# mrjoshuak/go-blosc

Measured on AMD Instinct MI355X. Metric: GB/s compress+decompress, 1 GiB float32 Shuffle+LZ4, higher is better.
Workload: dtype u8; 1 GPU; 1024 MiB f32 frame per GPU, shuffle=1 typesize=4 + LZ4, compress then decompress, device-resident; index_trailer=True, chunk_bytes=4096, decode_entry=hb_decompress_frame_dev_hdr (header known to the host)

## Files before the change

go-blosc_amd/csrc/hb_dec_unit.h:

```cpp
#pragma once
#include "hb_lz4.h"
#include "hb_dec_common.h"

__device__ __forceinline__ uint32_t ld32(const uint8_t *p) { return ld4u(p); }

__device__ __forceinline__ void dec_plan_check(const uint8_t *__restrict__ index, uint64_t index_bytes, uint64_t n_src, uint64_t cap,
                                               DecPlan *plan, hb_result *result) {
    plan->mode = DEC_SERIAL; plan->fail = 0; plan->nunits = 0; plan->nbytes = 0; plan->post = 0; plan->stride = 1;
    result->status = HB_OK; result->flags = 0; result->bytes = 0; result->total_bytes = 0; result->reserved = 0;
    if (!index || index_bytes < HB_IDX_HDR_BYTES + 2 * HB_IDX_ENTRY) return;
    uint32_t h[8];
    for (int i = 0; i < 8; i++) h[i] = ld32(index + 4 * i);
    if (h[0] != HB_IDX_MAGIC || h[1] != (HB_IDX_VERSION | (HB_IDX_ENTRY << 16))) return;
    if (h[7] != (h[0] ^ h[1] ^ h[2] ^ h[3] ^ h[4] ^ h[5])) return;
    const uint64_t nunits = h[2];
    if (nunits == 0 || HB_IDX_HDR_BYTES + (nunits + 1) * HB_IDX_ENTRY > index_bytes) return;
    if (h[4] != n_src || h[5] > cap) return;
    if (h[3] != HB_CHUNK || nunits != ((uint64_t)h[5] + HB_CHUNK - 1) / HB_CHUNK) return;
    plan->nunits = (uint32_t)nunits;
    plan->nbytes = h[5];
    const uint32_t m = ((uint32_t)nunits + 7u) / 8u;
    uint32_t P = m / 4u + 1u;
    for (;;) {
        uint32_t x = P, y = m;
        while (y) { const uint32_t t = x % y; x = y; y = t; }
        if (x == 1u) break;
        P++;
    }
    plan->stride = P;
    plan->mode = DEC_INDEXED;
}

#ifndef DEC_IN_WIN
#define DEC_IN_WIN  1536u
#endif
#define DEC_IN_MARGIN 320u
#define DEC_OUT_MAX HB_CHUNK
#ifndef DEC_LEAN
#define DEC_LEAN 1
#endif
#ifndef DEC_WAVES
#define DEC_WAVES 6
#endif

struct DecCtx {
    const uint8_t *src; uint64_t n_src;
    uint8_t *dst;
    const uint8_t *ent;
    DecPlan *plan;
    uint32_t nbytes, nunits;
    int bun4, ush;
};
#ifndef DEC_PREFETCH
#define DEC_PREFETCH 0
#endif
#ifndef DEC_STAGE_DEPTH
#define DEC_STAGE_DEPTH 4
#endif
#define DEC_NO_UNIT 0xFFFFFFFFu
struct DecPre {
    uint32_t u;
    uint32_t e[8];
    uint32_t win;
};
typedef const __attribute__((address_space(4))) uint32_t *dec_cu32p;
__device__ __forceinline__ void dec_ld_uniform16(const uint8_t *p, uint32_t *o) {
    const uintptr_t a = (uintptr_t)p;
    const dec_cu32p q = (dec_cu32p)(a & ~(uintptr_t)3);
    const uint32_t sh = ((uint32_t)a & 3u) * 8u;
    const uint32_t w0 = q[0], w1 = q[1], w2 = q[2], w3 = q[3];
    uint32_t w4 = w3;
    if (sh != 0u) w4 = q[4];
    const uint32_t r0 = sh ? (uint32_t)((((uint64_t)w1 << 32) | w0) >> sh) : w0, r1 = sh ? (uint32_t)((((uint64_t)w2 << 32) | w1) >> sh) : w1;
    const uint32_t r2 = sh ? (uint32_t)((((uint64_t)w3 << 32) | w2) >> sh) : w2, r3 = sh ? (uint32_t)((((uint64_t)w4 << 32) | w3) >> sh) : w3;
    o[0] = (uint32_t)__builtin_amdgcn_readfirstlane((int)r0); o[1] = (uint32_t)__builtin_amdgcn_readfirstlane((int)r1);
    o[2] = (uint32_t)__builtin_amdgcn_readfirstlane((int)r2); o[3] = (uint32_t)__builtin_amdgcn_readfirstlane((int)r3);
}
__device__ __forceinline__ uint32_t dec_ld_uniform1(const uint8_t *p) {
    const uintptr_t a = (uintptr_t)p;
    return (uint32_t)__builtin_amdgcn_readfirstlane((int)((*(dec_cu32p)(a & ~(uintptr_t)3) >> (((uint32_t)a & 3u) * 8u)) & 255u));
}

template <int USH, class F>
__device__ __forceinline__ void dec_flush_ush(uint8_t *udst, const uint8_t *s_out, const uint32_t outlen, const int lane, const uint32_t ush_rt, F &&after) {
#if defined(LAB_DEC_FLUSH) && LAB_DEC_FLUSH == 1
    after();
#elif defined(LAB_DEC_FLUSH) && LAB_DEC_FLUSH == 2
    for (uint32_t i = lane * 16u; i < outlen; i += 1024u) st16u(udst + i, *(const u32x4 *)(s_out + i));
    after();
#else
    const uint32_t ush = USH > 0 ? (uint32_t)USH : ush_rt;
    constexpr uint32_t G = USH == 4 ? 8u : 16u;
    const uint32_t step = 64u * ush;
    uint8_t *p = udst + (uint32_t)lane * ush;
    const uint8_t *q = s_out + lane;
#if DEC_PREFETCH
    if (USH > 0 && outlen == DEC_OUT_MAX) {
#pragma unroll
        for (uint32_t g = 0; g < DEC_OUT_MAX / (64u * G); g++) {
#pragma unroll
            for (uint32_t k = 0; k < G; k++) p[k * step] = q[64u * k];
            p += G * step; q += 64u * G;
        }
        after();
        return;
    }
#endif
    uint32_t i = 0;
    for (; i + 64u * G <= outlen; i += 64u * G) {
#pragma unroll
        for (uint32_t k = 0; k < G; k++) p[k * step] = q[64u * k];
        p += G * step; q += 64u * G;
    }
    for (i += (uint32_t)lane; i < outlen; i += 64u) { *p = *q; p += step; q += 64; }
    after();
#endif
}
template <int USH, int BUN4>
__device__ __forceinline__ void dec_unit(const DecCtx &c, const uint32_t u, uint8_t *s_in, uint8_t *s_out, uint2 *s_tq, const int lane,
                                         const uint32_t u_next, DecPre &pre) {
    const uint8_t *const src = c.src; const uint64_t n_src = c.n_src; uint8_t *const dst = c.dst; const uint8_t *const ent = c.ent;
    DecPlan *const plan = c.plan; const uint32_t nbytes = c.nbytes, nunits = c.nunits;
    const int bun4 = BUN4 < 0 ? c.bun4 : BUN4, ush = USH < 0 ? c.ush : USH;
#define RFL(x) ((uint32_t)__builtin_amdgcn_readfirstlane((int)(x)))
#if DEC_PREFETCH
#define DEC_LD_BYTE(p) dec_ld_uniform1(p)
    uint32_t e[8];
    const bool have = pre.u == u;
    const bool staged0 = have && pre.win != 0u;
    if (have) { for (int k = 0; k < 8; k++) e[k] = pre.e[k]; }
    else { dec_ld_uniform16(ent + 16 * (size_t)u, e); dec_ld_uniform16(ent + 16 * (size_t)(u + 1), e + 4); }
    pre.u = DEC_NO_UNIT; pre.win = 0u;
    const uint32_t s0 = e[0], d0 = e[1], s1 = e[4], d1 = e[5], rem1 = e[6], tok1 = e[7];
    uint32_t rem = e[2], tokpos = e[3];
    uint32_t en[8];
    if (u_next != DEC_NO_UNIT) { dec_ld_uniform16(ent + 16 * (size_t)u_next, en); dec_ld_uniform16(ent + 16 * (size_t)(u_next + 1u), en + 4); }
#else
#define DEC_LD_BYTE(p) RFL((uint32_t)*(p))
    const bool staged0 = false;
    const u32x4 e0 = ld16u(ent + 16 * (size_t)u), e1 = ld16u(ent + 16 * (size_t)(u + 1));
    const uint32_t s0 = RFL(e0.x), d0 = RFL(e0.y), s1 = RFL(e1.x), d1 = RFL(e1.y), rem1 = RFL(e1.z), tok1 = RFL(e1.w);
    uint32_t rem = RFL(e0.z), tokpos = RFL(e0.w);
#endif
    const bool last = (u + 1 == nunits);
    bool ok = s0 <= s1 && s1 <= n_src && d0 <= d1 && d1 <= nbytes && (d1 - d0) <= DEC_OUT_MAX;
    if (u == 0) ok = ok && s0 == 0 && d0 == 0 && rem == HB_IDX_AT_TOKEN;
    if (last) ok = ok && s1 == n_src && d1 == nbytes;
    if (rem != HB_IDX_AT_TOKEN && tokpos >= n_src) ok = false;
    if (bun4 && ((d0 | d1) & 31u)) ok = false;
    const uint32_t ne = ush ? nbytes / (uint32_t)ush : 1u;
    const uint32_t pj = ush ? d0 / ne : 0u;
    if (ush && (pj >= (uint32_t)ush || d1 > (pj + 1u) * ne)) ok = false;
    uint8_t *const udst = ush ? dst + (size_t)(d0 - pj * ne) * (uint32_t)ush + pj : dst + d0;
    if (!ok) { if (lane == 0) atomicExch(&plan->fail, 1u); return; }
    const uint32_t slen = s1 - s0, outlen = d1 - d0;
    const uint8_t *g = src + s0;
    u32x4 pv0 = {0u, 0u, 0u, 0u}, pv1 = {0u, 0u, 0u, 0u};
    uint32_t pnv = 0;
    auto pf_issue = [&]() __attribute__((always_inline)) {
#if DEC_PREFETCH
        if (u_next == DEC_NO_UNIT) return;
        pre.u = u_next;
        for (int k = 0; k < 8; k++) pre.e[k] = en[k];
        const uint32_t ns0 = en[0], nd0 = en[1], nrem = en[2], ns1 = en[4], nd1 = en[5];
        if (!(ns0 <= ns1 && ns1 <= n_src && nd0 <= nd1 && nd1 <= nbytes && (nd1 - nd0) <= DEC_OUT_MAX)) return;
        if (nrem != HB_IDX_AT_TOKEN && nrem >= nd1 - nd0) return;
        const uint8_t *ng = src + ns0;
        const uint32_t nsh = (uint32_t)((uintptr_t)ng & 15u);
        const uint32_t avail = nsh + (ns1 - ns0);
        pnv = ((avail < DEC_IN_WIN ? avail : DEC_IN_WIN) + 15u) >> 4;
        const u32x4 *ga = (const u32x4 *)(ng - nsh);
        if ((uint32_t)lane < pnv) pv0 = ga[lane];
        if ((uint32_t)lane + 64u < pnv) pv1 = ga[lane + 64];
#endif
    };
    auto pf_commit = [&]() __attribute__((always_inline)) {
#if DEC_PREFETCH
        if (pnv == 0u) return;
        wave_sync();
        if ((uint32_t)lane < pnv) ((u32x4 *)s_in)[lane] = pv0;
        if ((uint32_t)lane + 64u < pnv) ((u32x4 *)s_in)[lane + 64] = pv1;
        pre.win = 1u;
        wave_sync();
#endif
    };

    if (rem != HB_IDX_AT_TOKEN && rem >= outlen) {
        const uint32_t left = rem - outlen;
        bool fine = slen == outlen;
        if (last) fine = fine && left == 0 && (DEC_LD_BYTE(src + tokpos) & 15u) == 0u; else fine = fine && rem1 == left && tok1 == tokpos;
        if (!fine) { if (lane == 0) atomicExch(&plan->fail, 1u); return; }
        if (ush) {
#if DEC_STAGE_DEPTH > 1
            constexpr int LD = (USH < 0 && DEC_STAGE_DEPTH > 2) ? 2 : DEC_STAGE_DEPTH;
            for (uint32_t i0 = lane * 16u; i0 < outlen; i0 += 1024u * LD) {
                u32x4 lv[LD];
#pragma unroll
                for (int k = 0; k < LD; k++) {
                    const uint32_t i = i0 + 1024u * k;
                    lv[k] = u32x4{0u, 0u, 0u, 0u};
                    if (i + 16u <= outlen) lv[k] = ld16u(g + i);
                }
#pragma unroll
                for (int k = 0; k < LD; k++) {
                    const uint32_t i = i0 + 1024u * k;
                    if (i + 16u <= outlen) *(u32x4 *)(s_out + i) = lv[k];
                    else for (uint32_t r = i; r < outlen; r++) s_out[r] = g[r];
                }
            }
#else
            for (uint32_t i = lane * 16u; i < outlen; i += 1024u) {
                if (i + 16u <= outlen) *(u32x4 *)(s_out + i) = ld16u(g + i);
                else for (uint32_t r = i; r < outlen; r++) s_out[r] = g[r];
            }
#endif
            wave_sync();
            pf_issue();
            dec_flush_ush<USH>(udst, s_out, outlen, lane, (uint32_t)ush, pf_commit);
            wave_sync();
            return;
        }
        pf_issue();
        if (!bun4) wave_copy_g2g(dst + d0, g, outlen, lane);
        else {
            for (uint32_t w = lane; w < outlen / 32u; w += 64) {
                u32x4 oa, ob;
                bitshuffle4_window<true>(ld16u(g + 32u * w), ld16u(g + 32u * w + 16u), oa, ob);
                st16u(dst + d0 + 32u * w, oa);
                st16u(dst + d0 + 32u * w + 16u, ob);
            }
        }
        pf_commit();
        return;
    }

    const uint32_t sh = (uint32_t)((uintptr_t)g & 15u);
    uint32_t wlo = 0, staged = 0;
    int shw = 0;
    auto stage = [&](const uint32_t at, const bool there = false) __attribute__((always_inline)) {
        wave_sync();
        const uint32_t a16 = (sh + at) & ~15u;
        const uint32_t avail = sh + slen - a16;
        const uint32_t cnt = avail < DEC_IN_WIN ? avail : DEC_IN_WIN;
        const u32x4 *ga = (const u32x4 *)(g - sh + a16);
        const uint32_t nv = (cnt + 15u) >> 4;
#if DEC_STAGE_DEPTH > 1
        if (!there) {
            constexpr int SV = (int)(((DEC_IN_WIN + 15u) / 16u + 63u) / 64u);
            static_assert(SV <= 4, "stage(): four vectors per lane");
            const u32x4 *gl = ga + lane; u32x4 *sl = (u32x4 *)s_in + lane;
            const uint32_t ul = (uint32_t)lane;
            u32x4 a0, a1, a2, a3;
            if (SV > 0 && ul < nv) a0 = gl[0];
            if (SV > 1 && ul + 64u < nv) a1 = gl[64];
            if (SV > 2 && ul + 128u < nv) a2 = gl[128];
            if (SV > 3 && ul + 192u < nv) a3 = gl[192];
            if (SV > 0 && ul < nv) sl[0] = a0;
            if (SV > 1 && ul + 64u < nv) sl[64] = a1;
            if (SV > 2 && ul + 128u < nv) sl[128] = a2;
            if (SV > 3 && ul + 192u < nv) sl[192] = a3;
        }
#else
        if (!there) for (uint32_t i = lane; i < nv; i += 64) ((u32x4 *)s_in)[i] = ga[i];
#endif
        wlo = a16 > sh ? a16 - sh : 0u;
        staged = a16 + cnt - sh;
        shw = (int)sh - (int)a16;
        wave_sync();
    };
#if DEC_STAGE_DEPTH > 1 && !DEC_PREFETCH
    uint32_t tokv = 0;
    if (rem != HB_IDX_AT_TOKEN) tokv = (uint32_t)src[tokpos];
    stage(0u, staged0);
    uint32_t tok = RFL(tokv);
#else
    stage(0u, staged0);
    uint32_t tok = 0;
    if (rem != HB_IDX_AT_TOKEN) tok = DEC_LD_BYTE(src + tokpos);
#endif
#define INB(i) s_in[(uint32_t)((int)(i) + shw)]
    uint32_t si = 0, di = 0;
    bool at_token = false;
    bool done = false;

    int slow = 1;
    uint32_t nq = 0;
    uint32_t last_ntok = DEC_BPERM_MIN; (void)last_ntok;
    if (rem == HB_IDX_AT_TOKEN) { rem = 0; slow = 0; }
    while (ok && !done) {
        if (slow) {
            if (slow == 2) {
                if (si >= slen) { ok = false; break; }
                tokpos = s0 + si;
                tok = RFL((uint32_t)((si >= wlo && si < staged) ? INB(si) : g[si]));
                si++;
                rem = tok >> 4;
                if (rem == 15u && !dec_read_ext(s_in, shw, wlo, staged, g, slen, si, rem, lane)) { ok = false; break; }
            }
            slow = 0;
            {
                const uint32_t take = min(rem, outlen - di);
                if (take > slen - si) { ok = false; break; }
                if (si >= wlo && si + take <= staged) { for (uint32_t i = lane; i < take; i += 64) s_out[di + i] = INB(si + i); }
                else { for (uint32_t i = lane; i < take; i += 64) s_out[di + i] = g[si + i]; }
                si += take; di += take; rem -= take;
            }
            if (rem > 0 || di == outlen) { at_token = false; done = true; break; }
            if (slen - si < 2) { ok = false; break; }
            const uint32_t b0 = RFL((uint32_t)((si >= wlo && si < staged) ? INB(si) : g[si]));
            const uint32_t b1 = RFL((uint32_t)((si + 1 >= wlo && si + 1 < staged) ? INB(si + 1) : g[si + 1]));
            const uint32_t offset = b0 | (b1 << 8);
            si += 2;
            uint32_t mlen = (tok & 15u) + 4u;
            if ((tok & 15u) == 15u && !dec_read_ext(s_in, shw, wlo, staged, g, slen, si, mlen, lane)) { ok = false; break; }
            if (offset == 0 || offset > di || mlen > outlen - di) { ok = false; break; }
            dec_match_copy(s_out, di, offset, mlen, lane);
            di += mlen;
            if (si >= wlo && si + 4u <= staged && di < outlen) {
                const uint32_t t2 = RFL((uint32_t)INB(si)), l2 = t2 >> 4;
                if (l2 < 15u && (t2 & 15u) == 15u) {
                    const uint32_t op = si + 1u + l2;
                    if (op + 3u <= staged && RFL((uint32_t)INB(op + 2u)) == 255u) slow = 2;
                }
            }
            continue;
        }
        if (nq == 0u && staged < slen && si + DEC_IN_MARGIN > staged) {
            stage(si);
        }
#if DEC_LEAN
        const bool stop = dec_fill_lean(s_in, (uint32_t)shw, staged, slen, si, nq, s_tq, lane, last_ntok);
        bool rewound = false;
        ok = dec_drain<true>(s_in, shw, s_out, outlen, 0u, di, si, nq, s_tq, stop, rewound, lane);
#else
        const bool stop = dec_fill(s_in, (uint32_t)shw, staged, slen, si, nq, s_tq, lane);
        bool rewound = false;
        ok = dec_drain(s_in, shw, s_out, outlen, 0u, di, si, nq, s_tq, stop, rewound, lane);
#endif
        if (!ok) break;
        if (rewound) { slow = 2; continue; }
        if (stop) {
            if (si == slen || di == outlen) { at_token = true; done = true; }
            else if (staged < slen && si + DEC_IN_MARGIN > staged) continue;
            else slow = 2;
        }
    }
    if (ok) {
        ok = (si == slen) && (di == outlen);
        if (last) ok = ok && (at_token || (rem == 0 && (tok & 15u) == 0u));
        else if (at_token) ok = ok && rem1 == HB_IDX_AT_TOKEN;
        else ok = ok && rem1 == rem && tok1 == tokpos;
    }
    if (!ok) { if (lane == 0) atomicExch(&plan->fail, 1u); wave_sync(); return; }
    wave_sync();
    pf_issue();
    if (bun4) {
        for (uint32_t w = lane; w < outlen / 32u; w += 64) {
            u32x4 oa, ob;
            bitshuffle4_window<true>(((const u32x4 *)s_out)[2 * w], ((const u32x4 *)s_out)[2 * w + 1], oa, ob);
            ((u32x4 *)s_out)[2 * w] = oa;
            ((u32x4 *)s_out)[2 * w + 1] = ob;
        }
        wave_sync();
    }
    if (ush) {
        dec_flush_ush<USH>(udst, s_out, outlen, lane, (uint32_t)ush, pf_commit);
    } else {
        uint8_t *o = dst + d0;
        uint32_t head = (uint32_t)((16u - ((uintptr_t)o & 15u)) & 15u);
        if (head > outlen) head = outlen;
        if ((uint32_t)lane < head) o[lane] = s_out[lane];
        const uint32_t body = (outlen - head) >> 4;
        if (head == 0) { for (uint32_t i = lane; i < body; i += 64) *(u32x4 *)(o + i * 16u) = *(const u32x4 *)(s_out + i * 16u); }
        else {
            for (uint32_t i = lane; i < body; i += 64) {
                const uint8_t *q = s_out + head + i * 16u;
                u32x4 v;
                v.x = (uint32_t)q[0] | ((uint32_t)q[1] << 8) | ((uint32_t)q[2] << 16) | ((uint32_t)q[3] << 24);
                v.y = (uint32_t)q[4] | ((uint32_t)q[5] << 8) | ((uint32_t)q[6] << 16) | ((uint32_t)q[7] << 24);
                v.z = (uint32_t)q[8] | ((uint32_t)q[9] << 8) | ((uint32_t)q[10] << 16) | ((uint32_t)q[11] << 24);
                v.w = (uint32_t)q[12] | ((uint32_t)q[13] << 8) | ((uint32_t)q[14] << 16) | ((uint32_t)q[15] << 24);
                *(u32x4 *)(o + head + i * 16u) = v;
            }
        }
        const uint32_t done_b = head + body * 16u;
        if (done_b + lane < outlen) o[done_b + lane] = s_out[done_b + lane];
        pf_commit();
    }
    wave_sync();
}
#undef DEC_LD_BYTE
```

go-blosc_amd/csrc/hb_getitem.hip:

```cpp
#include "hb_frame_plan.h"
#include "hb_dec_common.h"
#include "hb_dec_unit.h"
#include <vector>
#include <cstring>

namespace {

enum { GI_NONE = 0, GI_BYTE = 1, GI_BIT = 2 };

struct GiGeom {
    uint32_t mode, ts, ne, nbytes;
    uint32_t start, nitems;
    uint32_t nplanes, upp;
    uint32_t flo, fhi;
};

__host__ __device__ __forceinline__ void gi_range(const GiGeom &g, uint32_t j, uint32_t &lo, uint32_t &hi) {
    if (g.mode == GI_BYTE) { lo = j * g.ne + g.start; hi = lo + g.nitems; }
    else { lo = g.flo; hi = g.fhi; }
}
__device__ __forceinline__ const uint8_t *gi_src(const uint8_t *base, const GiGeom &g, uint32_t j, int staged) {
    uint32_t lo, hi;
    gi_range(g, j, lo, hi);
    return staged ? base + (size_t)j * g.upp * HB_CHUNK + (lo & (HB_CHUNK - 1u)) : base + lo;
}
__device__ __forceinline__ bool gi_indexed_ok(const DecPlan *plan) { return plan->mode == DEC_INDEXED && plan->fail == 0u; }

__global__ void k_gi_plan(const uint8_t *__restrict__ index, uint64_t index_bytes, uint64_t n_src, uint32_t nbytes, DecPlan *plan, hb_result *result) {
    dec_plan_check(index, index_bytes, n_src, (uint64_t)nbytes, plan, result);
    if (plan->mode == DEC_INDEXED && plan->nbytes != nbytes) plan->mode = DEC_SERIAL;
}

__device__ __forceinline__ void gi_unit_item(const uint8_t *__restrict__ src, uint64_t n_src, const uint8_t *ent, DecPlan *plan, uint32_t nunits, uint8_t *stage,
                                             const GiGeom &g, uint32_t it, uint8_t *s_in, uint8_t *s_out, uint2 *s_tq, int lane) {
    const uint32_t j = it / g.upp, k = it % g.upp;
    uint32_t lo, hi;
    gi_range(g, j, lo, hi);
    const uint32_t u0 = lo / HB_CHUNK, u = u0 + k;
    if (u > (hi - 1u) / HB_CHUNK) return;
    bool ok = u < nunits;
    if (ok) {
        const uint32_t d0 = RFL(ld4u(ent + 16 * (size_t)u + 4)), d1 = RFL(ld4u(ent + 16 * (size_t)(u + 1) + 4));
        const uint64_t end = (uint64_t)HB_CHUNK * (u + 1u);
        ok = d0 == HB_CHUNK * u && d1 == (uint32_t)(end < g.nbytes ? end : g.nbytes);
    }
    if (!ok) { if (lane == 0) atomicExch(&plan->fail, 1u); return; }
    DecCtx c; c.src = src; c.n_src = n_src; c.ent = ent; c.plan = plan; c.nbytes = g.nbytes; c.nunits = nunits; c.bun4 = 0; c.ush = 0;
    c.dst = (uint8_t *)((uintptr_t)stage + ((size_t)j * g.upp + k) * HB_CHUNK - (size_t)HB_CHUNK * u);
    DecPre pre; pre.u = DEC_NO_UNIT; pre.win = 0u;
    dec_unit<0, 0>(c, u, s_in, s_out, s_tq, lane, DEC_NO_UNIT, pre);
}

__global__ __launch_bounds__(64) __attribute__((amdgpu_waves_per_eu(DEC_WAVES))) void k_gi_units(const uint8_t *__restrict__ src, uint64_t n_src,
                                                    const uint8_t *__restrict__ index, DecPlan *plan, uint8_t *stage, const GiGeom g) {
    __shared__ __attribute__((aligned(16))) uint8_t s_in[DEC_IN_WIN + 128];
    __shared__ __attribute__((aligned(16))) uint8_t s_out[DEC_OUT_MAX + 64];
    __shared__ __attribute__((aligned(16))) uint2 s_tq[DEC_LEAN ? DTQ / 4 : DTQ];
    if (plan->mode != DEC_INDEXED) return;
    const int lane = threadIdx.x;
    const uint32_t nunits = plan->nunits;
    const uint8_t *ent = index + HB_IDX_HDR_BYTES;
    const uint32_t total = g.nplanes * g.upp;
    for (uint32_t it = blockIdx.x; it < total; it += gridDim.x) gi_unit_item(src, n_src, ent, plan, nunits, stage, g, it, s_in, s_out, s_tq, lane);
}

__device__ __forceinline__ bool gi_gate(const DecPlan *plan, const hb_result *r3) {
    if (r3) return !(plan && gi_indexed_ok(plan)) && r3->status == HB_OK;
    return !plan || gi_indexed_ok(plan);
}

template <int TS>
__device__ __forceinline__ void gi_gather_vec(uint8_t *__restrict__ dst, const uint8_t *__restrict__ base, const GiGeom &g, int staged, uint32_t head, uint32_t bx) {
    const uint32_t ngrp = (g.nitems - head) / 16u;
    const uint32_t t = bx * 256u + threadIdx.x;
    if (t < ngrp) {
        const uint32_t i0 = head + 16u * t;
        u32x4 p[TS], o[TS];
#pragma unroll
        for (int j = 0; j < TS; j++) p[j] = ld16u(gi_src(base, g, (uint32_t)j, staged) + i0);
        if constexpr (TS == 2) {
#pragma unroll
            for (int w = 0; w < 8; w++) o[w / 4][w % 4] = __builtin_amdgcn_perm(p[1][w / 2], p[0][w / 2], (w & 1) ? 0x07030602u : 0x05010400u);
        } else {
            constexpr int G = TS / 4;
            uint32_t T[G][16];
#pragma unroll
            for (int q = 0; q < G; q++)
#pragma unroll
                for (int k = 0; k < 4; k++)
                    transpose4x4(p[4 * q][k], p[4 * q + 1][k], p[4 * q + 2][k], p[4 * q + 3][k], T[q][4 * k], T[q][4 * k + 1], T[q][4 * k + 2], T[q][4 * k + 3]);
#pragma unroll
            for (int w = 0; w < 4 * TS; w++) o[w / 4][w % 4] = T[w % G][w / G];
        }
        uint8_t *d = dst + (size_t)i0 * TS;
#pragma unroll
        for (int q = 0; q < TS; q++) st16u(d + 16 * q, o[q]);
    }
    if (bx == 0) {
        const uint32_t body_end = head + 16u * ngrp, nedge = head + (g.nitems - body_end);
        for (uint32_t b = threadIdx.x; b < nedge * TS; b += 256u) {
            const uint32_t ie = b / TS, j = b % TS, i = ie < head ? ie : body_end + (ie - head);
            dst[(size_t)i * TS + j] = gi_src(base, g, j, staged)[i];
        }
    }
}
template <int TS>
__global__ __launch_bounds__(256) void k_gi_gather_vec(uint8_t *__restrict__ dst, const uint8_t *__restrict__ base, const DecPlan *plan, const GiGeom g,
                                                        int staged, uint32_t head) {
    if (!gi_gate(plan, nullptr)) return;
    gi_gather_vec<TS>(dst, base, g, staged, head, blockIdx.x);
}
__device__ __forceinline__ void gi_gather_bytes(uint8_t *__restrict__ dst, const uint8_t *__restrict__ base, const GiGeom &g, int staged, uint32_t bx, uint32_t gx) {
    const uint64_t total = (uint64_t)g.nitems * g.ts, stride = (uint64_t)gx * 256u;
    for (uint64_t b = (uint64_t)bx * 256u + threadIdx.x; b < total; b += stride) {
        const uint32_t i = (uint32_t)(b / g.ts), j = (uint32_t)(b % g.ts);
        dst[b] = gi_src(base, g, j, staged)[i];
    }
}
__global__ __launch_bounds__(256) void k_gi_gather_bytes(uint8_t *__restrict__ dst, const uint8_t *__restrict__ base, const DecPlan *plan, const GiGeom g, int staged) {
    if (!gi_gate(plan, nullptr)) return;
    gi_gather_bytes(dst, base, g, staged, blockIdx.x, gridDim.x);
}

__device__ __forceinline__ void gi_copy(uint8_t *__restrict__ dst, const uint8_t *__restrict__ src, uint64_t len, uint32_t bx, uint32_t gx) {
    const int lane = threadIdx.x & 63;
    const uint64_t nseg = (len + HB_CHUNK - 1) / HB_CHUNK, nw = (uint64_t)gx * 4u;
    for (uint64_t sgm = (uint64_t)bx * 4u + (threadIdx.x >> 6); sgm < nseg; sgm += nw) {
        const uint64_t at = sgm * HB_CHUNK;
        wave_copy_g2g(dst + at, src + at, (uint32_t)(len - at < HB_CHUNK ? len - at : HB_CHUNK), lane);
    }
}
__global__ __launch_bounds__(256) void k_gi_copy(uint8_t *__restrict__ dst, const uint8_t *__restrict__ src, uint64_t len, const DecPlan *plan, const hb_result *r3) {
    if (!gi_gate(plan, r3)) return;
    gi_copy(dst, src, len, blockIdx.x, gridDim.x);
}

__device__ __forceinline__ void gi_bit_verbatim(uint8_t *__restrict__ dst, const uint8_t *__restrict__ f, const GiGeom &g, uint64_t idx, uint64_t stride) {
    const uint32_t full = g.ne / 8u * 8u, e = g.start + g.nitems, v0 = g.start > full ? g.start : full;
    if (e <= v0) return;
    const uint64_t vb = (uint64_t)(e - v0) * g.ts;
    for (; idx < vb; idx += stride) dst[(size_t)(v0 - g.start) * g.ts + idx] = f[(size_t)v0 * g.ts + idx];
}
__device__ __forceinline__ void gi_bit_windows(const GiGeom &g, uint32_t &w0, uint32_t &w1) {
    const uint32_t full = g.ne / 8u * 8u, e = g.start + g.nitems, we = e < full ? e : full;
    w0 = g.start / 8u; w1 = (we + 7u) / 8u;
    if (g.start >= full || g.nitems == 0u) w1 = w0;
}
__device__ __forceinline__ void gi_bitun(uint8_t *__restrict__ dst, const uint8_t *__restrict__ f, const GiGeom &g, uint32_t bx, uint32_t gx) {
    uint32_t w0, w1;
    gi_bit_windows(g, w0, w1);
    const uint32_t e = g.start + g.nitems;
    const uint64_t total = (uint64_t)(w1 - w0) * g.ts, stride = (uint64_t)gx * 256u, tid = (uint64_t)bx * 256u + threadIdx.x;
    for (uint64_t idx = tid; idx < total; idx += stride) {
        const uint32_t w = w0 + (uint32_t)(idx / g.ts), bp = (uint32_t)(idx % g.ts);
        const uint8_t *s = f + (size_t)w * 8u * g.ts + 8u * bp;
        uint64_t x = 0;
#pragma unroll
        for (int i = 0; i < 8; i++) x |= (uint64_t)s[i] << (8 * i);
        const uint64_t y = bit_transpose8x8_msb(x);
#pragma unroll
        for (int el = 0; el < 8; el++) {
            const uint32_t i = 8u * w + (uint32_t)el;
            if (i >= g.start && i < e) dst[(size_t)(i - g.start) * g.ts + bp] = (uint8_t)(y >> (8 * el));
        }
    }
    gi_bit_verbatim(dst, f, g, tid, stride);
}
__global__ __launch_bounds__(256) void k_gi_bitun(uint8_t *__restrict__ dst, const uint8_t *__restrict__ f, const DecPlan *plan, const GiGeom g) {
    if (!gi_gate(plan, nullptr)) return;
    gi_bitun(dst, f, g, blockIdx.x, gridDim.x);
}
__device__ __forceinline__ void gi_bitun4(uint8_t *__restrict__ dst, const uint8_t *__restrict__ f, const GiGeom &g, uint32_t bx, uint32_t gx) {
    uint32_t w0, w1;
    gi_bit_windows(g, w0, w1);
    const uint32_t e = g.start + g.nitems;
    const uint64_t stride = (uint64_t)gx * 256u, tid = (uint64_t)bx * 256u + threadIdx.x;
    for (uint64_t idx = tid; idx < w1 - w0; idx += stride) {
        const uint32_t w = w0 + (uint32_t)idx;
        u32x4 oa, ob;
        bitshuffle4_window<true>(ld16u(f + (size_t)w * 32u), ld16u(f + (size_t)w * 32u + 16u), oa, ob);
        if (8u * w >= g.start && 8u * w + 8u <= e) {
            st16u(dst + (size_t)(8u * w - g.start) * 4u, oa);
            st16u(dst + (size_t)(8u * w - g.start) * 4u + 16u, ob);
        } else {
            const uint32_t el[8] = {oa.x, oa.y, oa.z, oa.w, ob.x, ob.y, ob.z, ob.w};
#pragma unroll
            for (int k = 0; k < 8; k++) {
                const uint32_t i = 8u * w + (uint32_t)k;
                if (i >= g.start && i < e) st4u(dst + (size_t)(i - g.start) * 4u, el[k]);
            }
        }
    }
    gi_bit_verbatim(dst, f, g, tid, stride);
}
__global__ __launch_bounds__(256) void k_gi_bitun4(uint8_t *__restrict__ dst, const uint8_t *__restrict__ f, const DecPlan *plan, const GiGeom g) {
    if (!gi_gate(plan, nullptr)) return;
    gi_bitun4(dst, f, g, blockIdx.x, gridDim.x);
}

__device__ __forceinline__ void gi_finish(const DecPlan *plan, const hb_result *r3, hb_result *result, uint64_t bytes, int preset) {
    int status = HB_OK; uint32_t flags = 0;
    if (preset >= 0) flags = (uint32_t)preset;
    else if (plan && gi_indexed_ok(plan)) flags = 3u;
    else if (r3) { status = r3->status; flags = r3->flags & 1u; }
    else status = HB_ERR_SHORT_BUFFER;
    result->status = status; result->flags = status ? 0u : flags; result->bytes = status ? 0 : bytes; result->total_bytes = result->bytes; result->reserved = 0;
}
__global__ void k_gi_finish(const DecPlan *plan, const hb_result *r3, hb_result *result, uint64_t bytes, int preset) { gi_finish(plan, r3, result, bytes, preset); }

enum { GIK_VEC2 = 0, GIK_VEC4, GIK_VEC8, GIK_VEC16, GIK_BYTES, GIK_BITUN4, GIK_BITUN, GIK_COPY, GIK_COUNT };
struct GiJob {
    GiGeom g;
    const uint8_t *frame;
    uint8_t *dst;
    uint64_t n, stage_off;
    uint32_t cbytes;
    int32_t path, status;
    uint32_t head, nblk;
    uint32_t pad;
};
static_assert(sizeof(GiJob) == 96, "GiJob is uploaded as it is");

__global__ __launch_bounds__(64) void k_gib_plan(const GiJob *__restrict__ jobs, DecPlan *plans, hb_result *results, uint32_t njobs) {
    const uint32_t j = blockIdx.x * 64u + threadIdx.x;
    if (j >= njobs) return;
    const GiJob &J = jobs[j];
    DecPlan *plan = plans + j;
    const uint64_t ioff = ((uint64_t)J.cbytes + 7u) & ~(uint64_t)7;
    dec_plan_check(J.path == 1 ? J.frame + ioff : nullptr, J.n - ioff, (uint64_t)J.cbytes - HB_HEADER_SIZE, (uint64_t)J.g.nbytes, plan, results + j);
    if (plan->mode == DEC_INDEXED && plan->nbytes != J.g.nbytes) plan->mode = DEC_SERIAL;
}

__global__ __launch_bounds__(64) __attribute__((amdgpu_waves_per_eu(DEC_WAVES))) void k_gib_units(const GiJob *__restrict__ jobs, DecPlan *plans,
                                                    const uint32_t *__restrict__ item0, uint32_t njobs, uint32_t total, uint8_t *stage) {
    __shared__ __attribute__((aligned(16))) uint8_t s_in[DEC_IN_WIN + 128];
    __shared__ __attribute__((aligned(16))) uint8_t s_out[DEC_OUT_MAX + 64];
    __shared__ __attribute__((aligned(16))) uint2 s_tq[DEC_LEAN ? DTQ / 4 : DTQ];
    const int lane = threadIdx.x;
    for (uint32_t it = blockIdx.x; it < total; it += gridDim.x) {
        const uint32_t j = hb_owner(item0, njobs, it);
        DecPlan *plan = plans + j;
        if (plan->mode != DEC_INDEXED) continue;
        const GiJob &J = jobs[j];
        const GiGeom g = J.g;
        const uint8_t *ent = J.frame + (((size_t)J.cbytes + 7u) & ~(size_t)7) + HB_IDX_HDR_BYTES;
        gi_unit_item(J.frame + HB_HEADER_SIZE, (uint64_t)J.cbytes - HB_HEADER_SIZE, ent, plan, plan->nunits, stage + J.stage_off, g, it - item0[j], s_in, s_out, s_tq, lane);
    }
}

template <int KIND>
__global__ __launch_bounds__(256) void k_gib_gather(const GiJob *__restrict__ jobs, const DecPlan *plans, const uint32_t *__restrict__ gjob,
                                                     const uint32_t *__restrict__ gblk, uint32_t nkind, uint8_t *stage) {
    const uint32_t i = hb_owner(gblk, nkind, blockIdx.x), j = gjob[i];
    const GiJob &J = jobs[j];
    const int staged = J.path == 1;
    if (!gi_gate(staged ? plans + j : nullptr, nullptr)) return;
    const GiGeom g = J.g;
    const uint32_t bx = blockIdx.x - gblk[i], gx = J.nblk;
    uint8_t *dst = J.dst;
    const uint8_t *base = staged ? stage + J.stage_off : J.frame + HB_HEADER_SIZE;
    if constexpr (KIND <= GIK_VEC16) gi_gather_vec<(2 << KIND)>(dst, base, g, staged, J.head, bx);
    else if constexpr (KIND == GIK_BYTES) gi_gather_bytes(dst, base, g, staged, bx, gx);
    else {
        const uint8_t *f = staged ? base - (size_t)(g.flo & ~(HB_CHUNK - 1u)) : base;
        if constexpr (KIND == GIK_BITUN4) gi_bitun4(dst, f, g, bx, gx);
        else if constexpr (KIND == GIK_BITUN) gi_bitun(dst, f, g, bx, gx);
        else gi_copy(dst, f + g.flo, (uint64_t)g.nitems * g.ts, bx, gx);
    }
}

__global__ __launch_bounds__(64) void k_gib_finish(const GiJob *__restrict__ jobs, const DecPlan *plans, hb_result *results, uint32_t njobs) {
    const uint32_t j = blockIdx.x * 64u + threadIdx.x;
    if (j >= njobs) return;
    const GiJob &J = jobs[j];
    hb_result *r = results + j;
    if (J.path == 0) { r->status = J.status; r->flags = 0; r->bytes = 0; r->total_bytes = 0; r->reserved = 0; return; }
    gi_finish(J.path == 1 ? plans + j : nullptr, nullptr, r, (uint64_t)J.g.nitems * J.g.ts, J.path == 2 ? 2 : -1);
}

inline size_t gi_align(size_t b) { return (b + 255) & ~(size_t)255; }
inline unsigned gi_grid(uint64_t items, unsigned per_block, unsigned cap) {
    const uint64_t b = (items + per_block - 1) / per_block;
    return (unsigned)(b < 1 ? 1 : (b > cap ? cap : b));
}

struct GiCall {
    int path, ts;
    GiGeom g;
    uint64_t bytes;
    size_t stage, small, full, dst3, work3, wb3, n3;
};
enum { GI_OFF_PLAN = 0, GI_OFF_R3 = 64, GI_OFF_STAGE = 256 };

int gi_prepare(const hb_header &h, size_t n, int64_t start, int64_t nitems, int typesize_override, GiCall &c) {
    const int rc = hb_getitem_check(&h, n, start, nitems, typesize_override, 0, &c.ts);
    if (rc) return rc;
    const uint32_t ts = (uint32_t)c.ts;
    GiGeom &g = c.g;
    g.ts = ts; g.nbytes = h.nbytes; g.ne = h.nbytes / ts; g.start = (uint32_t)start; g.nitems = (uint32_t)nitems;
    const int unf = hb_frame_unfilter(h, c.ts, true);
    g.mode = unf == HB_OP_BITUNSHUFFLE ? GI_BIT : unf == HB_OP_UNSHUFFLE ? GI_BYTE : GI_NONE;
    const uint32_t e = g.start + g.nitems;
    g.nplanes = g.mode == GI_BYTE ? ts : 1u;
    g.flo = g.start * ts; g.fhi = e * ts;
    if (g.mode == GI_BIT) {
        const uint32_t full = g.ne / 8u * 8u;
        if (g.start < full) g.flo = g.start / 8u * 8u * ts;
        if (e <= full) g.fhi = (e + 7u) / 8u * 8u * ts;
    }
    g.upp = 0;
    if (g.nitems) g.upp = g.mode == GI_BYTE ? (g.nitems + HB_CHUNK - 2u) / HB_CHUNK + 1u : (g.fhi - 1u) / HB_CHUNK - g.flo / HB_CHUNK + 1u;
    c.bytes = (uint64_t)g.nitems * ts;
    c.path = hb_frame_is_memcpy(h) ? 2 : (hb_codec_carried(h.codec, HB_CARRY_LZ4) && hb_frame_stored_index(h, n)) ? 1 : 3;
    c.stage = c.path == 1 ? gi_align((size_t)g.nplanes * g.upp * HB_CHUNK) + 256 : 0;
    c.small = GI_OFF_STAGE + c.stage;
    c.n3 = c.path == 1 ? (size_t)h.cbytes : n;
    c.wb3 = hb_frame_maybe_foreign(h, c.n3) ? hb_decompress_frame_workspace_foreign(h.nbytes) : hb_decompress_frame_workspace(h.nbytes);
    c.dst3 = c.small;
    c.work3 = c.dst3 + gi_align((size_t)h.nbytes) + 256;
    c.full = c.path == 2 ? c.small : c.work3 + gi_align(c.wb3);
    if (c.path == 3) c.small = c.full;
    return HB_OK;
}

struct GiBatchLayout { size_t jobs, item0, gjob, gblk, upload, plans, stage, total; };
GiBatchLayout gi_batch_layout(size_t njobs, size_t stage_bytes) {
    GiBatchLayout L{};
    size_t o = 0;
    auto take = [&](size_t b) { size_t at = o; o += gi_align(b); return at; };
    L.jobs = take(njobs * sizeof(GiJob));
    L.item0 = take(njobs * 4);
    L.gjob = take(njobs * 4);
    L.gblk = take(njobs * 4);
    L.upload = o;
    L.plans = take(njobs * sizeof(DecPlan));
    L.stage = take(stage_bytes);
    L.total = o;
    return L;
}
static_assert(sizeof(GiJob) + sizeof(DecPlan) + 12 + 6 * 255 <= HB_GETITEM_BATCH_JOB_BYTES, "the per-job constant of include/hipblosc.h");

struct GiBatch {
    std::vector<GiJob> tab;
    std::vector<uint32_t> item0, gjob, gblk;
    uint32_t kind0[GIK_COUNT + 1];
    uint32_t kblocks[GIK_COUNT];
    uint64_t items;
    size_t stage;
};

int gi_gather_shape(const GiCall &c, const uint8_t *dst, uint32_t &head, uint32_t &nblk) {
    const GiGeom &g = c.g;
    head = 0;
    if (g.mode == GI_NONE) { nblk = gi_grid((c.bytes + HB_CHUNK - 1) / HB_CHUNK, 4, 1u << 16); return GIK_COPY; }
    if (g.mode == GI_BIT) {
        const uint64_t nwin = (g.fhi - g.flo) / (8u * g.ts) + 1u;
        if (g.ts == 4u) { nblk = gi_grid(nwin, 256, 1u << 16); return GIK_BITUN4; }
        nblk = gi_grid(nwin * g.ts, 256, 1u << 16); return GIK_BITUN;
    }
    if (g.ts == 2u || g.ts == 4u || g.ts == 8u || g.ts == 16u) {
        const uint32_t h16 = (uint32_t)((16u - ((uintptr_t)dst & 15u)) & 15u);
        head = h16 % g.ts == 0u ? h16 / g.ts : 0u;
        if (head > g.nitems) head = g.nitems;
        nblk = gi_grid((g.nitems - head) / 16u, 256, 1u << 22);
        return g.ts == 2u ? GIK_VEC2 : g.ts == 4u ? GIK_VEC4 : g.ts == 8u ? GIK_VEC8 : GIK_VEC16;
    }
    nblk = gi_grid(c.bytes, 256, 1u << 14);
    return GIK_BYTES;
}

int gi_batch_prepare(int nframes, const hb_header *hdrs, const void *const *d_frame, const size_t *n, int njobs, const hb_getitem_job *jobs,
                     void *const *d_dst, const size_t *cap, int typesize_override, GiBatch &B) {
    if (nframes < 0 || njobs < 0) return HB_ERR_BAD_ARG;
    B.items = 0; B.stage = 0;
    for (int k = 0; k < GIK_COUNT; k++) B.kblocks[k] = 0;
    for (int k = 0; k <= GIK_COUNT; k++) B.kind0[k] = 0;
    if (njobs == 0) return HB_OK;
    if (!hdrs || !n || !jobs) return HB_ERR_BAD_ARG;
    for (int j = 0; j < njobs; j++)
        if (jobs[j].frame >= (uint32_t)nframes || jobs[j].reserved != 0u) return HB_ERR_BAD_ARG;
    const size_t nj = (size_t)njobs;
    B.tab.assign(nj, GiJob{});
    B.item0.assign(nj, 0u); B.gjob.assign(nj, 0u); B.gblk.assign(nj, 0u);
    std::vector<int> kind(nj, -1);
    uint64_t kb[GIK_COUNT] = {0};
    for (size_t j = 0; j < nj; j++) {
        const hb_getitem_job &q = jobs[j];
        const hb_header &h = hdrs[q.frame];
        GiJob &J = B.tab[j];
        B.item0[j] = (uint32_t)B.items;
        GiCall c;
        int st = gi_prepare(h, n[q.frame], q.start, q.nitems, typesize_override, c);
        if (st == HB_OK && c.path == 1) { J.stage_off = B.stage; B.stage += c.stage; }
        if (st == HB_OK && cap && (uint64_t)cap[j] < c.bytes) st = HB_ERR_SHORT_BUFFER;
        if (st == HB_OK && d_frame && (!d_frame[q.frame] || (!d_dst[j] && c.bytes))) st = HB_ERR_BAD_ARG;
        if (st == HB_OK && c.path == 3) st = HB_ERR_SHORT_BUFFER;
        if (st != HB_OK) { J.path = 0; J.status = st; continue; }
        J.g = c.g; J.path = c.path; J.status = HB_OK;
        J.frame = d_frame ? (const uint8_t *)d_frame[q.frame] : nullptr; J.dst = d_dst ? (uint8_t *)d_dst[j] : nullptr;
        J.n = n[q.frame]; J.cbytes = h.cbytes;
        if (!c.g.nitems) continue;
        if (c.path == 1) B.items += (uint64_t)c.g.nplanes * c.g.upp;
        kind[j] = gi_gather_shape(c, J.dst, J.head, J.nblk);
        kb[kind[j]] += J.nblk;
        if (B.items > HB_GETITEM_BATCH_MAX_WORK || kb[kind[j]] > HB_GETITEM_BATCH_MAX_WORK) return HB_ERR_BAD_ARG;
    }
    uint32_t at = 0;
    for (int k = 0; k < GIK_COUNT; k++) {
        B.kind0[k] = at;
        uint32_t blk = 0;
        for (size_t j = 0; j < nj; j++)
            if (kind[j] == k) { B.gjob[at] = (uint32_t)j; B.gblk[at] = blk; blk += B.tab[j].nblk; at++; }
        B.kblocks[k] = blk;
    }
    B.kind0[GIK_COUNT] = at;
    return HB_OK;
}

}

extern "C" {

size_t hb_getitem_frames_batch_workspace(int nframes, const hb_header *hdrs, const size_t *n, int njobs, const hb_getitem_job *jobs, int typesize_override) {
    GiBatch B;
    if (gi_batch_prepare(nframes, hdrs, nullptr, n, njobs, jobs, nullptr, nullptr, typesize_override, B)) return 0;
    const size_t total = gi_batch_layout((size_t)njobs, B.stage).total;
    return total ? total : 256;
}

int hb_getitem_frames_batch_device(int nframes, const hb_header *hdrs, const void *const *d_frame, const size_t *n, int njobs, const hb_getitem_job *jobs,
                                   void *const *d_dst, const size_t *cap, int typesize_override, void *d_work, size_t work_bytes, hb_result *d_results,
                                   void *stream) {
    if (nframes < 0 || njobs < 0) return HB_ERR_BAD_ARG;
    if (njobs == 0) return HB_OK;
    if (!hdrs || !d_frame || !n || !jobs || !d_dst || !cap || !d_work || ((uintptr_t)d_work & 255u) || !d_results) return HB_ERR_BAD_ARG;
    GiBatch B;
    const int rc = gi_batch_prepare(nframes, hdrs, d_frame, n, njobs, jobs, d_dst, cap, typesize_override, B);
    if (rc) return rc;
    const GiBatchLayout L = gi_batch_layout((size_t)njobs, B.stage);
    if (work_bytes < L.total) return HB_ERR_SHORT_BUFFER;
    if (hb_init() != HB_OK) return HB_ERR_NO_DEVICE;
    hipStream_t s = (hipStream_t)stream;
    uint8_t *w = (uint8_t *)d_work;
    const size_t nj = (size_t)njobs;
    std::vector<uint8_t> up(L.upload, 0);
    memcpy(up.data() + L.jobs, B.tab.data(), nj * sizeof(GiJob));
    memcpy(up.data() + L.item0, B.item0.data(), nj * 4);
    memcpy(up.data() + L.gjob, B.gjob.data(), nj * 4);
    memcpy(up.data() + L.gblk, B.gblk.data(), nj * 4);
    hb_prof_begin("gib_upload", s);
    HB_HIP_TRY(hipMemcpyAsync(w, up.data(), L.upload, hipMemcpyHostToDevice, s));
    hb_prof_end(s);
    const GiJob *d_jobs = (const GiJob *)(w + L.jobs);
    DecPlan *d_plans = (DecPlan *)(w + L.plans);
    const uint32_t *d_item0 = (const uint32_t *)(w + L.item0), *d_gjob = (const uint32_t *)(w + L.gjob), *d_gblk = (const uint32_t *)(w + L.gblk);
    uint8_t *d_stage = w + L.stage;
    const unsigned jgrid = (unsigned)((nj + 63) / 64);
    hb_prof_begin("k_gib_plan", s);
    hipLaunchKernelGGL(k_gib_plan, dim3(jgrid), dim3(64), 0, s, d_jobs, d_plans, d_results, (uint32_t)njobs);
    hb_prof_end(s);
    if (B.items) {
        const uint32_t total = (uint32_t)B.items;
        hb_prof_begin("k_gib_units", s);
        hipLaunchKernelGGL(k_gib_units, dim3(total < 65536u ? total : 65536u), dim3(64), 0, s, d_jobs, d_plans, d_item0, (uint32_t)njobs, total, d_stage);
        hb_prof_end(s);
    }
    for (int k = 0; k < GIK_COUNT; k++) {
        const uint32_t k0 = B.kind0[k], nk = B.kind0[k + 1] - k0, blocks = B.kblocks[k];
        if (!nk) continue;
        hb_prof_begin("k_gib_gather", s);
#define GIB_LAUNCH(K) hipLaunchKernelGGL(k_gib_gather<K>, dim3(blocks), dim3(256), 0, s, d_jobs, (const DecPlan *)d_plans, d_gjob + k0, d_gblk + k0, nk, d_stage)
        switch (k) {
        case GIK_VEC2: GIB_LAUNCH(GIK_VEC2); break;
        case GIK_VEC4: GIB_LAUNCH(GIK_VEC4); break;
        case GIK_VEC8: GIB_LAUNCH(GIK_VEC8); break;
        case GIK_VEC16: GIB_LAUNCH(GIK_VEC16); break;
        case GIK_BYTES: GIB_LAUNCH(GIK_BYTES); break;
        case GIK_BITUN4: GIB_LAUNCH(GIK_BITUN4); break;
        case GIK_BITUN: GIB_LAUNCH(GIK_BITUN); break;
        default: GIB_LAUNCH(GIK_COPY); break;
        }
#undef GIB_LAUNCH
        hb_prof_end(s);
    }
    hb_prof_begin("k_gib_finish", s);
    hipLaunchKernelGGL(k_gib_finish, dim3(jgrid), dim3(64), 0, s, d_jobs, (const DecPlan *)d_plans, d_results, (uint32_t)njobs);
    hb_prof_end(s);
    HB_HIP_TRY(hipGetLastError());
    return HB_OK;
}

size_t hb_getitem_frame_workspace(const hb_header *hdr, size_t n, int64_t start, int64_t nitems, int typesize_override, int full) {
    GiCall c;
    if (!hdr || gi_prepare(*hdr, n, start, nitems, typesize_override, c)) return 0;
    return full ? c.full : c.small;
}

int hb_getitem_frame_device(const hb_header *hdr, const void *d_frame, size_t n, int64_t start, int64_t nitems, void *d_dst, size_t cap,
                            int typesize_override, void *d_work, size_t work_bytes, hb_result *d_result, void *stream) {
    if (!hdr) return HB_ERR_BAD_ARG;
    GiCall c;
    int rc = gi_prepare(*hdr, n, start, nitems, typesize_override, c);
    if (rc) return rc;
    if ((uint64_t)cap < c.bytes) return HB_ERR_SHORT_BUFFER;
    if (hb_init() != HB_OK) return HB_ERR_NO_DEVICE;
    if (!d_frame || !d_work || ((uintptr_t)d_work & 255u) || !d_result || (!d_dst && c.bytes)) return HB_ERR_BAD_ARG;
    if (work_bytes < c.small) return HB_ERR_SHORT_BUFFER;
    const hb_header &h = *hdr;
    const GiGeom &g = c.g;
    hipStream_t s = (hipStream_t)stream;
    uint8_t *w = (uint8_t *)d_work, *dst = (uint8_t *)d_dst;
    DecPlan *plan = (DecPlan *)(w + GI_OFF_PLAN);
    hb_result *r3 = (hb_result *)(w + GI_OFF_R3);
    const uint8_t *payload = (const uint8_t *)d_frame + HB_HEADER_SIZE;
    const bool have3 = c.path == 3 || (c.path == 1 && work_bytes >= c.full);

    if (c.path != 3) {
        const DecPlan *gate = c.path == 1 ? plan : nullptr;
        const int staged = c.path == 1;
        const uint8_t *base = staged ? w + GI_OFF_STAGE : payload;
        if (c.path == 1) {
            const size_t ioff = hb_frame_index_offset(h);
            const uint8_t *index = (const uint8_t *)d_frame + ioff;
            hb_prof_begin("k_gi_plan", s);
            hipLaunchKernelGGL(k_gi_plan, dim3(1), dim3(1), 0, s, index, (uint64_t)(n - ioff), (uint64_t)(h.cbytes - HB_HEADER_SIZE), h.nbytes, plan, d_result);
            hb_prof_end(s);
            if (g.nitems) {
                const uint32_t total = g.nplanes * g.upp;
                hb_prof_begin("k_gi_units", s);
                hipLaunchKernelGGL(k_gi_units, dim3(total < 65536u ? total : 65536u), dim3(64), 0, s, payload, (uint64_t)(h.cbytes - HB_HEADER_SIZE), index, plan,
                                   w + GI_OFF_STAGE, g);
                hb_prof_end(s);
            }
        }
        if (g.nitems) {
            hb_prof_begin("k_gi_gather", s);
            const uint8_t *f = staged ? base - (size_t)(g.flo & ~(HB_CHUNK - 1u)) : base;
            if (g.mode == GI_NONE) {
                hipLaunchKernelGGL(k_gi_copy, dim3(gi_grid((c.bytes + HB_CHUNK - 1) / HB_CHUNK, 4, 1u << 16)), dim3(256), 0, s, dst, f + g.flo, c.bytes, gate, (const hb_result *)nullptr);
            } else if (g.mode == GI_BIT) {
                const uint64_t nwin = (g.fhi - g.flo) / (8u * g.ts) + 1u;
                if (g.ts == 4u) hipLaunchKernelGGL(k_gi_bitun4, dim3(gi_grid(nwin, 256, 1u << 16)), dim3(256), 0, s, dst, f, gate, g);
                else hipLaunchKernelGGL(k_gi_bitun, dim3(gi_grid(nwin * g.ts, 256, 1u << 16)), dim3(256), 0, s, dst, f, gate, g);
            } else if (g.ts == 2u || g.ts == 4u || g.ts == 8u || g.ts == 16u) {
                const uint32_t h16 = (uint32_t)((16u - ((uintptr_t)dst & 15u)) & 15u);
                uint32_t head = h16 % g.ts == 0u ? h16 / g.ts : 0u;
                if (head > g.nitems) head = g.nitems;
                const unsigned grid = gi_grid((g.nitems - head) / 16u, 256, 1u << 22);
                switch (g.ts) {
                case 2: hipLaunchKernelGGL(k_gi_gather_vec<2>, dim3(grid), dim3(256), 0, s, dst, base, gate, g, staged, head); break;
                case 4: hipLaunchKernelGGL(k_gi_gather_vec<4>, dim3(grid), dim3(256), 0, s, dst, base, gate, g, staged, head); break;
                case 8: hipLaunchKernelGGL(k_gi_gather_vec<8>, dim3(grid), dim3(256), 0, s, dst, base, gate, g, staged, head); break;
                default: hipLaunchKernelGGL(k_gi_gather_vec<16>, dim3(grid), dim3(256), 0, s, dst, base, gate, g, staged, head); break;
                }
            } else {
                hipLaunchKernelGGL(k_gi_gather_bytes, dim3(gi_grid(c.bytes, 256, 1u << 14)), dim3(256), 0, s, dst, base, gate, g, staged);
            }
            hb_prof_end(s);
        }
    }
    if (have3) {
        rc = hb_decompress_frame_dev_hdr(hdr, d_frame, c.n3, w + c.dst3, h.nbytes, typesize_override, w + c.work3, c.wb3, r3, stream);
        if (rc) return rc;
        if (c.bytes) {
            hb_prof_begin("k_gi_copy", s);
            hipLaunchKernelGGL(k_gi_copy, dim3(gi_grid((c.bytes + HB_CHUNK - 1) / HB_CHUNK, 4, 1u << 16)), dim3(256), 0, s, dst, (const uint8_t *)(w + c.dst3) + (size_t)g.start * g.ts,
                               c.bytes, c.path == 1 ? (const DecPlan *)plan : (const DecPlan *)nullptr, (const hb_result *)r3);
            hb_prof_end(s);
        }
    }
    hb_prof_begin("k_gi_finish", s);
    hipLaunchKernelGGL(k_gi_finish, dim3(1), dim3(1), 0, s, c.path == 1 ? (const DecPlan *)plan : (const DecPlan *)nullptr, have3 ? (const hb_result *)r3 : (const hb_result *)nullptr,
                       d_result, c.bytes, c.path == 2 ? 2 : -1);
    hb_prof_end(s);
    HB_HIP_TRY(hipGetLastError());
    return HB_OK;
}

}
```

go-blosc_amd/csrc/hb_lz4_dec.hip:

```cpp
#include "hb_lz4.h"
#include "hb_dec_common.h"
#include "hb_dec_unit.h"

size_t hb_lz4_dec_workspace(size_t n_out) { return 256 + hb_lz4_region_workspace(n_out); }

__global__ void k_dec_plan(const uint8_t *__restrict__ index, uint64_t index_bytes, uint64_t n_src, uint64_t cap,
                           DecPlan *plan, hb_result *result) {
    dec_plan_check(index, index_bytes, n_src, cap, plan, result);
}

template <int USH, int BUN4>
__global__ __launch_bounds__(64) __attribute__((amdgpu_waves_per_eu(DEC_WAVES))) void k_dec_indexed(const uint8_t *__restrict__ src, uint64_t n_src,
                                                    uint8_t *__restrict__ dst, const uint8_t *__restrict__ index,
                                                    DecPlan *plan, int bun4_rt, int ush_rt, uint32_t plane_mask) {
    const int bun4 = BUN4 < 0 ? bun4_rt : BUN4, ush = USH < 0 ? ush_rt : USH;
    __shared__ __attribute__((aligned(16))) uint8_t s_in[DEC_IN_WIN + 128];
    __shared__ __attribute__((aligned(16))) uint8_t s_out[DEC_OUT_MAX + 64];
    __shared__ __attribute__((aligned(16))) uint2 s_tq[DEC_LEAN ? DTQ / 4 : DTQ];
    if (plan->mode != DEC_INDEXED) return;
    const int lane = threadIdx.x;
    const uint32_t nunits = plan->nunits;
    const uint8_t *ent = index + HB_IDX_HDR_BYTES;
    const uint32_t nbytes = plan->nbytes;

    const uint32_t P = plan->stride;
    const uint32_t mgrp = (nunits + 7u) / 8u;
    auto unit_of = [&](const uint32_t it) __attribute__((always_inline)) -> uint32_t {
        if (it >= mgrp * 8u) return DEC_NO_UNIT;
        uint32_t u = (uint32_t)(((uint64_t)(it >> 3) * P) % mgrp) * 8u + ((it + (it >> 3)) & 7u);
        const bool fused_order = ush && nunits % (uint32_t)ush == 0u && (gridDim.x % (8u * (uint32_t)ush) == 0u || gridDim.x >= nunits);
        if (fused_order ? it >= nunits : u >= nunits) return DEC_NO_UNIT;
        if (fused_order) {
            const uint32_t T = (uint32_t)ush, nblk = nunits / T;
            const uint32_t grp = it / (8u * T), r = it % (8u * T);
            uint32_t b = grp * 8u + (r & 7u), j = ((r >> 3) + it / gridDim.x) % T;
            if (grp * 8u + 8u > nblk) {
                const uint32_t k = it - grp * 8u * T, nb = nblk - grp * 8u;
                b = grp * 8u + k % nb; j = k / nb;
            }
            u = j * nblk + b;
            if (!((plane_mask >> j) & 1u)) return DEC_NO_UNIT;
        }
        return u;
    };
    DecCtx c; c.src = src; c.n_src = n_src; c.dst = dst; c.ent = ent; c.plan = plan; c.nbytes = nbytes; c.nunits = nunits; c.bun4 = bun4; c.ush = ush;
    DecPre pre; pre.u = DEC_NO_UNIT; pre.win = 0u;
    for (uint32_t it = blockIdx.x; it < mgrp * 8u; it += gridDim.x) {
        const uint32_t u = unit_of(it);
        if (u == DEC_NO_UNIT) continue;
        const uint32_t u_next = DEC_PREFETCH ? unit_of(it + gridDim.x) : DEC_NO_UNIT;
        dec_unit<USH, BUN4>(c, u, s_in, s_out, s_tq, lane, u_next, pre);
    }
}

__global__ __launch_bounds__(64) void k_bt_dec_plan(const DecBatchFrame *__restrict__ bf, uint32_t nframes, uint32_t *__restrict__ unit_frame, uint32_t total_units) {
    const uint32_t f = blockIdx.x;
    const DecBatchFrame b = bf[f];
    const uint32_t next = f + 1 < nframes ? bf[f + 1].unit0 : total_units;
    __shared__ uint32_t s_mode;
    if (threadIdx.x == 0) {
        dec_plan_check(b.preset == 1 ? b.index : nullptr, b.index_bytes, b.n_src, (uint64_t)b.nbytes, b.plan, b.result);
        b.plan->pad[0] = 0; b.plan->pad[1] = 0;
        if (b.plan->mode == DEC_INDEXED && (b.plan->nunits != b.nunits || b.plan->nbytes != b.nbytes)) b.plan->mode = DEC_SERIAL;
        s_mode = b.plan->mode;
    }
    __syncthreads();
    const bool indexed = s_mode == DEC_INDEXED;
    for (uint32_t u = threadIdx.x; u < next - b.unit0; u += 64) unit_frame[b.unit0 + u] = (u < b.nunits && indexed) ? f : 0xFFFFFFFFu;
}

__global__ __launch_bounds__(64) __attribute__((amdgpu_waves_per_eu(DEC_WAVES))) void k_dec_indexed_batch(const DecBatchFrame *__restrict__ bf,
                                                    const uint32_t *__restrict__ unit_frame, uint32_t total_units) {
    __shared__ __attribute__((aligned(16))) uint8_t s_in[DEC_IN_WIN + 128];
    __shared__ __attribute__((aligned(16))) uint8_t s_out[DEC_OUT_MAX + 64];
    __shared__ __attribute__((aligned(16))) uint2 s_tq[DEC_LEAN ? DTQ / 4 : DTQ];
    const int lane = threadIdx.x;
    for (uint32_t it = blockIdx.x; it < total_units; it += gridDim.x) {
        const uint32_t fid = unit_frame[it];
        if (fid == 0xFFFFFFFFu) continue;
        const DecBatchFrame &f = bf[fid];
        DecCtx c; c.src = f.src; c.n_src = f.n_src; c.dst = f.dst; c.ent = f.index + HB_IDX_HDR_BYTES; c.plan = f.plan;
        c.nbytes = f.nbytes; c.nunits = f.nunits; c.bun4 = f.bun4; c.ush = f.ush;
        uint32_t u = it - f.unit0;
        if (c.ush) {
            const uint32_t T = (uint32_t)c.ush, nblk = c.nunits / T;
            const uint32_t grp = u / (8u * T), r = u % (8u * T);
            uint32_t b = grp * 8u + (r & 7u), j = ((r >> 3) + it / gridDim.x) % T;
            if (grp * 8u + 8u > nblk) { const uint32_t k = u - grp * 8u * T, nb = nblk - grp * 8u; b = grp * 8u + k % nb; j = k / nb; }
            u = j * nblk + b;
        }
        if (u >= c.nunits) continue;
        DecPre pre; pre.u = DEC_NO_UNIT; pre.win = 0u;
        dec_unit<-1, -1>(c, u, s_in, s_out, s_tq, lane, DEC_NO_UNIT, pre);
    }
}

size_t hb_lz4_dec_batch_units(int nframes, const DecBatchFrame *h, uint32_t *unit0_out) {
    uint64_t units = 0;
    for (int k = 0; k < nframes; k++) {
        const uint32_t g = h[k].ush ? 8u * (uint32_t)h[k].ush : 8u;
        units = (units + g - 1) / g * g;
        unit0_out[k] = (uint32_t)units;
        units += h[k].nunits;
    }
    return (size_t)((units + 7) / 8 * 8);
}

int hb_launch_lz4_decode_batch_indexed(int nframes, const DecBatchFrame *d_bf, uint32_t *d_unit_frame, uint32_t total_units, int any_ush, hipStream_t s) {
    hb_prof_begin("k_dec_plan", s);
    hipLaunchKernelGGL(k_bt_dec_plan, dim3((unsigned)nframes), dim3(64), 0, s, d_bf, (uint32_t)nframes, d_unit_frame, total_units);
    hb_prof_end(s);
    if (total_units) {
        unsigned grid = total_units < 256u * 256u ? total_units : 256u * 256u;
        if (any_ush && total_units > 256u * 16u) {
            const unsigned gran = 32u;
            unsigned g2 = total_units / (unsigned)any_ush / gran * gran;
            if (total_units > 256u * 64u && g2 < 256u * 64u) g2 = 256u * 64u;
            if (g2 > 256u * 256u) g2 = 256u * 256u;
            if (g2) grid = g2;
        }
        hb_prof_begin("k_dec_indexed", s);
        hipLaunchKernelGGL(k_dec_indexed_batch, dim3(grid), dim3(64), 0, s, d_bf, (const uint32_t *)d_unit_frame, total_units);
        hb_prof_end(s);
    }
    HB_HIP_TRY(hipGetLastError());
    return HB_OK;
}


__global__ __launch_bounds__(64) void k_dec_serial(const uint8_t *__restrict__ src, uint64_t n_src,
                                                   uint8_t *__restrict__ dst, uint64_t cap, DecPlan *plan,
                                                   hb_result *result, int frame, uint32_t expect, int mark_post) {
    __shared__ __attribute__((aligned(16))) uint8_t s_win[SER_WIN + 128];
    __shared__ __attribute__((aligned(16))) uint8_t s_img[SER_HIST + SER_PAGE + 1024];
    __shared__ __attribute__((aligned(16))) uint2 s_tq[DTQ];
    const int lane = threadIdx.x;
    if (plan->mode == DEC_INDEXED && !plan->fail) {
        if (lane == 0) {
            const uint64_t got = plan->nbytes;
            result->flags = 1; result->bytes = got; result->total_bytes = got;
            result->status = (frame && got != expect) ? HB_ERR_SIZE_MISMATCH : HB_OK;
        }
        return;
    }
    if (mark_post && lane == 0) plan->post = 1;
    int err;
    const uint64_t got = dec_serial_core(src, n_src, dst, cap, s_win, s_img, s_tq, lane, err);
    if (lane == 0) {
        result->flags = 0; result->total_bytes = 0;
        if (err) { result->status = HB_ERR_DECOMPRESSION_FAILED; result->bytes = 0; }
        else if (frame && got != expect) { result->status = HB_ERR_SIZE_MISMATCH; result->bytes = got; }
        else { result->status = HB_OK; result->bytes = got; }
    }
}

__global__ void k_set_result(hb_result *result, int status, uint64_t bytes) {
    result->status = status; result->flags = 0; result->bytes = bytes; result->total_bytes = bytes; result->reserved = 0;
}

int hb_launch_lz4_decode(const hb_dec_args &a, hipStream_t s) {
    if (a.memcpy_payload) {
        if (a.n != a.expect) {
            hipLaunchKernelGGL(k_set_result, dim3(1), dim3(1), 0, s, a.result, HB_ERR_SIZE_MISMATCH, (uint64_t)a.n);
        } else {
            if (a.n) HB_HIP_TRY(hipMemcpyAsync(a.dst, a.src, a.n, hipMemcpyDeviceToDevice, s));
            hipLaunchKernelGGL(k_set_result, dim3(1), dim3(1), 0, s, a.result, HB_OK, (uint64_t)a.n);
        }
        HB_HIP_TRY(hipGetLastError());
        return HB_OK;
    }
    DecPlan *plan = (DecPlan *)a.work;
    const uint8_t *index = a.index;
    size_t index_bytes = a.index_bytes;
    if (hb_lz4_region_wanted(a)) {
        const int rc = hb_launch_lz4_region_index(a, &index, &index_bytes, s);
        if (rc) return rc;
    }
    hb_prof_begin("k_dec_plan", s);
    hipLaunchKernelGGL(k_dec_plan, dim3(1), dim3(1), 0, s, index, (uint64_t)index_bytes, (uint64_t)a.n,
                       (uint64_t)a.cap, plan, a.result);
    hb_prof_end(s);
    if (index) {
        const uint64_t units = (a.cap + HB_CHUNK - 1) / HB_CHUNK;
        const uint64_t units8 = (units + 7) / 8 * 8;
        unsigned grid = (unsigned)(units8 < 8 ? 8 : (units8 < 256u * 256u ? units8 : 256u * 256u));
        if (a.fused_unshuffle_ts && units > 256u * 16u) {
            const unsigned gran = 8u * (unsigned)a.fused_unshuffle_ts;
            unsigned g2 = (unsigned)(units / (uint64_t)a.fused_unshuffle_ts) / gran * gran;
            if (units > 256u * 64u && g2 < 256u * 64u) g2 = 256u * 64u;
            if (g2 > 256u * 256u) g2 = 256u * 256u;
            if (g2) grid = g2;
        }
        hb_prof_begin("k_dec_indexed", s);
#define HB_LAUNCH_DEC(USH, BUN4) hipLaunchKernelGGL((k_dec_indexed<USH, BUN4>), dim3(grid), dim3(64), 0, s, a.src, (uint64_t)a.n, a.dst, index, plan, \
                                                    a.fused_bitunshuffle4, a.fused_unshuffle_ts, hb_dbg_plane_mask())
        if (a.fused_bitunshuffle4 && !a.fused_unshuffle_ts) HB_LAUNCH_DEC(0, 1);
        else if (a.fused_bitunshuffle4) HB_LAUNCH_DEC(-1, -1);
        else if (a.fused_unshuffle_ts == 0) HB_LAUNCH_DEC(0, 0);
        else if (a.fused_unshuffle_ts == 2) HB_LAUNCH_DEC(2, 0);
        else if (a.fused_unshuffle_ts == 4) HB_LAUNCH_DEC(4, 0);
        else HB_LAUNCH_DEC(-1, -1);
#undef HB_LAUNCH_DEC
        hb_prof_end(s);
    }
    const int fused_any = a.fused_bitunshuffle4 || a.fused_unshuffle_ts;
    uint8_t *serial_dst = fused_any ? a.staged : a.dst;
    if (hb_lz4_region_wanted(a) && a.sym_work) {
        const int rc = hb_launch_lz4_sym_decode(a, serial_dst, a.sym_work, fused_any, s);
        if (rc) return rc;
    }
    hb_prof_begin("k_dec_serial", s);
    hipLaunchKernelGGL(k_dec_serial, dim3(1), dim3(64), 0, s, a.src, (uint64_t)a.n, serial_dst, (uint64_t)a.cap, plan,
                       a.result, a.frame, a.expect, fused_any);
    hb_prof_end(s);
    if (fused_any) {
        const int rc = a.fused_bitunshuffle4
                           ? hb_launch_filter_gated(HB_OP_BITUNSHUFFLE, a.dst, a.staged, a.expect, 4, &plan->post, s)
                           : hb_launch_filter_gated(HB_OP_UNSHUFFLE, a.dst, a.staged, a.expect, a.fused_unshuffle_ts, &plan->post, s);
        if (rc) return rc;
    }
    HB_HIP_TRY(hipGetLastError());
    return HB_OK;
}
```

go-blosc_amd/csrc/hb_lz4_enc.hip:

```cpp
#include "hb_lz4.h"
#include "hb_lz4_batch_frame.h"
#include <cstdlib>
#include <vector>
#include <type_traits>

#ifndef HLOG_HC
#define HLOG_HC 8
#endif
#ifndef ENC_HLOG
#define ENC_HLOG 8
#endif
#ifndef ENC_KEY
#define ENC_KEY 5
#endif
#define HLOGW(WAYS) ((WAYS) == 1 ? ENC_HLOG : HLOG_HC)
#define HSIZEW(WAYS) (1u << HLOGW(WAYS))
#define LITCAP 32u

struct __attribute__((aligned(16))) ChunkDesc {
    uint32_t lead;
    uint32_t enc_len;
    uint32_t last_end;
    uint32_t mcode0;
};

struct Agg {
    int64_t fixed;
    uint32_t F;
    uint32_t E;
    uint32_t has;
    uint32_t pad;
};

__device__ __forceinline__ Agg agg_identity() { Agg r; r.fixed = 0; r.F = 0; r.E = 0; r.has = 0; r.pad = 0; return r; }
__device__ __forceinline__ Agg agg_combine(const Agg &x, const Agg &y) {
    if (!y.has) return x;
    if (!x.has) return y;
    Agg r;
    r.has = 1; r.pad = 0; r.F = x.F; r.E = y.E;
    r.fixed = x.fixed + y.fixed + (int64_t)lz4_ext_bytes(y.F - x.E) - (int64_t)x.E;
    return r;
}
__device__ __forceinline__ Agg agg_of_chunk(const ChunkDesc &d, uint32_t start) {
    Agg r = agg_identity();
    if (d.last_end) {
        r.has = 1; r.F = start + d.lead; r.E = start + d.last_end;
        r.fixed = 1 + (int64_t)start + (int64_t)d.enc_len;
    }
    return r;
}
__device__ __forceinline__ int64_t agg_bytes(const Agg &p) { return p.has ? p.fixed + (int64_t)lz4_ext_bytes(p.F) : 0; }

struct EncPlan {
    uint64_t cbytes_block;
    uint32_t use_memcpy;
    uint32_t nchunks;
    uint64_t index_off;
    uint64_t pad[4];
};


struct EncLayout {
    size_t plan, desc, tile_agg, tile_nf, tile_pre, tile_suf, records, total;
    uint32_t nchunks, ntiles;
};
static inline EncLayout enc_layout(size_t n) {
    EncLayout L;
    L.nchunks = (uint32_t)((n + HB_CHUNK - 1) / HB_CHUNK);
    L.ntiles = (L.nchunks + HB_TILE_CHUNKS - 1) / HB_TILE_CHUNKS;
    size_t o = 0;
    auto take = [&](size_t bytes) { size_t at = o; o += (bytes + 255) & ~(size_t)255; return at; };
    L.plan = take(sizeof(EncPlan));
    L.desc = take((size_t)L.nchunks * sizeof(ChunkDesc));
    L.tile_agg = take((size_t)L.ntiles * sizeof(Agg));
    L.tile_nf = take((size_t)L.ntiles * 4);
    L.tile_pre = take((size_t)L.ntiles * sizeof(Agg));
    L.tile_suf = take((size_t)L.ntiles * 4);
    L.records = take((size_t)L.nchunks * HB_RSTRIDE + 256);
    L.total = o;
    return L;
}
size_t hb_lz4_enc_workspace(size_t n) { return enc_layout(n).total; }

__device__ __forceinline__ uint32_t lds_read4(const uint8_t *base, uint32_t a) {
    const uint32_t *w = (const uint32_t *)base;
    const uint32_t w0 = w[a >> 2], w1 = w[(a >> 2) + 1];
    return __builtin_amdgcn_alignbyte(w1, w0, a & 3u);
}

__device__ __forceinline__ void lds_copy_exact(uint8_t *d, const uint8_t *s, uint32_t len) {
    uint32_t k = 0;
    for (; k + 8u <= len; k += 8u) ((hb_u64u *)(d + k))->v = ((const hb_u64u *)(s + k))->v;
    if (len & 4u) { ((hb_u32u *)(d + k))->v = ((const hb_u32u *)(s + k))->v; k += 4u; }
    if (len & 2u) { ((hb_u16u *)(d + k))->v = ((const hb_u16u *)(s + k))->v; k += 2u; }
    if (len & 1u) d[k] = s[k];
}

#ifndef ENC_EXT_GATE
#define ENC_EXT_GATE 1
#endif
#ifndef ENC_HASH24
#define ENC_HASH24 1
#endif
#ifndef ENC_NOMUL
#define ENC_NOMUL 1
#endif
#ifndef ENC_INNER_STEP
#define ENC_INNER_STEP 1
#endif
#ifndef ENC_WAVES
#define ENC_WAVES 6
#endif
#ifndef ENC_GATE_ADAPT
#define ENC_GATE_ADAPT 0
#endif
#ifndef ENC_GATE_MAXRUNS
#define ENC_GATE_MAXRUNS 7
#endif
#ifndef ENC_GATE_HOLD
#define ENC_GATE_HOLD 3
#endif
#ifndef ENC_RUN_GATE
#define ENC_RUN_GATE 48
#endif
#ifdef ENC_DEBUG_TIMES
__device__ unsigned long long g_enc_t[8][16];
extern "C" int hblab_enc_times(unsigned long long *out, int reset) {
    if (out && hipMemcpyFromSymbol(out, HIP_SYMBOL(g_enc_t), sizeof(g_enc_t)) != hipSuccess) return -1;
    if (reset) { static unsigned long long z[8][16]; if (hipMemcpyToSymbol(HIP_SYMBOL(g_enc_t), z, sizeof(z)) != hipSuccess) return -1; }
    return 0;
}
#define DBG_CLK() ((unsigned long long)__builtin_amdgcn_s_memtime())
#define DBG_ADD(k, v) do { dbg_acc[k] += (unsigned long long)(v); } while (0)
#define DBG_DECL() unsigned long long dbg_acc[14] = {0, 0, 0, 0, 0, 0, 0, 0, 0, 0, 0, 0, 0, 0}
#define DBG_COMMIT() do { if (lane == 0) { for (int k_ = 0; k_ < 14; k_++) if (dbg_acc[k_]) atomicAdd(&g_enc_t[dbg_plane & 7][k_], dbg_acc[k_]); } } while (0)
#else
#define DBG_DECL() do { } while (0)
#define DBG_COMMIT() do { } while (0)
#define DBG_CLK() 0ull
#define DBG_ADD(k, v) do { } while (0)
#endif
#define QCAP 80
#define SOUT 768u

template <int WAYS>
__device__ __forceinline__ uint32_t enc_hash(const uint32_t v, const uint32_t v4) {
#if ENC_HASH24
    if constexpr (WAYS == 1 && ENC_HLOG == 8 && ENC_KEY == 5) {
        const uint32_t z = __builtin_amdgcn_alignbyte(v4, v, 2u);
        return ((uint32_t)__umul24(v, 0xF85117u) + (uint32_t)__umul24(z, 0xE01E5Bu)) >> 24;
    }
#endif
    return ((v + (v4 & (ENC_KEY == 6 && WAYS == 1 ? 0xFFFFu : 255u)) * 0x50505u) * 2246822519u) >> (32 - HLOGW(WAYS));
}

template <int WAYS>
__device__ __forceinline__ uint32_t enc_hash_run(const uint32_t b4) {
#if ENC_HASH24
    if constexpr (WAYS == 1 && ENC_HLOG == 8 && ENC_KEY == 5)
        return ((uint32_t)__umul24(b4, 0xF85117u) + (uint32_t)__umul24(b4, 0xE01E5Bu)) >> 24;
#endif
    return enc_hash<WAYS>(b4, b4);
}

template <int WAYS, int MODE>
__device__ __forceinline__ void match_chunk(const uint8_t *s_data, const uint32_t sh, const int len,
                                            uint8_t *s_out , uint16_t *s_tab, uint2 *s_q , uint32_t *s_st ,
                                            ChunkDesc *dsc, uint8_t *rec, const bool with_trailing, const bool keep_long, const int accel, const int lane,
                                            const int dbg_plane = 0) {
    constexpr bool SNAPPY = MODE == 1;
    constexpr bool SELF = MODE == 2;
    {
        {
            u32x4 z; z.x = 0; z.y = 0; z.z = 0; z.w = 0;
            for (uint32_t i = lane; i < HSIZEW(WAYS) * WAYS * 2 / 16; i += 64) ((u32x4 *)s_tab)[i] = z;
            if (lane < 2) ((u32x4 *)s_st)[lane] = z;
        }
        wave_sync();

        int pos = 0, anchor = 0, nq = 0, miss = 0, gate_left = 0;
#ifdef LAB_ENC
        unsigned long long lab_dummy = 0;
#endif
        int nseq = 0;
        uint32_t rec_done = 0, opend = 0;
        uint32_t batch_anchor = 0, lead = 0, mcode0 = 0;
        auto ld_state = [&]() __attribute__((always_inline)) {
            const u32x4 a = ((const u32x4 *)s_st)[0], b = ((const u32x4 *)s_st)[1];
            nseq = (int)__builtin_amdgcn_readfirstlane(a.x); batch_anchor = __builtin_amdgcn_readfirstlane(a.y);
            lead = __builtin_amdgcn_readfirstlane(a.z); mcode0 = __builtin_amdgcn_readfirstlane(a.w);
            rec_done = __builtin_amdgcn_readfirstlane(b.x); opend = __builtin_amdgcn_readfirstlane(b.y);
        };
        auto st_state = [&]() __attribute__((always_inline)) {
            if (lane == 0) {
                u32x4 a, b;
                a.x = (uint32_t)nseq; a.y = batch_anchor; a.z = lead; a.w = mcode0; b.x = rec_done; b.y = opend; b.z = 0; b.w = 0;
                ((u32x4 *)s_st)[0] = a; ((u32x4 *)s_st)[1] = b;
            }
            wave_sync();
        };
        const int mstart_max = len - 12;
        const int mend_max = len - 5;
        const uint8_t *data = s_data + sh;
#define RD4(x) lds_read4(s_data, sh + (uint32_t)(x))

        auto drain = [&](const bool all) __attribute__((always_inline)) {
            wave_sync();
            const uint32_t full = all ? ((opend + 15u) & ~15u) : (opend & ~15u);
            if (full) {
                for (uint32_t i = lane * 16u; i < full; i += 1024u) *(u32x4 *)(rec + rec_done + i) = *(const u32x4 *)(s_out + i);
                if (!all && lane == 0) { const u32x4 t = *(const u32x4 *)(s_out + full); *(u32x4 *)s_out = t; }
                rec_done += full;
                opend = all ? 0u : opend - full;
                wave_sync();
            }
        };
        auto stream_literals = [&](uint32_t from, uint32_t cnt) __attribute__((always_inline)) {
            while (cnt) {
                const uint32_t piece = cnt < SOUT - opend ? cnt : SOUT - opend;
                for (uint32_t k = lane * 4u; k < piece; k += 256u) {
                    if (k + 4u <= piece) ((hb_u32u *)(s_out + opend + k))->v = RD4(from + k);
                    else for (uint32_t r = k; r < piece; r++) s_out[opend + r] = data[from + r];
                }
                opend += piece; from += piece; cnt -= piece;
                drain(false);
            }
        };

        auto copy_long_literals = [&](unsigned long long lm, const uint32_t prev, const uint32_t litdst, const uint32_t lit) __attribute__((always_inline)) {
            while (lm) {
                const int l = __builtin_ctzll(lm);
                const uint32_t s = __builtin_amdgcn_readlane(prev, l), dq = __builtin_amdgcn_readlane(litdst, l);
                const uint32_t ln = __builtin_amdgcn_readlane(lit, l);
                for (uint32_t k = lane * 4u; k < ln; k += 256u) {
                    if (k + 4u <= ln) ((hb_u32u *)(s_out + dq + k))->v = ((const hb_u32u *)(data + s + k))->v;
                    else for (uint32_t r = k; r < ln; r++) s_out[dq + r] = data[s + r];
                }
                lm &= lm - 1;
            }
        };

        auto flush_end = [&](const uint32_t end, const int cnt, const uint2 r0, const uint2 r1) __attribute__((always_inline)) {
            batch_anchor = __builtin_amdgcn_readlane(end, cnt - 1);
            nseq += cnt;
            drain(false);
            nq -= cnt;
            if (lane < nq) s_q[lane] = r0;
            if (lane + 64 < nq) s_q[lane + 64] = r1;
            st_state();
        };

        auto flush = [&]() __attribute__((always_inline)) {
            ld_state();
            const int take = nq < 64 ? nq : 64;
            const uint2 e = s_q[lane];
            const uint32_t q_mp = e.x & 0xFFFFu, q_ml = e.x >> 16, q_off = e.y;
            const uint32_t end = q_mp + q_ml;
            const uint32_t prev = wave_shr1(end, batch_anchor);
            const uint32_t lit = q_mp - prev, mcode = q_ml - 4u;
            const bool first = !SELF && (nseq == 0) && lane == 0;
            const uint32_t nbl = first ? 0u : lz4_ext_bytes16(lit), nbm = lz4_ext_bytes16(mcode);
            const uint32_t size = lane < take ? ((first ? 0u : 1u) + nbl + lit + 2u + nbm) : 0u;
            const uint32_t incl = wave_incl_scan_dpp(size);
            int cnt = __builtin_popcountll(hb_ballot(lane < take && incl <= SOUT - opend));
            const uint32_t i0 = (uint32_t)(lane + (cnt ? cnt : 1)), i1 = i0 + 64u;
            const uint2 r0 = s_q[i0 < QCAP ? i0 : 0], r1 = s_q[i1 < QCAP ? i1 : 0];
            wave_sync();
            if (nseq == 0) {
                lead = __builtin_amdgcn_readlane(lit, 0);
                const uint32_t m0 = __builtin_amdgcn_readlane(mcode, 0);
                mcode0 = m0 < 15u ? m0 : 15u;
            }
            if (cnt == 0) {
                cnt = 1;
                if (lane == 0) {
                    uint32_t q = opend;
                    if (!first) {
                        s_out[q++] = (uint8_t)((15u << 4) | (mcode < 15u ? mcode : 15u));
                        for (uint32_t k = 0; k + 1 < nbl; k++) s_out[q++] = 255;
                        s_out[q++] = (uint8_t)((lit - 15u) - 255u * (nbl - 1));
                    }
                }
                opend += (uint32_t)__builtin_amdgcn_readlane((first ? 0u : 1u) + nbl, 0);
                wave_sync();
                stream_literals(__builtin_amdgcn_readlane(prev, 0), __builtin_amdgcn_readlane(lit, 0));
                if (lane == 0) {
                    uint32_t q = opend;
                    ((hb_u16u *)(s_out + q))->v = (uint16_t)q_off;
                    q += 2;
                    if (nbm) {
                        for (uint32_t k = 0; k + 1 < nbm; k++) s_out[q++] = 255;
                        s_out[q++] = (uint8_t)((mcode - 15u) - 255u * (nbm - 1));
                    }
                }
                opend += 2u + (uint32_t)__builtin_amdgcn_readlane(nbm, 0);
            } else {
                const bool act = lane < cnt;
                uint32_t q = opend + incl - size;
                const uint32_t litdst = q + (first ? 0u : 1u + nbl);
                if (act && lit <= LITCAP) lds_copy_exact(s_out + litdst, data + prev, lit);
                if (act) {
                    if (!first) {
                        s_out[q++] = (uint8_t)(((lit < 15u ? lit : 15u) << 4) | (mcode < 15u ? mcode : 15u));
                        if (nbl) {
                            for (uint32_t k = 0; k + 1 < nbl; k++) s_out[q++] = 255;
                            s_out[q++] = (uint8_t)((lit - 15u) - 255u * (nbl - 1));
                        }
                    }
                    q += lit;
                    ((hb_u16u *)(s_out + q))->v = (uint16_t)q_off;
                    q += 2;
                    if (nbm) {
                        for (uint32_t k = 0; k + 1 < nbm; k++) s_out[q++] = 255;
                        s_out[q++] = (uint8_t)((mcode - 15u) - 255u * (nbm - 1));
                    }
                }
                copy_long_literals(hb_ballot(act && lit > LITCAP), prev, litdst, lit);
                opend += (uint32_t)__builtin_amdgcn_readlane(incl, cnt - 1);
            }
            flush_end(end, cnt, r0, r1);
        };

        auto sn_lit_header = [&](uint32_t q, uint32_t lit) __attribute__((always_inline)) -> uint32_t {
            const uint32_t x = lit - 1u;
            if (x < 60u) { s_out[q] = (uint8_t)(x << 2); return 1u; }
            if (x < 256u) { s_out[q] = (uint8_t)(60u << 2); s_out[q + 1] = (uint8_t)x; return 2u; }
            s_out[q] = (uint8_t)(61u << 2); s_out[q + 1] = (uint8_t)x; s_out[q + 2] = (uint8_t)(x >> 8); return 3u;
        };
        auto sn_copies = [&](uint32_t q, uint32_t ml, uint32_t off) __attribute__((always_inline)) -> uint32_t {
            const uint32_t q0 = q;
            while (ml >= 68u) { s_out[q] = (uint8_t)((63u << 2) | 2u); s_out[q + 1] = (uint8_t)off; s_out[q + 2] = (uint8_t)(off >> 8); q += 3u; ml -= 64u; }
            if (ml > 64u) { s_out[q] = (uint8_t)((59u << 2) | 2u); s_out[q + 1] = (uint8_t)off; s_out[q + 2] = (uint8_t)(off >> 8); q += 3u; ml -= 60u; }
            if (ml >= 12u || off >= 2048u) { s_out[q] = (uint8_t)(((ml - 1u) << 2) | 2u); s_out[q + 1] = (uint8_t)off; s_out[q + 2] = (uint8_t)(off >> 8); q += 3u; }
            else { s_out[q] = (uint8_t)(((off >> 8) << 5) | ((ml - 4u) << 2) | 1u); s_out[q + 1] = (uint8_t)off; q += 2u; }
            return q - q0;
        };
        auto flush_sn = [&]() __attribute__((always_inline)) {
            ld_state();
            const int take = nq < 64 ? nq : 64;
            const uint2 e = s_q[lane];
            const uint32_t q_mp = e.x & 0xFFFFu, q_ml = e.x >> 16, q_off = e.y;
            const uint32_t end = q_mp + q_ml;
            const uint32_t prev = wave_shr1(end, batch_anchor);
            const uint32_t lit = q_mp - prev;
            const uint32_t lh = lit == 0u ? 0u : (lit <= 60u ? 1u : (lit <= 256u ? 2u : 3u));
            const uint32_t n64 = q_ml >= 68u ? (q_ml - 68u) / 64u + 1u : 0u;
            const uint32_t rem = q_ml - 64u * n64;
            const uint32_t r60 = rem > 64u ? 1u : 0u;
            const uint32_t fin = rem - 60u * r60;
            const uint32_t csz = 3u * (n64 + r60) + ((fin >= 12u || q_off >= 2048u) ? 3u : 2u);
            const uint32_t size = lane < take ? lh + lit + csz : 0u;
            const uint32_t incl = wave_incl_scan_dpp(size);
            int cnt = __builtin_popcountll(hb_ballot(lane < take && incl <= SOUT - opend));
            const uint32_t i0 = (uint32_t)(lane + (cnt ? cnt : 1)), i1 = i0 + 64u;
            const uint2 r0 = s_q[i0 < QCAP ? i0 : 0], r1 = s_q[i1 < QCAP ? i1 : 0];
            wave_sync();
            if (cnt == 0) {
                cnt = 1;
                uint32_t hl = 0;
                if (lane == 0) hl = sn_lit_header(opend, lit);
                opend += (uint32_t)__builtin_amdgcn_readlane(hl, 0);
                wave_sync();
                stream_literals(__builtin_amdgcn_readlane(prev, 0), __builtin_amdgcn_readlane(lit, 0));
                uint32_t cl = 0;
                if (lane == 0) cl = sn_copies(opend, q_ml, q_off);
                opend += (uint32_t)__builtin_amdgcn_readlane(cl, 0);
            } else {
                const bool act = lane < cnt;
                uint32_t q = opend + incl - size;
                uint32_t litdst = 0;
                if (act) {
                    if (lit) q += sn_lit_header(q, lit);
                    litdst = q;
                    if (lit <= LITCAP) lds_copy_exact(s_out + q, data + prev, lit);
                    q += lit;
                    sn_copies(q, q_ml, q_off);
                }
                copy_long_literals(hb_ballot(act && lit > LITCAP), prev, litdst, lit);
                opend += (uint32_t)__builtin_amdgcn_readlane(incl, cnt - 1);
            }
            flush_end(end, cnt, r0, r1);
        };
        DBG_DECL();
        unsigned long long dbg_flush = 0;
        auto flush_any = [&]() __attribute__((always_inline)) {
            const unsigned long long c0 = DBG_CLK();
            if constexpr (SNAPPY) flush_sn(); else flush();
            const unsigned long long c1 = DBG_CLK();
            dbg_flush += c1 - c0; DBG_ADD(8, c1 - c0); DBG_ADD(9, 1);
        };
        (void)dbg_flush;
        const unsigned long long dbg_t0 = DBG_CLK(); (void)dbg_t0;

        auto step = [&](auto inner_tag) __attribute__((always_inline)) {
            constexpr bool INNER = decltype(inner_tag)::value;
            const unsigned long long dbg_s0 = DBG_CLK(); const unsigned long long dbg_f0 = dbg_flush; (void)dbg_s0; (void)dbg_f0;
            const int p = pos + lane;
            const uint32_t ap = sh + (uint32_t)p;
            const uint32_t *wp = (const uint32_t *)s_data + (ap >> 2);
            const uint32_t p0 = wp[0], p1 = wp[1], p2 = wp[2], p3 = wp[3];
            const uint32_t prevb = s_data[sh + (uint32_t)(pos > 0 ? pos - 1 : 0)];
            const uint32_t v = __builtin_amdgcn_alignbyte(p1, p0, ap & 3u);
            const uint32_t v4 = __builtin_amdgcn_alignbyte(p2, p1, ap & 3u);
            const uint32_t v8 = __builtin_amdgcn_alignbyte(p3, p2, ap & 3u);
            const bool valid = INNER || p <= mstart_max;
            const uint32_t vb = v & 255u;
            const uint32_t before = wave_shr1(vb, prevb);
#if ENC_NOMUL
            const uint32_t b4 = __builtin_amdgcn_perm(v, v, 0u);
#else
            const uint32_t b4 = vb * 0x01010101u;
#endif
            const unsigned long long m_first = INNER || pos > 0 ? ~0ull : ~1ull;
            const unsigned long long m_eqprev = hb_ballot(before == vb) & (INNER || len - pos >= 64 ? ~0ull : ((1ull << (len - pos)) - 1ull));
            const unsigned long long m_rle = hb_ballot(valid) & hb_ballot(v == b4) & m_eqprev & m_first;
            const bool rle = valid && (INNER || pos > 0 || lane > 0) && v == b4 && before == vb;
            bool runny = false; (void)runny;
#if ENC_RUN_GATE
            if constexpr (WAYS == 1) {
                uint32_t n_eq, n_runs;
                asm("s_bcnt1_i32_b64 %0, %1" : "=s"(n_eq) : "s"(m_eqprev) : "scc");
                runny = n_eq >= (uint32_t)ENC_RUN_GATE;
                const unsigned long long sel = m_rle & ~(m_rle << 1);
                n_runs = 64u;
                if (runny) asm volatile("s_bcnt1_i32_b64 %0, %1" : "=s"(n_runs) : "s"(sel) : "scc");
                if (runny && (!ENC_GATE_ADAPT || gate_left > 0) && n_runs - 1u < (uint32_t)ENC_GATE_MAXRUNS) {
                    gate_left--;
#if ENC_GATE_ADAPT && !defined(ENC_GATE_NOINS)
                    if (hb_lane_in(sel)) s_tab[enc_hash_run<WAYS>(b4)] = (uint16_t)(p - 1);
#endif
                    const unsigned long long nrun = ~(m_eqprev >> lane);
                    const uint32_t run = nrun ? (uint32_t)__builtin_ctzll(nrun) : 64u;
                    uint32_t ml = min(run, (uint32_t)(mend_max - p));
                    const int lastj = 63 - __builtin_clzll(sel);
                    const int mpj = pos + lastj, maxlj = mend_max - mpj;
                    const int runj = (int)__builtin_amdgcn_readlane(run, lastj);
                    int mlj = runj < maxlj ? runj : maxlj;
                    if (lastj + runj >= 64 && mlj < maxlj) {
                        const uint32_t rb4 = __builtin_amdgcn_readlane(b4, lastj);
                        for (;;) {
                            const int i = mlj + 4 * lane;
                            const int ic = i < maxlj ? i : maxlj;
                            const uint32_t x = RD4(mpj + ic) ^ rb4;
                            int eq = x ? (__builtin_ctz(x) >> 3) : 4;
                            const int avail = maxlj - i;
                            if (avail < eq) eq = avail > 0 ? avail : 0;
                            const unsigned long long part = hb_ballot(eq != 4);
                            if (part) {
                                const int f = __builtin_ctzll(part);
                                mlj += 4 * f + (int)__builtin_amdgcn_readlane((uint32_t)eq, f);
                                break;
                            }
                            mlj += 256;
                        }
                        if (lane == lastj) ml = (uint32_t)mlj;
                    }
                    const uint32_t rank = wave_rank(sel);
                    {
                        uint2 e; e.x = (uint32_t)p | (ml << 16); e.y = 1u;
                        s_q[hb_select_lane(sel, (uint32_t)nq + rank, (uint32_t)QCAP)] = e;
                    }
                    nq += __builtin_popcountll(sel);
                    anchor = mpj + mlj;
                    while (nq >= 64) flush_any();
                    miss = 0;
                    pos = anchor > pos + 64 ? anchor : pos + 64;
                    DBG_ADD(2, DBG_CLK() - dbg_s0 - (dbg_flush - dbg_f0)); DBG_ADD(3, 1);
                    return;
                }
            }
#endif
            const uint32_t h = enc_hash<WAYS>(v, v4);
            uint32_t cand, xa, xb, ac = 0, hc_fbit = 0;
            const uint32_t *wc = nullptr;
            uint32_t c3 = 0;
            bool hit;
            unsigned long long m_hit;
            if constexpr (WAYS == 1) {
                cand = s_tab[h];
                if constexpr (INNER) s_tab[hb_lane_in(m_rle) ? HSIZEW(WAYS) * WAYS : h] = (uint16_t)p;
                else if (valid && !rle) s_tab[h] = (uint16_t)p;
                ac = sh + cand;
                wc = (const uint32_t *)s_data + (ac >> 2);
                const uint32_t c0 = wc[0], c1 = wc[1], c2 = wc[2];
                c3 = wc[3];
                const uint32_t cv = __builtin_amdgcn_alignbyte(c1, c0, ac & 3u);
                const uint32_t cv4 = __builtin_amdgcn_alignbyte(c2, c1, ac & 3u);
                const uint32_t cv8 = __builtin_amdgcn_alignbyte(c3, c2, ac & 3u);
                m_hit = hb_ballot(valid) & hb_ballot((int)cand < p) & hb_ballot(cv == v);
                hit = valid && (int)cand < p && cv == v;
                xa = hit ? (cv4 ^ v4) : (b4 ^ v4); xb = hit ? (cv8 ^ v8) : (b4 ^ v8);
                cand = hit ? cand : (uint32_t)p - 1u;
            } else {
                uint32_t cw[WAYS];
                if constexpr (WAYS == 2) {
                    uint32_t *b = (uint32_t *)s_tab + h;
                    const uint32_t w = *b;
                    cw[0] = w & 0xFFFFu; cw[1] = w >> 16;
                    if (valid && !rle) *b = (uint32_t)p | (cw[0] << 16);
                } else {
                    u32x2 *b = (u32x2 *)s_tab + h;
                    const u32x2 w = *b;
                    cw[0] = w.x & 0xFFFFu; cw[1] = w.x >> 16; cw[2] = w.y & 0xFFFFu; cw[3] = w.y >> 16;
                    if (valid && !rle) { u32x2 nw; nw.x = (uint32_t)p | (cw[0] << 16); nw.y = cw[1] | (cw[2] << 16); *b = nw; }
                }
                const uint32_t p4 = wp[4], p5 = wp[5];
                const uint32_t v12 = __builtin_amdgcn_alignbyte(p4, p3, ap & 3u), v16 = __builtin_amdgcn_alignbyte(p5, p4, ap & 3u);
                hit = false; cand = (uint32_t)p - 1u;
#pragma unroll
                for (int k = 0; k < WAYS; k++) {
                    const uint32_t a2 = sh + cw[k];
                    const uint32_t *w2 = (const uint32_t *)s_data + (a2 >> 2);
                    const uint32_t d0 = w2[0], d1 = w2[1], d2 = w2[2], d3 = w2[3], d4 = w2[4], d5 = w2[5];
                    const uint32_t e0 = __builtin_amdgcn_alignbyte(d1, d0, a2 & 3u), e4 = __builtin_amdgcn_alignbyte(d2, d1, a2 & 3u);
                    const uint32_t e8 = __builtin_amdgcn_alignbyte(d3, d2, a2 & 3u), e12 = __builtin_amdgcn_alignbyte(d4, d3, a2 & 3u);
                    const uint32_t e16 = __builtin_amdgcn_alignbyte(d5, d4, a2 & 3u);
                    uint32_t fa, fb, fc, fd;
                    asm("v_ffbl_b32 %0, %1" : "=v"(fa) : "v"(e4 ^ v4));
                    asm("v_ffbl_b32 %0, %1" : "=v"(fb) : "v"(e8 ^ v8));
                    asm("v_ffbl_b32 %0, %1" : "=v"(fc) : "v"(e12 ^ v12));
                    asm("v_ffbl_b32 %0, %1" : "=v"(fd) : "v"(e16 ^ v16));
                    const uint32_t f = min(fa, min(fb, min(fc, min(fd, 32u) + 32u) + 32u) + 32u);
                    const bool ok = valid && (int)cw[k] < p && e0 == v;
                    if (ok && (!hit || f > hc_fbit)) { hit = true; hc_fbit = f; cand = cw[k]; }
                }
                m_hit = hb_ballot(hit);
                if (!hit) {
                    uint32_t fa, fb, fc, fd;
                    asm("v_ffbl_b32 %0, %1" : "=v"(fa) : "v"(b4 ^ v4));
                    asm("v_ffbl_b32 %0, %1" : "=v"(fb) : "v"(b4 ^ v8));
                    asm("v_ffbl_b32 %0, %1" : "=v"(fc) : "v"(b4 ^ v12));
                    asm("v_ffbl_b32 %0, %1" : "=v"(fd) : "v"(b4 ^ v16));
                    hc_fbit = min(fa, min(fb, min(fc, min(fd, 32u) + 32u) + 32u) + 32u);
                }
                xa = 0; xb = 0;
            }
            unsigned long long mask = m_hit | m_rle;
#if defined(LAB_ENC) && LAB_ENC == 2
            lab_dummy ^= mask; mask = 0; miss = -1;
#endif
            if (mask) {
                uint32_t fbit;
                if constexpr (WAYS == 1) {
                    if (keep_long && hit && (xa | xb) == 0u) s_tab[h] = (uint16_t)cand;
                    uint32_t fa, fb;
                    asm("v_ffbl_b32 %0, %1" : "=v"(fa) : "v"(xa));
                    asm("v_ffbl_b32 %0, %1" : "=v"(fb) : "v"(xb));
#if ENC_EXT_GATE
                    if ((hb_ballot((xa | xb) == 0u) & mask) == 0ull) {
                        fbit = min(fa, min(fb, 32u) + 32u);
                    } else
#endif
                    {
                        const uint32_t p4 = wp[4], p5 = wp[5], c4 = wc[4], c5 = wc[5];
                        const uint32_t v12 = __builtin_amdgcn_alignbyte(p4, p3, ap & 3u), v16 = __builtin_amdgcn_alignbyte(p5, p4, ap & 3u);
                        const uint32_t cv12 = __builtin_amdgcn_alignbyte(c4, c3, ac & 3u), cv16 = __builtin_amdgcn_alignbyte(c5, c4, ac & 3u);
                        const uint32_t xc = hit ? (cv12 ^ v12) : (b4 ^ v12), xd = hit ? (cv16 ^ v16) : (b4 ^ v16);
                        uint32_t fc, fd;
                        asm("v_ffbl_b32 %0, %1" : "=v"(fc) : "v"(xc));
                        asm("v_ffbl_b32 %0, %1" : "=v"(fd) : "v"(xd));
                        fbit = min(fa, min(fb, min(fc, min(fd, 32u) + 32u) + 32u) + 32u);
                    }
                } else {
                    fbit = hc_fbit;
                }
                uint32_t ml = 4u + (fbit >> 3);
                const uint32_t maxl = (uint32_t)(mend_max - p);
                unsigned long long lmask = mask & hb_ballot(fbit == 128u);
                if constexpr (!INNER) { lmask &= hb_ballot(ml < maxl); ml = min(ml, maxl); }
                if (lmask & m_rle & ~m_hit) {
                    const unsigned long long nrun = ~(m_eqprev >> lane);
                    const uint32_t run = nrun ? (uint32_t)__builtin_ctzll(nrun) : 64u;
                    const bool endstop = data[pos + 64] != data[pos + 63];
                    const bool inwin = !hit && fbit == 128u && ((uint32_t)lane + run < 64u || ((uint32_t)lane + run == 64u && endstop));
                    if (inwin) ml = min(run, maxl);
                    lmask &= ~(hb_ballot(inwin) & m_rle);
                }
                unsigned long long sel = 0;
                int last_end = anchor;
                if (lmask == 0) {
                    const uint32_t x = (uint32_t)lane + ml;
                    uint32_t succ = (uint32_t)lane;
                    if (x < 64u) {
                        const unsigned long long m = mask >> x;
                        if (m) succ = x + (uint32_t)__builtin_ctzll(m);
                    }
                    uint32_t lastj;
                    sel = wave_chain_walk(succ, (uint32_t)__builtin_ctzll(mask), lastj);
                    last_end = pos + (int)lastj + (int)__builtin_amdgcn_readlane(ml, (int)lastj);
                    mask = 0;
                }
                while (mask) {
                    const int j = __builtin_ctzll(mask);
                    int mlj = (int)__builtin_amdgcn_readlane(ml, j);
                    if ((lmask >> j) & 1ull) {
                        const int mp = pos + j, mc = (int)__builtin_amdgcn_readlane(cand, j);
                        const int maxl = mend_max - mp;
                        for (;;) {
                            const int i = mlj + 4 * lane;
                            const int ic = i < maxl ? i : maxl;
                            const uint32_t x = RD4(mp + ic) ^ RD4(mc + ic);
                            int eq = x ? (__builtin_ctz(x) >> 3) : 4;
                            const int avail = maxl - i;
                            if (avail < eq) eq = avail > 0 ? avail : 0;
                            const unsigned long long part = hb_ballot(eq != 4);
                            if (part) {
                                const int f = __builtin_ctzll(part);
                                mlj += 4 * f + (int)__builtin_amdgcn_readlane((uint32_t)eq, f);
                                break;
                            }
                            mlj += 256;
                        }
                        if (lane == j) ml = (uint32_t)mlj;
                    }
                    sel |= 1ull << j;
                    const int e = j + mlj;
                    last_end = pos + e;
                    mask = e >= 64 ? 0ull : (mask & (~0ull << e));
                }
#if ENC_RUN_GATE && ENC_GATE_ADAPT
                if constexpr (WAYS == 1) {
                    if (runny) {
                        const unsigned long long rstart = m_rle & ~(m_rle << 1);
                        gate_left = (int)__builtin_popcountll(rstart) <= (int)__builtin_popcountll(sel) + 1 ? ENC_GATE_HOLD : 0;
                    }
                }
#endif
#if defined(LAB_ENC) && LAB_ENC == 1
                lab_dummy ^= sel ^ ml ^ cand;
                anchor = last_end;
#else
                const uint32_t rank = wave_rank(sel);
                {
                    uint2 e; e.x = (uint32_t)p | (ml << 16); e.y = (uint32_t)p - cand;
                    s_q[hb_select_lane(sel, (uint32_t)nq + rank, (uint32_t)QCAP)] = e;
                }
                nq += __builtin_popcountll(sel);
                anchor = last_end;
                while (nq >= 64) flush_any();
#endif
                miss = 0;
                pos = anchor > pos + 64 ? anchor : pos + 64;
                DBG_ADD(0, DBG_CLK() - dbg_s0 - (dbg_flush - dbg_f0)); DBG_ADD(1, 1);
            } else {
                miss++;
                const int nxt = pos + 64 + miss * accel;
                pos = anchor > nxt ? anchor : nxt;
                DBG_ADD(4, DBG_CLK() - dbg_s0); DBG_ADD(5, 1);
            }
                };
        if (ENC_INNER_STEP) {
            if (pos <= mstart_max) step(std::false_type{});
            while (pos + 80 <= mstart_max) step(std::true_type{});
        }
        while (pos <= mstart_max) step(std::false_type{});
        const unsigned long long dbg_t1 = DBG_CLK(); (void)dbg_t1;
        DBG_ADD(6, dbg_t1 - dbg_t0); DBG_ADD(7, 1);
        while (nq > 0) flush_any();
        ld_state();
#ifdef LAB_ENC
        if (lab_dummy == 0x1234567ull) s_out[lane] = 1;
#endif
        auto finish_whole = [&]() __attribute__((always_inline)) {
            const uint32_t total = rec_done + opend;
            drain(true);
            if (lane == 0) {
                ChunkDesc d;
                d.lead = 0u; d.enc_len = total; d.last_end = (uint32_t)len; d.mcode0 = 0u;
                *dsc = d;
            }
            wave_sync();
        };
        if constexpr (SNAPPY) {
            const uint32_t tl = (uint32_t)(len - anchor);
            if (tl) {
                uint32_t hl = 0;
                if (lane == 0) hl = sn_lit_header(opend, tl);
                opend += (uint32_t)__builtin_amdgcn_readlane(hl, 0);
                wave_sync();
                stream_literals((uint32_t)anchor, tl);
            }
            finish_whole();
            return;
        }
        if constexpr (SELF) {
            const uint32_t tl = (uint32_t)(len - anchor);
            const uint32_t nb = lz4_ext_bytes(tl);
            if (lane == 0) {
                uint32_t q = opend;
                s_out[q++] = (uint8_t)((tl < 15u ? tl : 15u) << 4);
                if (nb) { for (uint32_t k = 0; k + 1 < nb; k++) s_out[q++] = 255; s_out[q++] = (uint8_t)((tl - 15u) - 255u * (nb - 1)); }
            }
            opend += 1u + nb;
            wave_sync();
            stream_literals((uint32_t)anchor, tl);
            finish_whole();
            return;
        }
        const uint32_t enc = rec_done + opend;
        if (with_trailing) {
            if (nseq == 0 && sh == 0) {
                for (int i = lane * 16; i < len; i += 64 * 16) *(u32x4 *)(rec + i) = *(const u32x4 *)(s_data + i);
            } else {
                stream_literals((uint32_t)anchor, (uint32_t)(len - anchor));
            }
        }
        drain(true);
        if (lane == 0) {
            ChunkDesc d;
            d.lead = nseq ? lead : 0u; d.enc_len = nseq ? enc : 0u;
            d.last_end = nseq ? (uint32_t)anchor : 0u; d.mcode0 = mcode0;
            *dsc = d;
        }
        wave_sync();
        DBG_ADD(10, DBG_CLK() - dbg_t1);
        DBG_COMMIT();
    }
#undef RD4
}

template <int WAYS, int MODE>
__global__ __launch_bounds__(64) void k_match(const uint8_t *__restrict__ src_, uint64_t n_,
                                              ChunkDesc *__restrict__ desc, uint8_t *__restrict__ records,
                                              uint32_t nchunks, int bits4, int keep_long, int accel,
                                              const BatchFrame *__restrict__ bf, const uint32_t *__restrict__ chunk_frame) {
    __shared__ __attribute__((aligned(16))) uint8_t s_data[HB_CHUNK + 112];
    __shared__ __attribute__((aligned(16))) uint8_t s_out[SOUT + 16];
    __shared__ __attribute__((aligned(16))) uint16_t s_tab[HSIZEW(WAYS) * WAYS + 8];
    static_assert(16 + (QCAP + 1) * 8 <= SOUT + 16, "the sequence queue (+ its spare slot) must fit into the staging buffer");
    uint2 *const s_q = (uint2 *)(s_out + 16);
    uint32_t *const s_st = (uint32_t *)(s_data + HB_CHUNK + 80);
    const int lane = threadIdx.x;
    for (uint32_t ck = blockIdx.x; ck < nchunks; ck += gridDim.x) {
        const uint8_t *src = src_;
        uint64_t n = n_, start = (uint64_t)ck * HB_CHUNK;
        if (bf) {
            const uint32_t fid = chunk_frame[ck];
            if (fid == 0xFFFFFFFFu) continue;
            const BatchFrame &f = bf[fid];
            src = f.src; n = f.n; start = (uint64_t)(ck - f.chunk0) * HB_CHUNK;
        }
        const int len = (int)((n - start) < HB_CHUNK ? (n - start) : HB_CHUNK);
        const uint8_t *g = src + start;
        const uint32_t sh = (uint32_t)((uintptr_t)g & 15u);
        const u32x4 *ga = (const u32x4 *)(g - sh);
        const uint32_t nv = (sh + (uint32_t)len + 15u) >> 4;
        if (!bits4) {
            for (uint32_t i = lane; i < nv; i += 64) ((u32x4 *)s_data)[i] = ga[i];
        } else {
            for (uint32_t w = lane; w < (uint32_t)len / 32u; w += 64) {
                u32x4 oa, ob;
                bitshuffle4_window<false>(ga[2 * w], ga[2 * w + 1], oa, ob);
                ((u32x4 *)s_data)[2 * w] = oa;
                ((u32x4 *)s_data)[2 * w + 1] = ob;
            }
        }
        match_chunk<WAYS, MODE>(s_data, sh, len, s_out, s_tab, s_q, s_st, desc + ck, records + (size_t)ck * HB_RSTRIDE, bits4 != 0, keep_long != 0, accel, lane);
    }
}

template <int TS, int WAYS, int MODE>
__global__ __launch_bounds__(64) __attribute__((amdgpu_waves_per_eu(WAYS == 1 ? ENC_WAVES : 4))) void k_match_fused(const uint8_t *__restrict__ src_, ChunkDesc *__restrict__ desc,
                                                    uint8_t *__restrict__ records, uint32_t nblk_, uint32_t plane_mask, int accel,
                                                    const BatchFrame *__restrict__ bf, const uint32_t *__restrict__ chunk_frame, uint32_t total_) {
    __shared__ __attribute__((aligned(16))) uint8_t s_data[HB_CHUNK + 112];
    __shared__ __attribute__((aligned(16))) uint8_t s_out[SOUT + 16];
    __shared__ __attribute__((aligned(16))) uint16_t s_tab[HSIZEW(WAYS) * WAYS + 8];
    static_assert(16 + (QCAP + 1) * 8 <= SOUT + 16, "the sequence queue (+ its spare slot) must fit into the staging buffer");
    uint2 *const s_q = (uint2 *)(s_out + 16);
    uint32_t *const s_st = (uint32_t *)(s_data + HB_CHUNK + 80);
    const int lane = threadIdx.x;
    const uint32_t total = bf ? total_ : nblk_ * TS;
    for (uint32_t gi = blockIdx.x; gi < total; gi += gridDim.x) {
        const uint8_t *src = src_;
        uint32_t nblk = nblk_, i = gi, ck0 = 0;
        if (bf) {
            const uint32_t fid = chunk_frame[gi];
            if (fid == 0xFFFFFFFFu) continue;
            const BatchFrame &f = bf[fid];
            src = f.src; nblk = f.nblk; ck0 = f.chunk0; i = gi - ck0;
        }
        const uint32_t grp = i / (8u * TS), r = i % (8u * TS);
        uint32_t b = grp * 8u + (r & 7u), j = ((r >> 3) + gi / gridDim.x) % TS;
        if (grp * 8u + 8u > nblk) {
            const uint32_t k = i - grp * 8u * TS;
            const uint32_t nb = nblk - grp * 8u;
            b = grp * 8u + k % nb; j = k / nb;
        }
        if (!((plane_mask >> j) & 1u)) continue;
        const uint64_t e0 = (uint64_t)b * HB_CHUNK;
        wave_sync();
        const int dbg_plane = (int)j; (void)dbg_plane;
        DBG_DECL();
        const unsigned long long dbg_k0 = DBG_CLK(); (void)dbg_k0;
        if constexpr (TS == 2) {
            const uint32_t sel = j ? 0x07050301u : 0x06040200u;
            u32x4 v[HB_CHUNK / 512];
#pragma unroll
            for (int it = 0; it < (int)(HB_CHUNK / 512); it++)
                v[it] = ld16u(src + (e0 + (uint32_t)it * 512u + (uint32_t)lane * 8u) * 2);
#pragma unroll
            for (int it = 0; it < (int)(HB_CHUNK / 512); it++) {
                u32x2 pl;
                pl.x = __builtin_amdgcn_perm(v[it].y, v[it].x, sel);
                pl.y = __builtin_amdgcn_perm(v[it].w, v[it].z, sel);
                *(u32x2 *)&s_data[(uint32_t)it * 512u + (uint32_t)lane * 8u] = pl;
            }
        } else {
            const uint32_t q = j >> 2, rb = j & 3u;
            const uint32_t sel = 0x0c0c0000u | ((4u + rb) << 8) | rb;
            constexpr int NV = TS / 4;
            constexpr int STEPS = (int)(HB_CHUNK / 256);
#ifndef ENC_STAGE_VECS
#define ENC_STAGE_VECS 8
#endif
            constexpr int BATCH = (ENC_STAGE_VECS / NV) < STEPS ? (ENC_STAGE_VECS / NV) : STEPS;
            static_assert(STEPS % BATCH == 0, "chunk size must be a multiple of the staging batch");
#pragma unroll 1
            for (int it0 = 0; it0 < (int)(HB_CHUNK / 256); it0 += BATCH) {
                u32x4 v[BATCH][NV];
#pragma unroll
                for (int k = 0; k < BATCH; k++)
#pragma unroll
                    for (int c = 0; c < NV; c++)
                        v[k][c] = ld16u(src + (e0 + (uint32_t)(it0 + k) * 256u + (uint32_t)lane * 4u) * TS + c * 16);
#pragma unroll
                for (int k = 0; k < BATCH; k++) {
                    uint32_t w0, w1, w2, w3;
                    if constexpr (TS == 4) { w0 = v[k][0].x; w1 = v[k][0].y; w2 = v[k][0].z; w3 = v[k][0].w; }
                    else {
                        w0 = q ? v[k][0].y : v[k][0].x; w1 = q ? v[k][0].w : v[k][0].z;
                        w2 = q ? v[k][1].y : v[k][1].x; w3 = q ? v[k][1].w : v[k][1].z;
                    }
                    const uint32_t t = __builtin_amdgcn_perm(w1, w0, sel), u = __builtin_amdgcn_perm(w3, w2, sel);
                    *(uint32_t *)&s_data[(uint32_t)(it0 + k) * 256u + (uint32_t)lane * 4u] = __builtin_amdgcn_perm(u, t, 0x05040100u);
                }
            }
        }
        const uint32_t ck = ck0 + j * nblk + b;
#if defined(LAB_ENC) && LAB_ENC == 3
        wave_sync();
        if (lane == 0) { ChunkDesc d0; d0.lead = 0; d0.enc_len = s_data[ck & 4095u]; d0.last_end = 0; d0.mcode0 = 0; desc[ck] = d0; }
        continue;
#endif
        DBG_ADD(11, DBG_CLK() - dbg_k0);
        match_chunk<WAYS, MODE>(s_data, 0u, (int)HB_CHUNK, s_out, s_tab, s_q, s_st, desc + ck, records + (size_t)ck * HB_RSTRIDE, true, false, accel, lane, (int)j);
        DBG_ADD(12, DBG_CLK() - dbg_k0); DBG_ADD(13, 1);
        DBG_COMMIT();
    }
}

__device__ __forceinline__ void block_scan_agg(Agg *s, int t) {
    for (int d = 1; d < 256; d <<= 1) {
        Agg x = agg_identity(), y = agg_identity();
        if (t < 256) { x = s[t]; if (t >= d) y = s[t - d]; }
        __syncthreads();
        if (t < 256) s[t] = agg_combine(y, x);
        __syncthreads();
    }
}

__global__ __launch_bounds__(256) void k_tiles(const ChunkDesc *__restrict__ desc, uint32_t nchunks,
                                               Agg *__restrict__ tile_agg, uint32_t *__restrict__ tile_nf,
                                               const BatchFrame *__restrict__ bf, const uint32_t *__restrict__ tile_frame) {
    __shared__ Agg s[256];
    __shared__ uint32_t s_nf[256];
    const int t = threadIdx.x;
    uint32_t ck = blockIdx.x * HB_TILE_CHUNKS + t;
    if (bf) {
        const BatchFrame &f = bf[tile_frame[blockIdx.x]];
        ck = (blockIdx.x - f.tile0) * HB_TILE_CHUNKS + t; nchunks = f.nchunks; desc += f.chunk0;
    }
    Agg a = agg_identity();
    if (ck < nchunks) a = agg_of_chunk(desc[ck], ck * HB_CHUNK);
    s[t] = a;
    s_nf[t] = a.has ? a.F : 0xFFFFFFFFu;
    __syncthreads();
    block_scan_agg(s, t);
    for (int d = 128; d > 0; d >>= 1) {
        if (t < d) s_nf[t] = min(s_nf[t], s_nf[t + d]);
        __syncthreads();
    }
    if (t == 0) { tile_agg[blockIdx.x] = s[255]; tile_nf[blockIdx.x] = s_nf[0]; }
}

struct FrameInfo { int frame, codec, shuffle, typesize; unsigned opts; };

__global__ __launch_bounds__(256) void k_scan(const Agg *__restrict__ tile_agg, const uint32_t *__restrict__ tile_nf,
                                              Agg *__restrict__ tile_pre, uint32_t *__restrict__ tile_suf,
                                              uint32_t ntiles, uint32_t nchunks, uint64_t n, EncPlan *plan,
                                              uint8_t *dst, FrameInfo fi, hb_result *result, int has_index,
                                              const BatchFrame *__restrict__ bf) {
    __shared__ Agg s[256];
    __shared__ uint32_t s_nf[256];
    __shared__ Agg carry;
    __shared__ uint32_t carry_nf;
    const int t = threadIdx.x;
    if (bf) {
        const BatchFrame &f = bf[blockIdx.x];
        tile_agg += f.tile0; tile_nf += f.tile0; tile_pre += f.tile0; tile_suf += f.tile0;
        ntiles = f.ntiles; nchunks = f.nchunks; n = f.n; plan = f.plan; dst = f.dst; result = f.result;
    }
    if (t == 0) { carry = agg_identity(); carry_nf = 0xFFFFFFFFu; }
    __syncthreads();
    for (uint32_t base = 0; base < ntiles; base += 256) {
        const uint32_t i = base + t;
        s[t] = (i < ntiles) ? tile_agg[i] : agg_identity();
        __syncthreads();
        block_scan_agg(s, t);
        const Agg excl = agg_combine(carry, t ? s[t - 1] : agg_identity());
        if (i < ntiles) tile_pre[i] = excl;
        __syncthreads();
        if (t == 0) carry = agg_combine(carry, s[255]);
        __syncthreads();
    }
    for (int64_t base = (int64_t)((ntiles + 255) / 256) * 256 - 256; base >= 0; base -= 256) {
        const uint32_t i = (uint32_t)base + t;
        s_nf[t] = (i < ntiles) ? tile_nf[i] : 0xFFFFFFFFu;
        __syncthreads();
        for (int d = 1; d < 256; d <<= 1) {
            const uint32_t x = s_nf[t], y = (t + d < 256) ? s_nf[t + d] : 0xFFFFFFFFu;
            __syncthreads();
            s_nf[t] = min(x, y);
            __syncthreads();
        }
        const uint32_t excl = min(carry_nf, (t + 1 < 256) ? s_nf[t + 1] : 0xFFFFFFFFu);
        if (i < ntiles) tile_suf[i] = excl;
        __syncthreads();
        if (t == 0) carry_nf = min(carry_nf, s_nf[0]);
        __syncthreads();
    }
    if (t == 0) {
        const Agg all = carry;
        const uint64_t a2 = all.has ? all.E : 0;
        const uint64_t tl = n - a2;
        const uint64_t C = (uint64_t)agg_bytes(all) + 1 + lz4_ext_bytes((uint32_t)tl) + tl;
        plan->cbytes_block = C;
        plan->nchunks = nchunks;
        uint32_t use_memcpy = 0;
        uint64_t payload = C;
        if (fi.frame) {
            use_memcpy = !(fi.opts & HB_OPT_INTERNAL_BLOCK) && C >= n;
            if (use_memcpy) payload = n;
            uint8_t flags = 0;
            if (fi.shuffle == HB_SHUFFLE) flags |= HB_FLAG_SHUFFLE;
            else if (fi.shuffle == HB_BITSHUFFLE) flags |= HB_FLAG_BITSHUFFLE;
            if (use_memcpy) flags |= HB_FLAG_MEMCPY;
            const uint32_t cbytes = (uint32_t)(HB_HEADER_SIZE + payload);
            dst[0] = HB_FORMAT_VERSION; dst[1] = (uint8_t)fi.codec; dst[2] = flags; dst[3] = (uint8_t)fi.typesize;
            ((uint32_t *)dst)[1] = (uint32_t)n; ((uint32_t *)dst)[2] = (uint32_t)n; ((uint32_t *)dst)[3] = cbytes;
            result->flags = flags;
            result->bytes = cbytes;
            uint64_t total = cbytes;
            plan->index_off = 0;
            if (has_index && !use_memcpy) {
                plan->index_off = ((uint64_t)cbytes + 7) & ~7ull;
                total = plan->index_off + HB_IDX_HDR_BYTES + (uint64_t)HB_IDX_ENTRY * (nchunks + 1);
                for (uint64_t i = cbytes; i < plan->index_off; i++) dst[i] = 0;
            }
            result->total_bytes = total;
        } else {
            if (nchunks == 0) dst[0] = 0;
            result->flags = 0;
            result->bytes = C;
            result->total_bytes = C;
            plan->index_off = 0;
        }
        plan->use_memcpy = use_memcpy;
        result->status = HB_OK;
        result->reserved = 0;
    }
}

#ifndef STITCH_NT
#define STITCH_NT 0
#endif
#ifndef STITCH_DEPTH
#define STITCH_DEPTH 0
#endif
#ifndef STITCH_GLOBAL
#define STITCH_GLOBAL 1
#endif
#if STITCH_NT
#define STITCH_COPY wave_copy_g2g_nt
#elif STITCH_DEPTH
#define STITCH_COPY wave_copy_g2g_deep<STITCH_DEPTH, STITCH_GLOBAL != 0>
#else
#define STITCH_COPY wave_copy_g2g
#endif
#define STITCH_THREADS 512
__global__ __launch_bounds__(STITCH_THREADS) void k_stitch(
        const ChunkDesc *__restrict__ desc, const uint8_t *__restrict__ records, const uint8_t *__restrict__ src,
        const Agg *__restrict__ tile_pre, const uint32_t *__restrict__ tile_suf, const EncPlan *__restrict__ plan,
        uint32_t nchunks, uint64_t n, uint8_t *__restrict__ out ,
        uint8_t *__restrict__ index_base_ext, uint8_t *__restrict__ frame_base, const uint8_t *__restrict__ memcpy_src,
        int lit_from_records, const BatchFrame *__restrict__ bf, const uint32_t *__restrict__ tile_frame) {
    __shared__ Agg s[256];
    __shared__ uint32_t s_nf[256];
    __shared__ ChunkDesc s_desc[256];
    const int t = threadIdx.x, lane = t & 63;
#if STITCH_DEPTH
    const int wave = __builtin_amdgcn_readfirstlane(t >> 6);
#else
    const int wave = t >> 6;
#endif
    constexpr int NW = STITCH_THREADS / 64;
    uint32_t tile = blockIdx.x;
    if (bf) {
        const BatchFrame &f = bf[tile_frame[blockIdx.x]];
        tile = blockIdx.x - f.tile0;
        desc += f.chunk0; records += (size_t)f.chunk0 * HB_RSTRIDE; src = f.src; tile_pre += f.tile0; tile_suf += f.tile0;
        plan = f.plan; nchunks = f.nchunks; n = f.n; out = f.dst + HB_HEADER_SIZE; frame_base = f.dst; memcpy_src = f.memcpy_src;
    }
    const uint32_t ck0 = tile * HB_TILE_CHUNKS;
    const uint32_t cnt = min(HB_TILE_CHUNKS, nchunks - ck0);

    if (plan->use_memcpy) {
        const uint64_t b0 = (uint64_t)ck0 * HB_CHUNK;
        const uint64_t b1 = min((uint64_t)(ck0 + cnt) * HB_CHUNK, n);
        for (uint64_t off = b0 + (uint64_t)wave * 16384u; off < b1; off += (uint64_t)NW * 16384u)
            if (memcpy_src) wave_copy_g2g(out + off, memcpy_src + off, (uint32_t)min((uint64_t)16384u, b1 - off), lane);
        return;
    }

    if (t < 256) {
        ChunkDesc d; d.lead = 0; d.enc_len = 0; d.last_end = 0; d.mcode0 = 0;
        if ((uint32_t)t < cnt) d = desc[ck0 + t];
        s_desc[t] = d;
        const Agg mine = ((uint32_t)t < cnt) ? agg_of_chunk(d, (ck0 + t) * HB_CHUNK) : agg_identity();
        s[t] = mine;
        s_nf[t] = mine.has ? mine.F : 0xFFFFFFFFu;
    }
    __syncthreads();
    block_scan_agg(s, t);
    for (int dd = 1; dd < 256; dd <<= 1) {
        uint32_t x = 0, y = 0xFFFFFFFFu;
        if (t < 256) { x = s_nf[t]; if (t + dd < 256) y = s_nf[t + dd]; }
        __syncthreads();
        if (t < 256) s_nf[t] = min(x, y);
        __syncthreads();
    }
    const Agg tpre = tile_pre[tile];
    const uint32_t tsuf = tile_suf[tile];
#define RFL(x) ((uint32_t)__builtin_amdgcn_readfirstlane((int)(x)))
    auto rfl_agg = [](const Agg &x) __attribute__((always_inline)) {
        Agg r;
        r.fixed = (int64_t)(((uint64_t)RFL((uint32_t)((uint64_t)x.fixed >> 32)) << 32) | RFL((uint32_t)(uint64_t)x.fixed));
        r.F = RFL(x.F); r.E = RFL(x.E); r.has = RFL(x.has); r.pad = 0;
        return r;
    };
    uint8_t *index = nullptr;
    if (index_base_ext) index = index_base_ext;
    else if (frame_base && plan->index_off) index = frame_base + plan->index_off;

    for (uint32_t c = wave; c < cnt; c += NW) {
        const uint32_t ck = ck0 + c;
        ChunkDesc cd = s_desc[c];
        cd.lead = RFL(cd.lead); cd.enc_len = RFL(cd.enc_len); cd.last_end = RFL(cd.last_end); cd.mcode0 = RFL(cd.mcode0);
        const uint32_t start = ck * HB_CHUNK;
        const uint32_t end = (uint32_t)min((uint64_t)start + HB_CHUNK, n);
        const Agg P = agg_combine(tpre, c ? rfl_agg(s[c - 1]) : agg_identity());
        uint32_t NF = min(tsuf, (c + 1 < 256) ? RFL(s_nf[c + 1]) : 0xFFFFFFFFu);
        if (NF == 0xFFFFFFFFu) NF = (uint32_t)n;
        const uint32_t a = P.has ? P.E : 0u;
        const uint64_t O = (uint64_t)agg_bytes(P);
        uint64_t I = O;
        uint32_t a2 = a, tpos = start;
        if (cd.last_end) {
            const uint32_t tl = start + cd.lead - a;
            const uint32_t hdr = 1 + lz4_ext_bytes(tl);
            const uint32_t carry_lits = start - a;
            wave_write_lit_header(out + O, tl, cd.mcode0, lane);
            STITCH_COPY(out + O + hdr + carry_lits, records + (size_t)ck * HB_RSTRIDE, cd.enc_len, lane);
            I = O + hdr + carry_lits + cd.enc_len;
            a2 = start + cd.last_end; tpos = a2;
        }
        const uint32_t hdr2 = 1 + lz4_ext_bytes(NF - a2);
        const uint8_t *lsrc = lit_from_records ? records + (size_t)ck * HB_RSTRIDE + (cd.last_end ? cd.enc_len : 0u) : src + tpos;
        STITCH_COPY(out + I + hdr2 + (tpos - a2), lsrc, end - tpos, lane);
        if (ck + 1 == nchunks) wave_write_lit_header(out + I, NF - a2, 0, lane);
        if (index && lane == 0) {
            uint32_t *e = (uint32_t *)(index + HB_IDX_HDR_BYTES) + 4 * (size_t)ck;
            if (ck == 0) { e[0] = 0; e[1] = 0; e[2] = HB_IDX_AT_TOKEN; e[3] = 0; }
            else {
                const uint32_t Fc = cd.last_end ? start + cd.lead : NF;
                const uint32_t hdrc = 1 + lz4_ext_bytes(Fc - a);
                e[0] = (uint32_t)(O + hdrc + (start - a)); e[1] = start; e[2] = Fc - start; e[3] = (uint32_t)O;
            }
            if (ck + 1 == nchunks) {
                e[4] = (uint32_t)plan->cbytes_block; e[5] = (uint32_t)n; e[6] = 0; e[7] = 0;
                uint32_t *h = (uint32_t *)index;
                h[0] = HB_IDX_MAGIC; h[1] = HB_IDX_VERSION | (HB_IDX_ENTRY << 16); h[2] = nchunks; h[3] = HB_CHUNK;
                h[4] = (uint32_t)plan->cbytes_block; h[5] = (uint32_t)n; h[6] = 0;
                h[7] = h[0] ^ h[1] ^ h[2] ^ h[3] ^ h[4] ^ h[5];
            }
        }
    }
}

__device__ __forceinline__ uint32_t uvarint_len(uint64_t v) { uint32_t k = 1; while (v >= 128) { v >>= 7; k++; } return k; }

__global__ __launch_bounds__(256) void k_sn_tiles(const ChunkDesc *__restrict__ desc, uint32_t nchunks, Agg *__restrict__ tile_agg) {
    __shared__ uint32_t s[256];
    const int t = threadIdx.x;
    const uint32_t ck = blockIdx.x * HB_TILE_CHUNKS + t;
    s[t] = ck < nchunks ? desc[ck].enc_len : 0u;
    __syncthreads();
    for (int d = 128; d > 0; d >>= 1) { if (t < d) s[t] += s[t + d]; __syncthreads(); }
    if (t == 0) { Agg a = agg_identity(); a.fixed = s[0]; tile_agg[blockIdx.x] = a; }
}

__global__ __launch_bounds__(256) void k_sn_scan(const Agg *__restrict__ tile_agg, Agg *__restrict__ tile_pre, uint32_t ntiles, uint32_t nchunks,
                                                 uint64_t n, EncPlan *plan, uint8_t *dst, FrameInfo fi, hb_result *result, int has_index) {
    __shared__ uint64_t s[256];
    __shared__ uint64_t carry;
    const int t = threadIdx.x;
    if (t == 0) carry = 0;
    __syncthreads();
    for (uint32_t base = 0; base < ntiles; base += 256) {
        const uint32_t i = base + t;
        const uint64_t mine = i < ntiles ? (uint64_t)tile_agg[i].fixed : 0ull;
        s[t] = mine;
        __syncthreads();
        for (int d = 1; d < 256; d <<= 1) {
            const uint64_t y = t >= d ? s[t - d] : 0ull;
            __syncthreads();
            s[t] += y;
            __syncthreads();
        }
        if (i < ntiles) { Agg a = agg_identity(); a.fixed = (int64_t)(carry + s[t] - mine); tile_pre[i] = a; }
        __syncthreads();
        if (t == 0) carry += s[255];
        __syncthreads();
    }
    if (t == 0) {
        const uint32_t hl = uvarint_len(n);
        const uint64_t C = hl + carry;
        plan->cbytes_block = C;
        plan->nchunks = nchunks;
        const uint32_t use_memcpy = !(fi.opts & HB_OPT_INTERNAL_BLOCK) && C >= n;
        const uint64_t payload = use_memcpy ? n : C;
        uint8_t flags = 0;
        if (fi.shuffle == HB_SHUFFLE) flags |= HB_FLAG_SHUFFLE;
        else if (fi.shuffle == HB_BITSHUFFLE) flags |= HB_FLAG_BITSHUFFLE;
        if (use_memcpy) flags |= HB_FLAG_MEMCPY;
        const uint32_t cbytes = (uint32_t)(HB_HEADER_SIZE + payload);
        dst[0] = HB_FORMAT_VERSION; dst[1] = (uint8_t)fi.codec; dst[2] = flags; dst[3] = (uint8_t)fi.typesize;
        ((uint32_t *)dst)[1] = (uint32_t)n; ((uint32_t *)dst)[2] = (uint32_t)n; ((uint32_t *)dst)[3] = cbytes;
        if (!use_memcpy) {
            uint64_t v = n; uint8_t *o = dst + HB_HEADER_SIZE;
            while (v >= 128) { *o++ = (uint8_t)(v | 128u); v >>= 7; }
            *o = (uint8_t)v;
        }
        result->flags = flags; result->bytes = cbytes;
        uint64_t total = cbytes;
        plan->index_off = 0;
        if (has_index && !use_memcpy) {
            plan->index_off = ((uint64_t)cbytes + 7) & ~7ull;
            total = plan->index_off + HB_SNX_HDR_BYTES + (uint64_t)HB_SNX_ENTRY * (nchunks + 1);
            for (uint64_t i = cbytes; i < plan->index_off; i++) dst[i] = 0;
        }
        result->total_bytes = total;
        plan->use_memcpy = use_memcpy;
        result->status = HB_OK; result->reserved = 0;
    }
}

__global__ __launch_bounds__(STITCH_THREADS) void k_sn_pack(const ChunkDesc *__restrict__ desc, const uint8_t *__restrict__ records,
                                                            const Agg *__restrict__ tile_pre, const EncPlan *__restrict__ plan, uint32_t nchunks,
                                                            uint64_t n, uint8_t *__restrict__ out , uint8_t *__restrict__ frame_base,
                                                            const uint8_t *__restrict__ memcpy_src) {
    __shared__ uint32_t s[256];
    const int t = threadIdx.x, wave = t >> 6, lane = t & 63;
    constexpr int NW = STITCH_THREADS / 64;
    const uint32_t ck0 = blockIdx.x * HB_TILE_CHUNKS;
    const uint32_t cnt = min(HB_TILE_CHUNKS, nchunks - ck0);
    if (plan->use_memcpy) {
        const uint64_t b0 = (uint64_t)ck0 * HB_CHUNK, b1 = min((uint64_t)(ck0 + cnt) * HB_CHUNK, n);
        for (uint64_t off = b0 + (uint64_t)wave * 16384u; off < b1; off += (uint64_t)NW * 16384u)
            if (memcpy_src) wave_copy_g2g(out + off, memcpy_src + off, (uint32_t)min((uint64_t)16384u, b1 - off), lane);
        return;
    }
    uint32_t mine = 0;
    if (t < 256) { mine = (uint32_t)t < cnt ? desc[ck0 + t].enc_len : 0u; s[t] = mine; }
    __syncthreads();
    for (int d = 1; d < 256; d <<= 1) {
        uint32_t y = 0;
        if (t < 256 && t >= d) y = s[t - d];
        __syncthreads();
        if (t < 256) s[t] += y;
        __syncthreads();
    }
    const uint32_t hl = uvarint_len(n);
    const uint64_t tbase = (uint64_t)hl + (uint64_t)tile_pre[blockIdx.x].fixed;
    uint8_t *index = (frame_base && plan->index_off) ? frame_base + plan->index_off : nullptr;
    for (uint32_t c = wave; c < cnt; c += NW) {
        const uint32_t ck = ck0 + c;
        const uint32_t incl = (uint32_t)__builtin_amdgcn_readfirstlane((int)s[c]);
        const uint32_t len = (uint32_t)__builtin_amdgcn_readfirstlane((int)desc[ck].enc_len);
        const uint64_t O = tbase + incl - len;
        STITCH_COPY(out + O, records + (size_t)ck * HB_RSTRIDE, len, lane);
        if (index && lane == 0) {
            uint32_t *e = (uint32_t *)(index + HB_SNX_HDR_BYTES);
            e[ck] = (uint32_t)O;
            if (ck + 1 == nchunks) {
                e[nchunks] = (uint32_t)plan->cbytes_block;
                uint32_t *h = (uint32_t *)index;
                h[0] = HB_SNX_MAGIC; h[1] = HB_IDX_VERSION | (HB_SNX_ENTRY << 16); h[2] = nchunks; h[3] = HB_CHUNK;
                h[4] = (uint32_t)plan->cbytes_block; h[5] = (uint32_t)n; h[6] = hl;
                h[7] = h[0] ^ h[1] ^ h[2] ^ h[3] ^ h[4] ^ h[5] ^ h[6];
            }
        }
    }
}

static inline void enc_policy(const hb_enc_args &a, int &ways, int &accel) {
    const int level = a.level < 1 ? 1 : (a.level > 9 ? 9 : a.level);
    ways = 1; accel = 64;
    if (a.codec == HB_LZ4HC) { ways = level <= 3 ? 1 : (level <= 5 ? 2 : 4); accel = 0; }
    else if (a.codec == HB_LZ4 && a.frame) accel = level <= 3 ? 128 : (level <= 6 ? 64 : 0);
}

#define HB_LAUNCH_FUSED(TS, W, SN) hipLaunchKernelGGL((k_match_fused<TS, W, SN>), dim3(grid), dim3(64), 0, s, a.src, desc, records, nblk, hb_dbg_plane_mask(), accel, bf, chunk_frame, total_items)
static void launch_match_fused(const hb_enc_args &a, unsigned grid, ChunkDesc *desc, uint8_t *records, uint32_t nblk, hipStream_t s,
                               const BatchFrame *bf = nullptr, const uint32_t *chunk_frame = nullptr, uint32_t total_items = 0) {
    int ways, accel;
    enc_policy(a, ways, accel);
    const bool sn = a.codec == HB_SNAPPY;
    switch (a.fused_ts) {
    case 2: if (sn) HB_LAUNCH_FUSED(2, 1, true); else if (ways == 1) HB_LAUNCH_FUSED(2, 1, false); else if (ways == 2) HB_LAUNCH_FUSED(2, 2, false); else HB_LAUNCH_FUSED(2, 4, false); break;
    case 4: if (sn) HB_LAUNCH_FUSED(4, 1, true); else if (ways == 1) HB_LAUNCH_FUSED(4, 1, false); else if (ways == 2) HB_LAUNCH_FUSED(4, 2, false); else HB_LAUNCH_FUSED(4, 4, false); break;
    default: if (sn) HB_LAUNCH_FUSED(8, 1, true); else if (ways == 1) HB_LAUNCH_FUSED(8, 1, false); else if (ways == 2) HB_LAUNCH_FUSED(8, 2, false); else HB_LAUNCH_FUSED(8, 4, false); break;
    }
}
#define HB_LAUNCH_MATCH(W, SN) hipLaunchKernelGGL((k_match<W, SN>), dim3(grid), dim3(64), 0, s, a.src, (uint64_t)a.n, desc, records, nchunks, a.fused_bits, keep_long, accel, bf, chunk_frame)
static void launch_match(const hb_enc_args &a, unsigned grid, ChunkDesc *desc, uint8_t *records, uint32_t nchunks, hipStream_t s,
                         const BatchFrame *bf = nullptr, const uint32_t *chunk_frame = nullptr) {
    int ways, accel;
    enc_policy(a, ways, accel);
    const int keep_long = (a.frame && a.shuffle == HB_SHUFFLE && a.typesize > 1) ? 0 : 1;
    if (a.codec == HB_SNAPPY) HB_LAUNCH_MATCH(1, true);
    else if (ways == 1) HB_LAUNCH_MATCH(1, false);
    else if (ways == 2) HB_LAUNCH_MATCH(2, false);
    else HB_LAUNCH_MATCH(4, false);
}

static inline uint32_t batch_granule(bool fused_ts, int typesize) { return fused_ts ? 8u * (uint32_t)typesize : 1u; }

void hb_launch_match_selfcontained(const uint8_t *src, size_t n, void *desc, uint8_t *records, uint32_t nchunks, int accel, hipStream_t s) {
    const unsigned grid = nchunks < 256u * 256u ? nchunks : 256u * 256u;
    hipLaunchKernelGGL((k_match<1, 2>), dim3(grid), dim3(64), 0, s, src, (uint64_t)n, (ChunkDesc *)desc, records, nchunks, 0, 0, accel, (const BatchFrame *)nullptr, (const uint32_t *)nullptr);
}

bool hb_launch_match_fused_selfcontained(const uint8_t *src, int typesize, void *desc, uint8_t *records, uint32_t nblk, int accel, hipStream_t s) {
    const uint64_t items = (uint64_t)nblk * (uint64_t)typesize;
    const unsigned grid = (unsigned)(items < 256u * 256u ? items : 256u * 256u);
    switch (typesize) {
    case 2: hipLaunchKernelGGL((k_match_fused<2, 1, 2>), dim3(grid), dim3(64), 0, s, src, (ChunkDesc *)desc, records, nblk, 0xFFFFFFFFu, accel, (const BatchFrame *)nullptr, (const uint32_t *)nullptr, 0u); return true;
    case 4: hipLaunchKernelGGL((k_match_fused<4, 1, 2>), dim3(grid), dim3(64), 0, s, src, (ChunkDesc *)desc, records, nblk, 0xFFFFFFFFu, accel, (const BatchFrame *)nullptr, (const uint32_t *)nullptr, 0u); return true;
    case 8: hipLaunchKernelGGL((k_match_fused<8, 1, 2>), dim3(grid), dim3(64), 0, s, src, (ChunkDesc *)desc, records, nblk, 0xFFFFFFFFu, accel, (const BatchFrame *)nullptr, (const uint32_t *)nullptr, 0u); return true;
    default: return false;
    }
}

void hb_launch_match_selfcontained_batch(const BatchFrame *bf, const uint32_t *chunk_frame, void *desc, uint8_t *records, uint32_t total_chunks, int accel, hipStream_t s) {
    const unsigned grid = total_chunks < 256u * 256u ? total_chunks : 256u * 256u;
    hipLaunchKernelGGL((k_match<1, 2>), dim3(grid), dim3(64), 0, s, (const uint8_t *)nullptr, (uint64_t)0, (ChunkDesc *)desc, records, total_chunks, 0, 0, accel, bf, chunk_frame);
}
bool hb_launch_match_fused_selfcontained_batch(const BatchFrame *bf, const uint32_t *chunk_frame, int typesize, void *desc, uint8_t *records, uint32_t total_items, int accel,
                                               hipStream_t s) {
    if (typesize != 2 && typesize != 4 && typesize != 8) return false;
    const uint32_t granule = batch_granule(true, typesize);
    unsigned grid = total_items < 256u * 256u ? total_items : 256u * 256u;
    if (total_items > 256u * 16u) {
        grid = total_items / (unsigned)typesize / granule * granule;
        if (total_items > 256u * 64u && grid < 256u * 64u) grid = 256u * 64u;
        if (grid > 256u * 256u) grid = 256u * 256u;
        if (grid == 0) grid = total_items;
    }
    switch (typesize) {
    case 2: hipLaunchKernelGGL((k_match_fused<2, 1, 2>), dim3(grid), dim3(64), 0, s, (const uint8_t *)nullptr, (ChunkDesc *)desc, records, 0u, 0xFFFFFFFFu, accel, bf, chunk_frame, total_items); break;
    case 4: hipLaunchKernelGGL((k_match_fused<4, 1, 2>), dim3(grid), dim3(64), 0, s, (const uint8_t *)nullptr, (ChunkDesc *)desc, records, 0u, 0xFFFFFFFFu, accel, bf, chunk_frame, total_items); break;
    default: hipLaunchKernelGGL((k_match_fused<8, 1, 2>), dim3(grid), dim3(64), 0, s, (const uint8_t *)nullptr, (ChunkDesc *)desc, records, 0u, 0xFFFFFFFFu, accel, bf, chunk_frame, total_items); break;
    }
    return true;
}

int hb_launch_lz4_encode(const hb_enc_args &a, hipStream_t s) {
    const EncLayout L = enc_layout(a.n);
    uint8_t *w = a.work;
    EncPlan *plan = (EncPlan *)(w + L.plan);
    ChunkDesc *desc = (ChunkDesc *)(w + L.desc);
    Agg *tile_agg = (Agg *)(w + L.tile_agg), *tile_pre = (Agg *)(w + L.tile_pre);
    uint32_t *tile_nf = (uint32_t *)(w + L.tile_nf), *tile_suf = (uint32_t *)(w + L.tile_suf);
    uint8_t *records = w + L.records;
    uint8_t *out = a.frame ? a.dst + HB_HEADER_SIZE : a.dst;
    FrameInfo fi{a.frame, a.codec, a.shuffle, a.typesize, a.opts};
    const int has_index = a.frame ? ((a.opts & HB_OPT_INDEX_TRAILER) ? 1 : 0) : (a.index ? 1 : 0);

    if (L.nchunks) {
        hb_prof_begin(a.fused_ts ? "k_match_fused" : "k_match", s);
        if (a.fused_ts) {
            const uint32_t nblk = L.nchunks / (uint32_t)a.fused_ts;
            unsigned grid = L.nchunks;
            if (grid > 256u * 16u) {
                const unsigned gran = 8u * (unsigned)a.fused_ts;
                grid = nblk / gran * gran;
                if (L.nchunks > 256u * 64u && grid < 256u * 64u) grid = 256u * 64u;
                if (grid > 256u * 256u) grid = 256u * 256u;
                if (grid == 0) grid = L.nchunks;
            }
            launch_match_fused(a, grid, desc, records, nblk, s);
        } else {
            const unsigned grid = L.nchunks < 256u * 256u ? L.nchunks : 256u * 256u;
            launch_match(a, grid, desc, records, L.nchunks, s);
        }
        hb_prof_end(s);
        if (a.codec == HB_SNAPPY) {
            hb_prof_begin("k_sn_tiles", s);
            hipLaunchKernelGGL(k_sn_tiles, dim3(L.ntiles), dim3(256), 0, s, desc, L.nchunks, tile_agg);
            hb_prof_end(s);
        } else {
            hb_prof_begin("k_tiles", s);
            hipLaunchKernelGGL(k_tiles, dim3(L.ntiles), dim3(256), 0, s, desc, L.nchunks, tile_agg, tile_nf, (const BatchFrame *)nullptr, (const uint32_t *)nullptr);
            hb_prof_end(s);
        }
    }
    if (a.codec == HB_SNAPPY) {
        hb_prof_begin("k_sn_scan", s);
        hipLaunchKernelGGL(k_sn_scan, dim3(1), dim3(256), 0, s, tile_agg, tile_pre, L.ntiles, L.nchunks, (uint64_t)a.n, plan, a.dst, fi, a.result, has_index);
        hb_prof_end(s);
        if ((a.fused_ts || a.fused_bits) && !a.memcpy_src) {
            const int rc = hb_launch_filter_gated(a.fused_bits ? HB_OP_BITSHUFFLE : HB_OP_SHUFFLE, out, a.src, a.n, a.fused_bits ? a.fused_bits : a.fused_ts, &plan->use_memcpy, s);
            if (rc) return rc;
        }
        hb_prof_begin("k_sn_pack", s);
        hipLaunchKernelGGL(k_sn_pack, dim3(L.ntiles), dim3(STITCH_THREADS), 0, s, desc, records, tile_pre, plan, L.nchunks, (uint64_t)a.n, out, a.dst, a.memcpy_src);
        hb_prof_end(s);
        HB_HIP_TRY(hipGetLastError());
        return HB_OK;
    }
    hb_prof_begin("k_scan", s);
    hipLaunchKernelGGL(k_scan, dim3(1), dim3(256), 0, s, tile_agg, tile_nf, tile_pre, tile_suf, L.ntiles, L.nchunks,
                       (uint64_t)a.n, plan, a.dst, fi, a.result, has_index, (const BatchFrame *)nullptr);
    hb_prof_end(s);
    if ((a.fused_ts || a.fused_bits) && !a.memcpy_src) {
        const int rc = hb_launch_filter_gated(a.fused_bits ? HB_OP_BITSHUFFLE : HB_OP_SHUFFLE, out, a.src, a.n, a.fused_bits ? a.fused_bits : a.fused_ts, &plan->use_memcpy, s);
        if (rc) return rc;
    }
    if (L.nchunks) {
        hb_prof_begin("k_stitch", s);
        hipLaunchKernelGGL(k_stitch, dim3(L.ntiles), dim3(STITCH_THREADS), 0, s, desc, records, a.src, tile_pre, tile_suf,
                           plan, L.nchunks, (uint64_t)a.n, out, a.frame ? (uint8_t *)nullptr : a.index,
                           a.frame ? a.dst : (uint8_t *)nullptr, a.memcpy_src, (a.fused_ts || a.fused_bits) ? 1 : 0,
                           (const BatchFrame *)nullptr, (const uint32_t *)nullptr);
        hb_prof_end(s);
    }
    HB_HIP_TRY(hipGetLastError());
    return HB_OK;
}

struct EncBatchLayout {
    size_t frames, plans, jobs, chunk_frame, tile_frame, desc, tile_agg, tile_nf, tile_pre, tile_suf, records, filtered, total;
    uint32_t total_chunks, total_tiles;
};

static EncBatchLayout enc_batch_layout(int nframes, const size_t *n, uint32_t granule, bool need_filtered) {
    EncBatchLayout L{};
    uint64_t chunks = 0, tiles = 0, fbytes = 0;
    for (int k = 0; k < nframes; k++) {
        const uint64_t c = (n[k] + HB_CHUNK - 1) / HB_CHUNK;
        chunks = (chunks + granule - 1) / granule * granule + c;
        tiles += (c + HB_TILE_CHUNKS - 1) / HB_TILE_CHUNKS;
        fbytes += (n[k] + 255) & ~(size_t)255;
    }
    L.total_chunks = (uint32_t)chunks; L.total_tiles = (uint32_t)tiles;
    size_t o = 0;
    auto take = [&](size_t bytes) { size_t at = o; o += (bytes + 255) & ~(size_t)255; return at; };
    L.frames = take((size_t)nframes * sizeof(BatchFrame));
    L.plans = take((size_t)nframes * sizeof(EncPlan));
    L.jobs = take((size_t)nframes * sizeof(hb_filter_job) * 2);
    L.chunk_frame = take((size_t)chunks * 4 + 4);
    L.tile_frame = take((size_t)tiles * 4 + 4);
    L.desc = take((size_t)chunks * sizeof(ChunkDesc));
    L.tile_agg = take((size_t)tiles * sizeof(Agg));
    L.tile_nf = take((size_t)tiles * 4);
    L.tile_pre = take((size_t)tiles * sizeof(Agg));
    L.tile_suf = take((size_t)tiles * 4);
    L.records = take((size_t)chunks * HB_RSTRIDE + 256);
    L.filtered = take(need_filtered ? fbytes + 256 : 0);
    L.total = o;
    return L;
}
size_t hb_lz4_enc_batch_workspace(int nframes, const size_t *n, int typesize) {
    if (nframes <= 0 || !n) return 256;
    const size_t a = enc_batch_layout(nframes, n, batch_granule(true, typesize > 0 && typesize <= 8 ? typesize : 8), false).total;
    const size_t b = enc_batch_layout(nframes, n, 1u, true).total;
    return a > b ? a : b;
}

__global__ __launch_bounds__(64) void k_bt_map(const BatchFrame *__restrict__ bf, uint32_t nframes, uint32_t *__restrict__ chunk_frame, uint32_t *__restrict__ tile_frame,
                                               uint32_t total_chunks) {
    const uint32_t f = blockIdx.x;
    const BatchFrame b = bf[f];
    const uint32_t next = f + 1 < nframes ? bf[f + 1].chunk0 : total_chunks;
    for (uint32_t c = threadIdx.x; c < next - b.chunk0; c += 64) chunk_frame[b.chunk0 + c] = c < b.nchunks ? f : 0xFFFFFFFFu;
    for (uint32_t t = threadIdx.x; t < b.ntiles; t += 64) tile_frame[b.tile0 + t] = f;
}

int hb_launch_lz4_encode_batch(int nframes, const hb_batch_frame *fr, int codec, int level, int shuffle, int typesize, unsigned opts,
                               uint8_t *work, size_t work_bytes, hipStream_t s) {
    if (nframes <= 0) return HB_OK;
    if (codec != HB_LZ4 && codec != HB_LZ4HC) return HB_ERR_INVALID_CODEC;
    const bool filt = (shuffle == HB_SHUFFLE || shuffle == HB_BITSHUFFLE) && typesize > 1;
    bool fused = filt && shuffle == HB_SHUFFLE && (typesize == 2 || typesize == 4 || typesize == 8) && !(opts & HB_OPT_NO_FUSION);
    bool fused_bits = filt && shuffle == HB_BITSHUFFLE && typesize == 4 && !(opts & HB_OPT_NO_FUSION);
    size_t max_n = 0;
    std::vector<size_t> ns((size_t)nframes);
    for (int k = 0; k < nframes; k++) {
        ns[(size_t)k] = fr[k].n;
        max_n = fr[k].n > max_n ? fr[k].n : max_n;
        if (fused && fr[k].n % ((size_t)typesize * HB_CHUNK) != 0) fused = false;
        if (fused_bits && (fr[k].n % 32 != 0 || ((uintptr_t)fr[k].src & 15u))) fused_bits = false;
    }
    const uint32_t granule = batch_granule(fused, typesize);
    const bool need_filtered = filt && !fused && !fused_bits;
    const EncBatchLayout L = enc_batch_layout(nframes, ns.data(), granule, need_filtered);
    if (work_bytes < L.total) return HB_ERR_SHORT_BUFFER;
    BatchFrame *d_bf = (BatchFrame *)(work + L.frames);
    EncPlan *d_plans = (EncPlan *)(work + L.plans);
    hb_filter_job *d_jobs = (hb_filter_job *)(work + L.jobs);
    uint32_t *chunk_frame = (uint32_t *)(work + L.chunk_frame), *tile_frame = (uint32_t *)(work + L.tile_frame);
    ChunkDesc *desc = (ChunkDesc *)(work + L.desc);
    Agg *tile_agg = (Agg *)(work + L.tile_agg), *tile_pre = (Agg *)(work + L.tile_pre);
    uint32_t *tile_nf = (uint32_t *)(work + L.tile_nf), *tile_suf = (uint32_t *)(work + L.tile_suf);
    uint8_t *records = work + L.records, *filtered = work + L.filtered;

    std::vector<BatchFrame> h((size_t)nframes);
    std::vector<hb_filter_job> jobs((size_t)nframes * 2);
    uint64_t chunks = 0, tiles = 0, foff = 0;
    for (int k = 0; k < nframes; k++) {
        const size_t n = fr[k].n;
        const uint32_t c = (uint32_t)((n + HB_CHUNK - 1) / HB_CHUNK);
        chunks = (chunks + granule - 1) / granule * granule;
        BatchFrame &b = h[(size_t)k];
        const bool f_filt = filt && n >= (size_t)typesize;
        const uint8_t *in = fr[k].src;
        if (need_filtered && f_filt) in = filtered + foff;
        b.src = (fused || fused_bits) ? fr[k].src : in;
        b.dst = fr[k].dst;
        b.memcpy_src = (opts & HB_OPT_REFERENCE_MEMCPY) ? fr[k].src : ((fused || fused_bits) ? nullptr : in);
        b.result = fr[k].result;
        b.plan = d_plans + k;
        b.n = n;
        b.chunk0 = (uint32_t)chunks; b.nchunks = c;
        b.tile0 = (uint32_t)tiles; b.ntiles = (c + HB_TILE_CHUNKS - 1) / HB_TILE_CHUNKS;
        b.nblk = fused ? c / (uint32_t)typesize : 0u; b.pad = 0;
        jobs[(size_t)k] = hb_filter_job{filtered + foff, fr[k].src, (need_filtered && f_filt) ? (uint64_t)n : 0ull, nullptr};
        jobs[(size_t)(nframes + k)] = hb_filter_job{fr[k].dst + HB_HEADER_SIZE, fr[k].src, ((fused || fused_bits) && !b.memcpy_src) ? (uint64_t)n : 0ull, &(d_plans + k)->use_memcpy};
        chunks += c; tiles += b.ntiles; foff += (n + 255) & ~(size_t)255;
    }
    HB_HIP_TRY(hipMemcpyAsync(d_bf, h.data(), h.size() * sizeof(BatchFrame), hipMemcpyHostToDevice, s));
    HB_HIP_TRY(hipMemcpyAsync(d_jobs, jobs.data(), jobs.size() * sizeof(hb_filter_job), hipMemcpyHostToDevice, s));
    hipLaunchKernelGGL(k_bt_map, dim3((unsigned)nframes), dim3(64), 0, s, d_bf, (uint32_t)nframes, chunk_frame, tile_frame, L.total_chunks);
    if (need_filtered) {
        hb_prof_begin(shuffle == HB_SHUFFLE ? "filter_shuffle" : "filter_bitshuffle", s);
        const int rc = hb_launch_filter_batch(shuffle == HB_SHUFFLE ? HB_OP_SHUFFLE : HB_OP_BITSHUFFLE, d_jobs, nframes, max_n, typesize, s);
        hb_prof_end(s);
        if (rc) return rc;
    }
    hb_enc_args a{};
    a.frame = 1; a.codec = codec; a.shuffle = shuffle; a.typesize = typesize; a.opts = opts; a.level = level;
    a.fused_ts = fused ? typesize : 0; a.fused_bits = fused_bits ? 4 : 0;
    FrameInfo fi{1, codec, shuffle, typesize, opts};
    const int has_index = (opts & HB_OPT_INDEX_TRAILER) ? 1 : 0;
    unsigned grid = L.total_chunks < 256u * 256u ? L.total_chunks : 256u * 256u;
    if (fused && L.total_chunks > 256u * 16u) {
        grid = L.total_chunks / (unsigned)typesize / granule * granule;
        if (L.total_chunks > 256u * 64u && grid < 256u * 64u) grid = 256u * 64u;
        if (grid > 256u * 256u) grid = 256u * 256u;
        if (grid == 0) grid = L.total_chunks;
    }
    hb_prof_begin(fused ? "k_match_fused" : "k_match", s);
    if (fused) launch_match_fused(a, grid, desc, records, 0u, s, d_bf, chunk_frame, L.total_chunks);
    else launch_match(a, grid, desc, records, L.total_chunks, s, d_bf, chunk_frame);
    hb_prof_end(s);
    hb_prof_begin("k_tiles", s);
    hipLaunchKernelGGL(k_tiles, dim3(L.total_tiles), dim3(256), 0, s, desc, 0u, tile_agg, tile_nf, (const BatchFrame *)d_bf, (const uint32_t *)tile_frame);
    hb_prof_end(s);
    hb_prof_begin("k_scan", s);
    hipLaunchKernelGGL(k_scan, dim3((unsigned)nframes), dim3(256), 0, s, tile_agg, tile_nf, tile_pre, tile_suf, 0u, 0u, (uint64_t)0, (EncPlan *)nullptr,
                       (uint8_t *)nullptr, fi, (hb_result *)nullptr, has_index, (const BatchFrame *)d_bf);
    hb_prof_end(s);
    if (fused || fused_bits) {
        const int rc = hb_launch_filter_batch(fused_bits ? HB_OP_BITSHUFFLE : HB_OP_SHUFFLE, d_jobs + nframes, nframes, max_n, typesize, s, 1);
        if (rc) return rc;
    }
    hb_prof_begin("k_stitch", s);
    hipLaunchKernelGGL(k_stitch, dim3(L.total_tiles), dim3(STITCH_THREADS), 0, s, desc, records, (const uint8_t *)nullptr, tile_pre, tile_suf,
                       (const EncPlan *)nullptr, 0u, (uint64_t)0, (uint8_t *)nullptr, (uint8_t *)nullptr, (uint8_t *)nullptr, (const uint8_t *)nullptr,
                       (fused || fused_bits) ? 1 : 0, (const BatchFrame *)d_bf, (const uint32_t *)tile_frame);
    hb_prof_end(s);
    HB_HIP_TRY(hipGetLastError());
    return HB_OK;
}
```

Before: 398.3 GB/s.

## Fold tile scan into k_tiles via ticket counter and drop decode prefetch path

The separate k_scan launch goes away on the encode path. k_tiles now finishes the cross-tile scan itself: a ticket counter in EncPlan lets the last tile do the scan. The per-tile block scan is rewritten with wave shuffles in place of the shared-memory Hillis-Steele loop. In the decoder, the unused DEC_PREFETCH machinery (DecPre, uniform loads, the pf_issue/pf_commit hooks) is removed. This saves one kernel launch and a single-block serial scan, but adds an atomic last-block pattern whose correctness depends on memory ordering.

```diff
diff --git a/go-blosc_amd/csrc/hb_dec_unit.h b/go-blosc_amd/csrc/hb_dec_unit.h
--- a/go-blosc_amd/csrc/hb_dec_unit.h
+++ b/go-blosc_amd/csrc/hb_dec_unit.h
@@ -51,61 +51,22 @@
     uint32_t nbytes, nunits;
     int bun4, ush;
 };
-#ifndef DEC_PREFETCH
-#define DEC_PREFETCH 0
-#endif
 #ifndef DEC_STAGE_DEPTH
 #define DEC_STAGE_DEPTH 4
 #endif
 #define DEC_NO_UNIT 0xFFFFFFFFu
-struct DecPre {
-    uint32_t u;
-    uint32_t e[8];
-    uint32_t win;
-};
-typedef const __attribute__((address_space(4))) uint32_t *dec_cu32p;
-__device__ __forceinline__ void dec_ld_uniform16(const uint8_t *p, uint32_t *o) {
-    const uintptr_t a = (uintptr_t)p;
-    const dec_cu32p q = (dec_cu32p)(a & ~(uintptr_t)3);
-    const uint32_t sh = ((uint32_t)a & 3u) * 8u;
-    const uint32_t w0 = q[0], w1 = q[1], w2 = q[2], w3 = q[3];
-    uint32_t w4 = w3;
-    if (sh != 0u) w4 = q[4];
-    const uint32_t r0 = sh ? (uint32_t)((((uint64_t)w1 << 32) | w0) >> sh) : w0, r1 = sh ? (uint32_t)((((uint64_t)w2 << 32) | w1) >> sh) : w1;
-    const uint32_t r2 = sh ? (uint32_t)((((uint64_t)w3 << 32) | w2) >> sh) : w2, r3 = sh ? (uint32_t)((((uint64_t)w4 << 32) | w3) >> sh) : w3;
-    o[0] = (uint32_t)__builtin_amdgcn_readfirstlane((int)r0); o[1] = (uint32_t)__builtin_amdgcn_readfirstlane((int)r1);
-    o[2] = (uint32_t)__builtin_amdgcn_readfirstlane((int)r2); o[3] = (uint32_t)__builtin_amdgcn_readfirstlane((int)r3);
-}
-__device__ __forceinline__ uint32_t dec_ld_uniform1(const uint8_t *p) {
-    const uintptr_t a = (uintptr_t)p;
-    return (uint32_t)__builtin_amdgcn_readfirstlane((int)((*(dec_cu32p)(a & ~(uintptr_t)3) >> (((uint32_t)a & 3u) * 8u)) & 255u));
-}
-
-template <int USH, class F>
-__device__ __forceinline__ void dec_flush_ush(uint8_t *udst, const uint8_t *s_out, const uint32_t outlen, const int lane, const uint32_t ush_rt, F &&after) {
+
+template <int USH>
+__device__ __forceinline__ void dec_flush_ush(uint8_t *udst, const uint8_t *s_out, const uint32_t outlen, const int lane, const uint32_t ush_rt) {
 #if defined(LAB_DEC_FLUSH) && LAB_DEC_FLUSH == 1
-    after();
 #elif defined(LAB_DEC_FLUSH) && LAB_DEC_FLUSH == 2
     for (uint32_t i = lane * 16u; i < outlen; i += 1024u) st16u(udst + i, *(const u32x4 *)(s_out + i));
-    after();
 #else
     const uint32_t ush = USH > 0 ? (uint32_t)USH : ush_rt;
     constexpr uint32_t G = USH == 4 ? 8u : 16u;
     const uint32_t step = 64u * ush;
     uint8_t *p = udst + (uint32_t)lane * ush;
     const uint8_t *q = s_out + lane;
-#if DEC_PREFETCH
-    if (USH > 0 && outlen == DEC_OUT_MAX) {
-#pragma unroll
-        for (uint32_t g = 0; g < DEC_OUT_MAX / (64u * G); g++) {
-#pragma unroll
-            for (uint32_t k = 0; k < G; k++) p[k * step] = q[64u * k];
-            p += G * step; q += 64u * G;
-        }
-        after();
-        return;
-    }
-#endif
     uint32_t i = 0;
     for (; i + 64u * G <= outlen; i += 64u * G) {
 #pragma unroll
@@ -113,35 +74,18 @@
         p += G * step; q += 64u * G;
     }
     for (i += (uint32_t)lane; i < outlen; i += 64u) { *p = *q; p += step; q += 64; }
-    after();
 #endif
 }
 template <int USH, int BUN4>
-__device__ __forceinline__ void dec_unit(const DecCtx &c, const uint32_t u, uint8_t *s_in, uint8_t *s_out, uint2 *s_tq, const int lane,
-                                         const uint32_t u_next, DecPre &pre) {
+__device__ __forceinline__ void dec_unit(const DecCtx &c, const uint32_t u, uint8_t *s_in, uint8_t *s_out, uint2 *s_tq, const int lane) {
     const uint8_t *const src = c.src; const uint64_t n_src = c.n_src; uint8_t *const dst = c.dst; const uint8_t *const ent = c.ent;
     DecPlan *const plan = c.plan; const uint32_t nbytes = c.nbytes, nunits = c.nunits;
     const int bun4 = BUN4 < 0 ? c.bun4 : BUN4, ush = USH < 0 ? c.ush : USH;
 #define RFL(x) ((uint32_t)__builtin_amdgcn_readfirstlane((int)(x)))
-#if DEC_PREFETCH
-#define DEC_LD_BYTE(p) dec_ld_uniform1(p)
-    uint32_t e[8];
-    const bool have = pre.u == u;
-    const bool staged0 = have && pre.win != 0u;
-    if (have) { for (int k = 0; k < 8; k++) e[k] = pre.e[k]; }
-    else { dec_ld_uniform16(ent + 16 * (size_t)u, e); dec_ld_uniform16(ent + 16 * (size_t)(u + 1), e + 4); }
-    pre.u = DEC_NO_UNIT; pre.win = 0u;
-    const uint32_t s0 = e[0], d0 = e[1], s1 = e[4], d1 = e[5], rem1 = e[6], tok1 = e[7];
-    uint32_t rem = e[2], tokpos = e[3];
-    uint32_t en[8];
-    if (u_next != DEC_NO_UNIT) { dec_ld_uniform16(ent + 16 * (size_t)u_next, en); dec_ld_uniform16(ent + 16 * (size_t)(u_next + 1u), en + 4); }
-#else
 #define DEC_LD_BYTE(p) RFL((uint32_t)*(p))
-    const bool staged0 = false;
     const u32x4 e0 = ld16u(ent + 16 * (size_t)u), e1 = ld16u(ent + 16 * (size_t)(u + 1));
     const uint32_t s0 = RFL(e0.x), d0 = RFL(e0.y), s1 = RFL(e1.x), d1 = RFL(e1.y), rem1 = RFL(e1.z), tok1 = RFL(e1.w);
     uint32_t rem = RFL(e0.z), tokpos = RFL(e0.w);
-#endif
     const bool last = (u + 1 == nunits);
     bool ok = s0 <= s1 && s1 <= n_src && d0 <= d1 && d1 <= nbytes && (d1 - d0) <= DEC_OUT_MAX;
     if (u == 0) ok = ok && s0 == 0 && d0 == 0 && rem == HB_IDX_AT_TOKEN;
@@ -155,35 +99,6 @@
     if (!ok) { if (lane == 0) atomicExch(&plan->fail, 1u); return; }
     const uint32_t slen = s1 - s0, outlen = d1 - d0;
     const uint8_t *g = src + s0;
-    u32x4 pv0 = {0u, 0u, 0u, 0u}, pv1 = {0u, 0u, 0u, 0u};
-    uint32_t pnv = 0;
-    auto pf_issue = [&]() __attribute__((always_inline)) {
-#if DEC_PREFETCH
-        if (u_next == DEC_NO_UNIT) return;
-        pre.u = u_next;
-        for (int k = 0; k < 8; k++) pre.e[k] = en[k];
-        const uint32_t ns0 = en[0], nd0 = en[1], nrem = en[2], ns1 = en[4], nd1 = en[5];
-        if (!(ns0 <= ns1 && ns1 <= n_src && nd0 <= nd1 && nd1 <= nbytes && (nd1 - nd0) <= DEC_OUT_MAX)) return;
-        if (nrem != HB_IDX_AT_TOKEN && nrem >= nd1 - nd0) return;
-        const uint8_t *ng = src + ns0;
-        const uint32_t nsh = (uint32_t)((uintptr_t)ng & 15u);
-        const uint32_t avail = nsh + (ns1 - ns0);
-        pnv = ((avail < DEC_IN_WIN ? avail : DEC_IN_WIN) + 15u) >> 4;
-        const u32x4 *ga = (const u32x4 *)(ng - nsh);
-        if ((uint32_t)lane < pnv) pv0 = ga[lane];
-        if ((uint32_t)lane + 64u < pnv) pv1 = ga[lane + 64];
-#endif
-    };
-    auto pf_commit = [&]() __attribute__((always_inline)) {
-#if DEC_PREFETCH
-        if (pnv == 0u) return;
-        wave_sync();
-        if ((uint32_t)lane < pnv) ((u32x4 *)s_in)[lane] = pv0;
-        if ((uint32_t)lane + 64u < pnv) ((u32x4 *)s_in)[lane + 64] = pv1;
-        pre.win = 1u;
-        wave_sync();
-#endif
-    };
 
     if (rem != HB_IDX_AT_TOKEN && rem >= outlen) {
         const uint32_t left = rem - outlen;
@@ -215,12 +130,10 @@
             }
 #endif
             wave_sync();
-            pf_issue();
-            dec_flush_ush<USH>(udst, s_out, outlen, lane, (uint32_t)ush, pf_commit);
+            dec_flush_ush<USH>(udst, s_out, outlen, lane, (uint32_t)ush);
             wave_sync();
             return;
         }
-        pf_issue();
         if (!bun4) wave_copy_g2g(dst + d0, g, outlen, lane);
         else {
             for (uint32_t w = lane; w < outlen / 32u; w += 64) {
@@ -230,14 +143,13 @@
                 st16u(dst + d0 + 32u * w + 16u, ob);
             }
         }
-        pf_commit();
         return;
     }
 
     const uint32_t sh = (uint32_t)((uintptr_t)g & 15u);
     uint32_t wlo = 0, staged = 0;
     int shw = 0;
-    auto stage = [&](const uint32_t at, const bool there = false) __attribute__((always_inline)) {
+    auto stage = [&](const uint32_t at) __attribute__((always_inline)) {
         wave_sync();
         const uint32_t a16 = (sh + at) & ~15u;
         const uint32_t avail = sh + slen - a16;
@@ -245,7 +157,7 @@
         const u32x4 *ga = (const u32x4 *)(g - sh + a16);
         const uint32_t nv = (cnt + 15u) >> 4;
 #if DEC_STAGE_DEPTH > 1
-        if (!there) {
+        {
             constexpr int SV = (int)(((DEC_IN_WIN + 15u) / 16u + 63u) / 64u);
             static_assert(SV <= 4, "stage(): four vectors per lane");
             const u32x4 *gl = ga + lane; u32x4 *sl = (u32x4 *)s_in + lane;
@@ -261,20 +173,20 @@
             if (SV > 3 && ul + 192u < nv) sl[192] = a3;
         }
 #else
-        if (!there) for (uint32_t i = lane; i < nv; i += 64) ((u32x4 *)s_in)[i] = ga[i];
+        for (uint32_t i = lane; i < nv; i += 64) ((u32x4 *)s_in)[i] = ga[i];
 #endif
         wlo = a16 > sh ? a16 - sh : 0u;
         staged = a16 + cnt - sh;
         shw = (int)sh - (int)a16;
         wave_sync();
     };
-#if DEC_STAGE_DEPTH > 1 && !DEC_PREFETCH
+#if DEC_STAGE_DEPTH > 1
     uint32_t tokv = 0;
     if (rem != HB_IDX_AT_TOKEN) tokv = (uint32_t)src[tokpos];
-    stage(0u, staged0);
+    stage(0u);
     uint32_t tok = RFL(tokv);
 #else
-    stage(0u, staged0);
+    stage(0u);
     uint32_t tok = 0;
     if (rem != HB_IDX_AT_TOKEN) tok = DEC_LD_BYTE(src + tokpos);
 #endif
@@ -353,7 +265,6 @@
     }
     if (!ok) { if (lane == 0) atomicExch(&plan->fail, 1u); wave_sync(); return; }
     wave_sync();
-    pf_issue();
     if (bun4) {
         for (uint32_t w = lane; w < outlen / 32u; w += 64) {
             u32x4 oa, ob;
@@ -364,7 +275,7 @@
         wave_sync();
     }
     if (ush) {
-        dec_flush_ush<USH>(udst, s_out, outlen, lane, (uint32_t)ush, pf_commit);
+        dec_flush_ush<USH>(udst, s_out, outlen, lane, (uint32_t)ush);
     } else {
         uint8_t *o = dst + d0;
         uint32_t head = (uint32_t)((16u - ((uintptr_t)o & 15u)) & 15u);
@@ -385,7 +296,6 @@
         }
         const uint32_t done_b = head + body * 16u;
         if (done_b + lane < outlen) o[done_b + lane] = s_out[done_b + lane];
-        pf_commit();
     }
     wave_sync();
 }
diff --git a/go-blosc_amd/csrc/hb_getitem.hip b/go-blosc_amd/csrc/hb_getitem.hip
--- a/go-blosc_amd/csrc/hb_getitem.hip
+++ b/go-blosc_amd/csrc/hb_getitem.hip
@@ -47,8 +47,7 @@
     if (!ok) { if (lane == 0) atomicExch(&plan->fail, 1u); return; }
     DecCtx c; c.src = src; c.n_src = n_src; c.ent = ent; c.plan = plan; c.nbytes = g.nbytes; c.nunits = nunits; c.bun4 = 0; c.ush = 0;
     c.dst = (uint8_t *)((uintptr_t)stage + ((size_t)j * g.upp + k) * HB_CHUNK - (size_t)HB_CHUNK * u);
-    DecPre pre; pre.u = DEC_NO_UNIT; pre.win = 0u;
-    dec_unit<0, 0>(c, u, s_in, s_out, s_tq, lane, DEC_NO_UNIT, pre);
+    dec_unit<0, 0>(c, u, s_in, s_out, s_tq, lane);
 }
 
 __global__ __launch_bounds__(64) __attribute__((amdgpu_waves_per_eu(DEC_WAVES))) void k_gi_units(const uint8_t *__restrict__ src, uint64_t n_src,
diff --git a/go-blosc_amd/csrc/hb_lz4_dec.hip b/go-blosc_amd/csrc/hb_lz4_dec.hip
--- a/go-blosc_amd/csrc/hb_lz4_dec.hip
+++ b/go-blosc_amd/csrc/hb_lz4_dec.hip
@@ -44,12 +44,10 @@
         return u;
     };
     DecCtx c; c.src = src; c.n_src = n_src; c.dst = dst; c.ent = ent; c.plan = plan; c.nbytes = nbytes; c.nunits = nunits; c.bun4 = bun4; c.ush = ush;
-    DecPre pre; pre.u = DEC_NO_UNIT; pre.win = 0u;
     for (uint32_t it = blockIdx.x; it < mgrp * 8u; it += gridDim.x) {
         const uint32_t u = unit_of(it);
         if (u == DEC_NO_UNIT) continue;
-        const uint32_t u_next = DEC_PREFETCH ? unit_of(it + gridDim.x) : DEC_NO_UNIT;
-        dec_unit<USH, BUN4>(c, u, s_in, s_out, s_tq, lane, u_next, pre);
+        dec_unit<USH, BUN4>(c, u, s_in, s_out, s_tq, lane);
     }
 }
 
@@ -90,8 +88,7 @@
             u = j * nblk + b;
         }
         if (u >= c.nunits) continue;
-        DecPre pre; pre.u = DEC_NO_UNIT; pre.win = 0u;
-        dec_unit<-1, -1>(c, u, s_in, s_out, s_tq, lane, DEC_NO_UNIT, pre);
+        dec_unit<-1, -1>(c, u, s_in, s_out, s_tq, lane);
     }
 }
 
diff --git a/go-blosc_amd/csrc/hb_lz4_enc.hip b/go-blosc_amd/csrc/hb_lz4_enc.hip
--- a/go-blosc_amd/csrc/hb_lz4_enc.hip
+++ b/go-blosc_amd/csrc/hb_lz4_enc.hip
@@ -56,8 +56,11 @@
     uint32_t use_memcpy;
     uint32_t nchunks;
     uint64_t index_off;
-    uint64_t pad[4];
+    uint32_t ticket;
+    uint32_t sub[7];
 };
+#define ENC_NSUB 7u
+static_assert(sizeof(EncPlan) == 56, "EncPlan: the workspace layouts keep their size");
 
 
 struct EncLayout {
@@ -723,7 +726,7 @@
 __global__ __launch_bounds__(64) void k_match(const uint8_t *__restrict__ src_, uint64_t n_,
                                               ChunkDesc *__restrict__ desc, uint8_t *__restrict__ records,
                                               uint32_t nchunks, int bits4, int keep_long, int accel,
-                                              const BatchFrame *__restrict__ bf, const uint32_t *__restrict__ chunk_frame) {
+                                              const BatchFrame *__restrict__ bf, const uint32_t *__restrict__ chunk_frame, uint32_t *ticket) {
     __shared__ __attribute__((aligned(16))) uint8_t s_data[HB_CHUNK + 112];
     __shared__ __attribute__((aligned(16))) uint8_t s_out[SOUT + 16];
     __shared__ __attribute__((aligned(16))) uint16_t s_tab[HSIZEW(WAYS) * WAYS + 8];
@@ -731,6 +734,7 @@
     uint2 *const s_q = (uint2 *)(s_out + 16);
     uint32_t *const s_st = (uint32_t *)(s_data + HB_CHUNK + 80);
     const int lane = threadIdx.x;
+    if (ticket && blockIdx.x == 0 && lane == 0) { for (int k = 0; k < 8; k++) ticket[k] = 0u; }
     for (uint32_t ck = blockIdx.x; ck < nchunks; ck += gridDim.x) {
         const uint8_t *src = src_;
         uint64_t n = n_, start = (uint64_t)ck * HB_CHUNK;
@@ -762,7 +766,7 @@
 template <int TS, int WAYS, int MODE>
 __global__ __launch_bounds__(64) __attribute__((amdgpu_waves_per_eu(WAYS == 1 ? ENC_WAVES : 4))) void k_match_fused(const uint8_t *__restrict__ src_, ChunkDesc *__restrict__ desc,
                                                     uint8_t *__restrict__ records, uint32_t nblk_, uint32_t plane_mask, int accel,
-                                                    const BatchFrame *__restrict__ bf, const uint32_t *__restrict__ chunk_frame, uint32_t total_) {
+                                                    const BatchFrame *__restrict__ bf, const uint32_t *__restrict__ chunk_frame, uint32_t total_, uint32_t *ticket) {
     __shared__ __attribute__((aligned(16))) uint8_t s_data[HB_CHUNK + 112];
     __shared__ __attribute__((aligned(16))) uint8_t s_out[SOUT + 16];
     __shared__ __attribute__((aligned(16))) uint16_t s_tab[HSIZEW(WAYS) * WAYS + 8];
@@ -771,6 +775,7 @@
     uint32_t *const s_st = (uint32_t *)(s_data + HB_CHUNK + 80);
     const int lane = threadIdx.x;
     const uint32_t total = bf ? total_ : nblk_ * TS;
+    if (ticket && blockIdx.x == 0 && lane == 0) { for (int k = 0; k < 8; k++) ticket[k] = 0u; }
     for (uint32_t gi = blockIdx.x; gi < total; gi += gridDim.x) {
         const uint8_t *src = src_;
         uint32_t nblk = nblk_, i = gi, ck0 = 0;
@@ -850,126 +855,153 @@
     }
 }
 
-__device__ __forceinline__ void block_scan_agg(Agg *s, int t) {
-    for (int d = 1; d < 256; d <<= 1) {
-        Agg x = agg_identity(), y = agg_identity();
-        if (t < 256) { x = s[t]; if (t >= d) y = s[t - d]; }
-        __syncthreads();
-        if (t < 256) s[t] = agg_combine(y, x);
-        __syncthreads();
-    }
+struct BlockScan {
+    Agg incl, excl, total;
+    uint32_t smin_incl, smin_excl, smin_total;
+};
+__device__ __forceinline__ Agg agg_shfl_up(const Agg &a, int d) {
+    Agg r;
+    const uint32_t lo = __shfl_up((uint32_t)(uint64_t)a.fixed, d), hi = __shfl_up((uint32_t)((uint64_t)a.fixed >> 32), d);
+    r.fixed = (int64_t)(((uint64_t)hi << 32) | lo);
+    r.F = __shfl_up(a.F, d); r.E = __shfl_up(a.E, d); r.has = __shfl_up(a.has, d); r.pad = 0;
+    return r;
+}
+template <bool AGG, bool NF>
+__device__ __forceinline__ BlockScan block_scan_ordered(Agg a, uint32_t nf, Agg *s_w, uint32_t *s_wn, int t) {
+    const int lane = t & 63, w = t >> 6;
+#pragma unroll
+    for (int d = 1; d < 64; d <<= 1) {
+        if (AGG) { const Agg y = agg_shfl_up(a, d); if (lane >= d) a = agg_combine(y, a); }
+        if (NF) { const uint32_t m = __shfl_down(nf, d); if (lane + d < 64) nf = min(nf, m); }
+    }
+    Agg ex = agg_identity(); uint32_t mx = 0xFFFFFFFFu;
+    if (AGG) { const Agg y = agg_shfl_up(a, 1); if (lane) ex = y; }
+    if (NF) { const uint32_t m = __shfl_down(nf, 1); if (lane < 63) mx = m; }
+    if (w < 4) {
+        if (AGG && lane == 63) s_w[w] = a;
+        if (NF && lane == 0) s_wn[w] = nf;
+    }
+    __syncthreads();
+    BlockScan r;
+    Agg p = agg_identity(), tot = agg_identity(); uint32_t m = 0xFFFFFFFFu, mt = 0xFFFFFFFFu;
+#pragma unroll
+    for (int k = 0; k < 4; k++) {
+        if (AGG) { const Agg x = s_w[k]; if (k < w) p = agg_combine(p, x); tot = agg_combine(tot, x); }
+        if (NF) { const uint32_t x = s_wn[k]; if (k > w) m = min(m, x); mt = min(mt, x); }
+    }
+    r.incl = agg_combine(p, a); r.excl = agg_combine(p, ex); r.total = tot;
+    r.smin_incl = min(nf, m); r.smin_excl = min(mx, m); r.smin_total = mt;
+    return r;
+}
+
+struct FrameInfo { int frame, codec, shuffle, typesize; unsigned opts; };
+
+__device__ __forceinline__ void scan_finish(const Agg &all, uint32_t nchunks, uint64_t n, EncPlan *plan, uint8_t *dst, const FrameInfo &fi,
+                                            hb_result *result, int has_index) {
+    const uint64_t a2 = all.has ? all.E : 0;
+    const uint64_t tl = n - a2;
+    const uint64_t C = (uint64_t)agg_bytes(all) + 1 + lz4_ext_bytes((uint32_t)tl) + tl;
+    plan->cbytes_block = C;
+    plan->nchunks = nchunks;
+    uint32_t use_memcpy = 0;
+    uint64_t payload = C;
+    if (fi.frame) {
+        use_memcpy = !(fi.opts & HB_OPT_INTERNAL_BLOCK) && C >= n;
+        if (use_memcpy) payload = n;
+        uint8_t flags = 0;
+        if (fi.shuffle == HB_SHUFFLE) flags |= HB_FLAG_SHUFFLE;
+        else if (fi.shuffle == HB_BITSHUFFLE) flags |= HB_FLAG_BITSHUFFLE;
+        if (use_memcpy) flags |= HB_FLAG_MEMCPY;
+        const uint32_t cbytes = (uint32_t)(HB_HEADER_SIZE + payload);
+        dst[0] = HB_FORMAT_VERSION; dst[1] = (uint8_t)fi.codec; dst[2] = flags; dst[3] = (uint8_t)fi.typesize;
+        ((uint32_t *)dst)[1] = (uint32_t)n; ((uint32_t *)dst)[2] = (uint32_t)n; ((uint32_t *)dst)[3] = cbytes;
+        result->flags = flags;
+        result->bytes = cbytes;
+        uint64_t total = cbytes;
+        plan->index_off = 0;
+        if (has_index && !use_memcpy) {
+            plan->index_off = ((uint64_t)cbytes + 7) & ~7ull;
+            total = plan->index_off + HB_IDX_HDR_BYTES + (uint64_t)HB_IDX_ENTRY * (nchunks + 1);
+            for (uint64_t i = cbytes; i < plan->index_off; i++) dst[i] = 0;
+        }
+        result->total_bytes = total;
+    } else {
+        if (nchunks == 0) dst[0] = 0;
+        result->flags = 0;
+        result->bytes = C;
+        result->total_bytes = C;
+        plan->index_off = 0;
+    }
+    plan->use_memcpy = use_memcpy;
+    result->status = HB_OK;
+    result->reserved = 0;
+}
+
+__device__ __forceinline__ void scan_frame(const Agg *tile_agg, const uint32_t *tile_nf, Agg *tile_pre, uint32_t *tile_suf, uint32_t ntiles, uint32_t nchunks,
+                                           uint64_t n, EncPlan *plan, uint8_t *dst, const FrameInfo &fi, hb_result *result, int has_index,
+                                           Agg *s_w, uint32_t *s_wn, uint32_t round, int t) {
+    const uint32_t R = (ntiles + 255u) / 256u;
+    Agg carry = agg_identity();
+    uint32_t carry_nf = 0xFFFFFFFFu;
+    auto ld_agg = [&](uint32_t r) __attribute__((always_inline)) { const uint32_t i = 256u * r + t; return i < ntiles ? tile_agg[i] : agg_identity(); };
+    auto ld_nf = [&](uint32_t r) __attribute__((always_inline)) { const uint32_t i = 256u * (R - 1u - r) + t; return i < ntiles ? tile_nf[i] : 0xFFFFFFFFu; };
+    Agg na = agg_identity(); uint32_t nn = 0xFFFFFFFFu;
+    if (R) { na = ld_agg(0u); nn = ld_nf(0u); }
+    for (uint32_t r = 0; r < R; r++, round ^= 1u) {
+        const Agg a = na; const uint32_t nf = nn;
+        if (r + 1u < R) { na = ld_agg(r + 1u); nn = ld_nf(r + 1u); }
+        const BlockScan bs = block_scan_ordered<true, true>(a, nf, s_w + 4u * round, s_wn + 4u * round, t);
+        const uint32_t i = 256u * r + t, j = 256u * (R - 1u - r) + t;
+        if (i < ntiles) tile_pre[i] = agg_combine(carry, bs.excl);
+        if (j < ntiles) tile_suf[j] = min(carry_nf, bs.smin_excl);
+        carry = agg_combine(carry, bs.total);
+        carry_nf = min(carry_nf, bs.smin_total);
+    }
+    if (t == 0) scan_finish(carry, nchunks, n, plan, dst, fi, result, has_index);
 }
 
 __global__ __launch_bounds__(256) void k_tiles(const ChunkDesc *__restrict__ desc, uint32_t nchunks,
-                                               Agg *__restrict__ tile_agg, uint32_t *__restrict__ tile_nf,
+                                               Agg *tile_agg, uint32_t *tile_nf, Agg *tile_pre, uint32_t *tile_suf,
+                                               uint32_t ntiles, uint64_t n, EncPlan *plan, uint8_t *dst, FrameInfo fi, hb_result *result, int has_index,
                                                const BatchFrame *__restrict__ bf, const uint32_t *__restrict__ tile_frame) {
-    __shared__ Agg s[256];
-    __shared__ uint32_t s_nf[256];
+    __shared__ Agg s_w[8];
+    __shared__ uint32_t s_wn[8];
+    __shared__ uint32_t s_last;
     const int t = threadIdx.x;
-    uint32_t ck = blockIdx.x * HB_TILE_CHUNKS + t;
+    uint32_t tile = blockIdx.x;
     if (bf) {
         const BatchFrame &f = bf[tile_frame[blockIdx.x]];
-        ck = (blockIdx.x - f.tile0) * HB_TILE_CHUNKS + t; nchunks = f.nchunks; desc += f.chunk0;
-    }
+        tile = blockIdx.x - f.tile0; nchunks = f.nchunks; desc += f.chunk0;
+        tile_agg += f.tile0; tile_nf += f.tile0; tile_pre += f.tile0; tile_suf += f.tile0;
+        ntiles = f.ntiles; n = f.n; plan = f.plan; dst = f.dst; result = f.result;
+    }
+    const uint32_t ck = tile * HB_TILE_CHUNKS + t;
     Agg a = agg_identity();
     if (ck < nchunks) a = agg_of_chunk(desc[ck], ck * HB_CHUNK);
-    s[t] = a;
-    s_nf[t] = a.has ? a.F : 0xFFFFFFFFu;
+    const BlockScan r = block_scan_ordered<true, true>(a, a.has ? a.F : 0xFFFFFFFFu, s_w, s_wn, t);
+    if (t == 0) {
+        unsigned long long *o = (unsigned long long *)(tile_agg + tile);
+        __hip_atomic_store(o + 0, (unsigned long long)r.total.fixed, __ATOMIC_RELAXED, __HIP_MEMORY_SCOPE_AGENT);
+        __hip_atomic_store(o + 1, ((unsigned long long)r.total.E << 32) | r.total.F, __ATOMIC_RELAXED, __HIP_MEMORY_SCOPE_AGENT);
+        __hip_atomic_store(o + 2, (unsigned long long)r.total.has, __ATOMIC_RELAXED, __HIP_MEMORY_SCOPE_AGENT);
+        __hip_atomic_store(tile_nf + tile, r.smin_total, __ATOMIC_RELAXED, __HIP_MEMORY_SCOPE_AGENT);
+        asm volatile("s_waitcnt vmcnt(0)" ::: "memory");
+        const uint32_t cls = tile % ENC_NSUB, ncls = (ntiles - cls + ENC_NSUB - 1u) / ENC_NSUB;
+        uint32_t last = __hip_atomic_fetch_add(&plan->sub[cls], 1u, __ATOMIC_RELAXED, __HIP_MEMORY_SCOPE_AGENT) + 1u == ncls ? 1u : 0u;
+        if (last) last = __hip_atomic_fetch_add(&plan->ticket, 1u, __ATOMIC_RELAXED, __HIP_MEMORY_SCOPE_AGENT) + 1u == min(ntiles, ENC_NSUB) ? 1u : 0u;
+        if (last) {
+            __builtin_amdgcn_fence(__ATOMIC_ACQUIRE, "agent");
+            asm volatile("s_waitcnt vmcnt(0)" ::: "memory");
+        }
+        s_last = last;
+    }
     __syncthreads();
-    block_scan_agg(s, t);
-    for (int d = 128; d > 0; d >>= 1) {
-        if (t < d) s_nf[t] = min(s_nf[t], s_nf[t + d]);
-        __syncthreads();
-    }
-    if (t == 0) { tile_agg[blockIdx.x] = s[255]; tile_nf[blockIdx.x] = s_nf[0]; }
-}
-
-struct FrameInfo { int frame, codec, shuffle, typesize; unsigned opts; };
-
-__global__ __launch_bounds__(256) void k_scan(const Agg *__restrict__ tile_agg, const uint32_t *__restrict__ tile_nf,
-                                              Agg *__restrict__ tile_pre, uint32_t *__restrict__ tile_suf,
-                                              uint32_t ntiles, uint32_t nchunks, uint64_t n, EncPlan *plan,
-                                              uint8_t *dst, FrameInfo fi, hb_result *result, int has_index,
-                                              const BatchFrame *__restrict__ bf) {
-    __shared__ Agg s[256];
-    __shared__ uint32_t s_nf[256];
-    __shared__ Agg carry;
-    __shared__ uint32_t carry_nf;
-    const int t = threadIdx.x;
-    if (bf) {
-        const BatchFrame &f = bf[blockIdx.x];
-        tile_agg += f.tile0; tile_nf += f.tile0; tile_pre += f.tile0; tile_suf += f.tile0;
-        ntiles = f.ntiles; nchunks = f.nchunks; n = f.n; plan = f.plan; dst = f.dst; result = f.result;
-    }
-    if (t == 0) { carry = agg_identity(); carry_nf = 0xFFFFFFFFu; }
-    __syncthreads();
-    for (uint32_t base = 0; base < ntiles; base += 256) {
-        const uint32_t i = base + t;
-        s[t] = (i < ntiles) ? tile_agg[i] : agg_identity();
-        __syncthreads();
-        block_scan_agg(s, t);
-        const Agg excl = agg_combine(carry, t ? s[t - 1] : agg_identity());
-        if (i < ntiles) tile_pre[i] = excl;
-        __syncthreads();
-        if (t == 0) carry = agg_combine(carry, s[255]);
-        __syncthreads();
-    }
-    for (int64_t base = (int64_t)((ntiles + 255) / 256) * 256 - 256; base >= 0; base -= 256) {
-        const uint32_t i = (uint32_t)base + t;
-        s_nf[t] = (i < ntiles) ? tile_nf[i] : 0xFFFFFFFFu;
-        __syncthreads();
-        for (int d = 1; d < 256; d <<= 1) {
-            const uint32_t x = s_nf[t], y = (t + d < 256) ? s_nf[t + d] : 0xFFFFFFFFu;
-            __syncthreads();
-            s_nf[t] = min(x, y);
-            __syncthreads();
-        }
-        const uint32_t excl = min(carry_nf, (t + 1 < 256) ? s_nf[t + 1] : 0xFFFFFFFFu);
-        if (i < ntiles) tile_suf[i] = excl;
-        __syncthreads();
-        if (t == 0) carry_nf = min(carry_nf, s_nf[0]);
-        __syncthreads();
-    }
-    if (t == 0) {
-        const Agg all = carry;
-        const uint64_t a2 = all.has ? all.E : 0;
-        const uint64_t tl = n - a2;
-        const uint64_t C = (uint64_t)agg_bytes(all) + 1 + lz4_ext_bytes((uint32_t)tl) + tl;
-        plan->cbytes_block = C;
-        plan->nchunks = nchunks;
-        uint32_t use_memcpy = 0;
-        uint64_t payload = C;
-        if (fi.frame) {
-            use_memcpy = !(fi.opts & HB_OPT_INTERNAL_BLOCK) && C >= n;
-            if (use_memcpy) payload = n;
-            uint8_t flags = 0;
-            if (fi.shuffle == HB_SHUFFLE) flags |= HB_FLAG_SHUFFLE;
-            else if (fi.shuffle == HB_BITSHUFFLE) flags |= HB_FLAG_BITSHUFFLE;
-            if (use_memcpy) flags |= HB_FLAG_MEMCPY;
-            const uint32_t cbytes = (uint32_t)(HB_HEADER_SIZE + payload);
-            dst[0] = HB_FORMAT_VERSION; dst[1] = (uint8_t)fi.codec; dst[2] = flags; dst[3] = (uint8_t)fi.typesize;
-            ((uint32_t *)dst)[1] = (uint32_t)n; ((uint32_t *)dst)[2] = (uint32_t)n; ((uint32_t *)dst)[3] = cbytes;
-            result->flags = flags;
-            result->bytes = cbytes;
-            uint64_t total = cbytes;
-            plan->index_off = 0;
-            if (has_index && !use_memcpy) {
-                plan->index_off = ((uint64_t)cbytes + 7) & ~7ull;
-                total = plan->index_off + HB_IDX_HDR_BYTES + (uint64_t)HB_IDX_ENTRY * (nchunks + 1);
-                for (uint64_t i = cbytes; i < plan->index_off; i++) dst[i] = 0;
-            }
-            result->total_bytes = total;
-        } else {
-            if (nchunks == 0) dst[0] = 0;
-            result->flags = 0;
-            result->bytes = C;
-            result->total_bytes = C;
-            plan->index_off = 0;
-        }
-        plan->use_memcpy = use_memcpy;
-        result->status = HB_OK;
-        result->reserved = 0;
-    }
+    if (!s_last) return;
+    scan_frame(tile_agg, tile_nf, tile_pre, tile_suf, ntiles, nchunks, n, plan, dst, fi, result, has_index, s_w, s_wn, 1u, t);
+}
+
+__global__ void k_scan(EncPlan *plan, uint8_t *dst, FrameInfo fi, hb_result *result, int has_index) {
+    scan_finish(agg_identity(), 0u, 0u, plan, dst, fi, result, has_index);
 }
 
 #ifndef STITCH_NT
@@ -998,6 +1030,8 @@
     __shared__ Agg s[256];
     __shared__ uint32_t s_nf[256];
     __shared__ ChunkDesc s_desc[256];
+    __shared__ Agg s_w[4];
+    __shared__ uint32_t s_wn[4];
     const int t = threadIdx.x, lane = t & 63;
 #if STITCH_DEPTH
     const int wave = __builtin_amdgcn_readfirstlane(t >> 6);
@@ -1023,23 +1057,16 @@
         return;
     }
 
+    Agg mine = agg_identity();
     if (t < 256) {
         ChunkDesc d; d.lead = 0; d.enc_len = 0; d.last_end = 0; d.mcode0 = 0;
         if ((uint32_t)t < cnt) d = desc[ck0 + t];
         s_desc[t] = d;
-        const Agg mine = ((uint32_t)t < cnt) ? agg_of_chunk(d, (ck0 + t) * HB_CHUNK) : agg_identity();
-        s[t] = mine;
-        s_nf[t] = mine.has ? mine.F : 0xFFFFFFFFu;
-    }
+        if ((uint32_t)t < cnt) mine = agg_of_chunk(d, (ck0 + t) * HB_CHUNK);
+    }
+    const BlockScan bs = block_scan_ordered<true, true>(mine, mine.has ? mine.F : 0xFFFFFFFFu, s_w, s_wn, t);
+    if (t < 256) { s[t] = bs.incl; s_nf[t] = bs.smin_incl; }
     __syncthreads();
-    block_scan_agg(s, t);
-    for (int dd = 1; dd < 256; dd <<= 1) {
-        uint32_t x = 0, y = 0xFFFFFFFFu;
-        if (t < 256) { x = s_nf[t]; if (t + dd < 256) y = s_nf[t + dd]; }
-        __syncthreads();
-        if (t < 256) s_nf[t] = min(x, y);
-        __syncthreads();
-    }
     const Agg tpre = tile_pre[tile];
     const uint32_t tsuf = tile_suf[tile];
 #define RFL(x) ((uint32_t)__builtin_amdgcn_readfirstlane((int)(x)))
@@ -1221,8 +1248,8 @@
     else if (a.codec == HB_LZ4 && a.frame) accel = level <= 3 ? 128 : (level <= 6 ? 64 : 0);
 }
 
-#define HB_LAUNCH_FUSED(TS, W, SN) hipLaunchKernelGGL((k_match_fused<TS, W, SN>), dim3(grid), dim3(64), 0, s, a.src, desc, records, nblk, hb_dbg_plane_mask(), accel, bf, chunk_frame, total_items)
-static void launch_match_fused(const hb_enc_args &a, unsigned grid, ChunkDesc *desc, uint8_t *records, uint32_t nblk, hipStream_t s,
+#define HB_LAUNCH_FUSED(TS, W, SN) hipLaunchKernelGGL((k_match_fused<TS, W, SN>), dim3(grid), dim3(64), 0, s, a.src, desc, records, nblk, hb_dbg_plane_mask(), accel, bf, chunk_frame, total_items, ticket)
+static void launch_match_fused(const hb_enc_args &a, unsigned grid, ChunkDesc *desc, uint8_t *records, uint32_t nblk, hipStream_t s, uint32_t *ticket,
                                const BatchFrame *bf = nullptr, const uint32_t *chunk_frame = nullptr, uint32_t total_items = 0) {
     int ways, accel;
     enc_policy(a, ways, accel);
@@ -1233,8 +1260,8 @@
     default: if (sn) HB_LAUNCH_FUSED(8, 1, true); else if (ways == 1) HB_LAUNCH_FUSED(8, 1, false); else if (ways == 2) HB_LAUNCH_FUSED(8, 2, false); else HB_LAUNCH_FUSED(8, 4, false); break;
     }
 }
-#define HB_LAUNCH_MATCH(W, SN) hipLaunchKernelGGL((k_match<W, SN>), dim3(grid), dim3(64), 0, s, a.src, (uint64_t)a.n, desc, records, nchunks, a.fused_bits, keep_long, accel, bf, chunk_frame)
-static void launch_match(const hb_enc_args &a, unsigned grid, ChunkDesc *desc, uint8_t *records, uint32_t nchunks, hipStream_t s,
+#define HB_LAUNCH_MATCH(W, SN) hipLaunchKernelGGL((k_match<W, SN>), dim3(grid), dim3(64), 0, s, a.src, (uint64_t)a.n, desc, records, nchunks, a.fused_bits, keep_long, accel, bf, chunk_frame, ticket)
+static void launch_match(const hb_enc_args &a, unsigned grid, ChunkDesc *desc, uint8_t *records, uint32_t nchunks, hipStream_t s, uint32_t *ticket,
                          const BatchFrame *bf = nullptr, const uint32_t *chunk_frame = nullptr) {
     int ways, accel;
     enc_policy(a, ways, accel);
@@ -1249,23 +1276,23 @@
 
 void hb_launch_match_selfcontained(const uint8_t *src, size_t n, void *desc, uint8_t *records, uint32_t nchunks, int accel, hipStream_t s) {
     const unsigned grid = nchunks < 256u * 256u ? nchunks : 256u * 256u;
-    hipLaunchKernelGGL((k_match<1, 2>), dim3(grid), dim3(64), 0, s, src, (uint64_t)n, (ChunkDesc *)desc, records, nchunks, 0, 0, accel, (const BatchFrame *)nullptr, (const uint32_t *)nullptr);
+    hipLaunchKernelGGL((k_match<1, 2>), dim3(grid), dim3(64), 0, s, src, (uint64_t)n, (ChunkDesc *)desc, records, nchunks, 0, 0, accel, (const BatchFrame *)nullptr, (const uint32_t *)nullptr, (uint32_t *)nullptr);
 }
 
 bool hb_launch_match_fused_selfcontained(const uint8_t *src, int typesize, void *desc, uint8_t *records, uint32_t nblk, int accel, hipStream_t s) {
     const uint64_t items = (uint64_t)nblk * (uint64_t)typesize;
     const unsigned grid = (unsigned)(items < 256u * 256u ? items : 256u * 256u);
     switch (typesize) {
-    case 2: hipLaunchKernelGGL((k_match_fused<2, 1, 2>), dim3(grid), dim3(64), 0, s, src, (ChunkDesc *)desc, records, nblk, 0xFFFFFFFFu, accel, (const BatchFrame *)nullptr, (const uint32_t *)nullptr, 0u); return true;
-    case 4: hipLaunchKernelGGL((k_match_fused<4, 1, 2>), dim3(grid), dim3(64), 0, s, src, (ChunkDesc *)desc, records, nblk, 0xFFFFFFFFu, accel, (const BatchFrame *)nullptr, (const uint32_t *)nullptr, 0u); return true;
-    case 8: hipLaunchKernelGGL((k_match_fused<8, 1, 2>), dim3(grid), dim3(64), 0, s, src, (ChunkDesc *)desc, records, nblk, 0xFFFFFFFFu, accel, (const BatchFrame *)nullptr, (const uint32_t *)nullptr, 0u); return true;
+    case 2: hipLaunchKernelGGL((k_match_fused<2, 1, 2>), dim3(grid), dim3(64), 0, s, src, (ChunkDesc *)desc, records, nblk, 0xFFFFFFFFu, accel, (const BatchFrame *)nullptr, (const uint32_t *)nullptr, 0u, (uint32_t *)nullptr); return true;
+    case 4: hipLaunchKernelGGL((k_match_fused<4, 1, 2>), dim3(grid), dim3(64), 0, s, src, (ChunkDesc *)desc, records, nblk, 0xFFFFFFFFu, accel, (const BatchFrame *)nullptr, (const uint32_t *)nullptr, 0u, (uint32_t *)nullptr); return true;
+    case 8: hipLaunchKernelGGL((k_match_fused<8, 1, 2>), dim3(grid), dim3(64), 0, s, src, (ChunkDesc *)desc, records, nblk, 0xFFFFFFFFu, accel, (const BatchFrame *)nullptr, (const uint32_t *)nullptr, 0u, (uint32_t *)nullptr); return true;
     default: return false;
     }
 }
 
 void hb_launch_match_selfcontained_batch(const BatchFrame *bf, const uint32_t *chunk_frame, void *desc, uint8_t *records, uint32_t total_chunks, int accel, hipStream_t s) {
     const unsigned grid = total_chunks < 256u * 256u ? total_chunks : 256u * 256u;
-    hipLaunchKernelGGL((k_match<1, 2>), dim3(grid), dim3(64), 0, s, (const uint8_t *)nullptr, (uint64_t)0, (ChunkDesc *)desc, records, total_chunks, 0, 0, accel, bf, chunk_frame);
+    hipLaunchKernelGGL((k_match<1, 2>), dim3(grid), dim3(64), 0, s, (const uint8_t *)nullptr, (uint64_t)0, (ChunkDesc *)desc, records, total_chunks, 0, 0, accel, bf, chunk_frame, (uint32_t *)nullptr);
 }
 bool hb_launch_match_fused_selfcontained_batch(const BatchFrame *bf, const uint32_t *chunk_frame, int typesize, void *desc, uint8_t *records, uint32_t total_items, int accel,
                                                hipStream_t s) {
@@ -1279,9 +1306,9 @@
         if (grid == 0) grid = total_items;
     }
     switch (typesize) {
-    case 2: hipLaunchKernelGGL((k_match_fused<2, 1, 2>), dim3(grid), dim3(64), 0, s, (const uint8_t *)nullptr, (ChunkDesc *)desc, records, 0u, 0xFFFFFFFFu, accel, bf, chunk_frame, total_items); break;
-    case 4: hipLaunchKernelGGL((k_match_fused<4, 1, 2>), dim3(grid), dim3(64), 0, s, (const uint8_t *)nullptr, (ChunkDesc *)desc, records, 0u, 0xFFFFFFFFu, accel, bf, chunk_frame, total_items); break;
-    default: hipLaunchKernelGGL((k_match_fused<8, 1, 2>), dim3(grid), dim3(64), 0, s, (const uint8_t *)nullptr, (ChunkDesc *)desc, records, 0u, 0xFFFFFFFFu, accel, bf, chunk_frame, total_items); break;
+    case 2: hipLaunchKernelGGL((k_match_fused<2, 1, 2>), dim3(grid), dim3(64), 0, s, (const uint8_t *)nullptr, (ChunkDesc *)desc, records, 0u, 0xFFFFFFFFu, accel, bf, chunk_frame, total_items, (uint32_t *)nullptr); break;
+    case 4: hipLaunchKernelGGL((k_match_fused<4, 1, 2>), dim3(grid), dim3(64), 0, s, (const uint8_t *)nullptr, (ChunkDesc *)desc, records, 0u, 0xFFFFFFFFu, accel, bf, chunk_frame, total_items, (uint32_t *)nullptr); break;
+    default: hipLaunchKernelGGL((k_match_fused<8, 1, 2>), dim3(grid), dim3(64), 0, s, (const uint8_t *)nullptr, (ChunkDesc *)desc, records, 0u, 0xFFFFFFFFu, accel, bf, chunk_frame, total_items, (uint32_t *)nullptr); break;
     }
     return true;
 }
@@ -1310,10 +1337,10 @@
                 if (grid > 256u * 256u) grid = 256u * 256u;
                 if (grid == 0) grid = L.nchunks;
             }
-            launch_match_fused(a, grid, desc, records, nblk, s);
+            launch_match_fused(a, grid, desc, records, nblk, s, &plan->ticket);
         } else {
             const unsigned grid = L.nchunks < 256u * 256u ? L.nchunks : 256u * 256u;
-            launch_match(a, grid, desc, records, L.nchunks, s);
+            launch_match(a, grid, desc, records, L.nchunks, s, &plan->ticket);
         }
         hb_prof_end(s);
         if (a.codec == HB_SNAPPY) {
@@ -1322,7 +1349,8 @@
             hb_prof_end(s);
         } else {
             hb_prof_begin("k_tiles", s);
-            hipLaunchKernelGGL(k_tiles, dim3(L.ntiles), dim3(256), 0, s, desc, L.nchunks, tile_agg, tile_nf, (const BatchFrame *)nullptr, (const uint32_t *)nullptr);
+            hipLaunchKernelGGL(k_tiles, dim3(L.ntiles), dim3(256), 0, s, desc, L.nchunks, tile_agg, tile_nf, tile_pre, tile_suf, L.ntiles, (uint64_t)a.n, plan, a.dst, fi,
+                               a.result, has_index, (const BatchFrame *)nullptr, (const uint32_t *)nullptr);
             hb_prof_end(s);
         }
     }
@@ -1340,10 +1368,11 @@
         HB_HIP_TRY(hipGetLastError());
         return HB_OK;
     }
-    hb_prof_begin("k_scan", s);
-    hipLaunchKernelGGL(k_scan, dim3(1), dim3(256), 0, s, tile_agg, tile_nf, tile_pre, tile_suf, L.ntiles, L.nchunks,
-                       (uint64_t)a.n, plan, a.dst, fi, a.result, has_index, (const BatchFrame *)nullptr);
-    hb_prof_end(s);
+    if (!L.nchunks) {
+        hb_prof_begin("k_scan", s);
+        hipLaunchKernelGGL(k_scan, dim3(1), dim3(1), 0, s, plan, a.dst, fi, a.result, has_index);
+        hb_prof_end(s);
+    }
     if ((a.fused_ts || a.fused_bits) && !a.memcpy_src) {
         const int rc = hb_launch_filter_gated(a.fused_bits ? HB_OP_BITSHUFFLE : HB_OP_SHUFFLE, out, a.src, a.n, a.fused_bits ? a.fused_bits : a.fused_ts, &plan->use_memcpy, s);
         if (rc) return rc;
@@ -1403,6 +1432,7 @@
                                                uint32_t total_chunks) {
     const uint32_t f = blockIdx.x;
     const BatchFrame b = bf[f];
+    if (threadIdx.x < 8) (&b.plan->ticket)[threadIdx.x] = 0u;
     const uint32_t next = f + 1 < nframes ? bf[f + 1].chunk0 : total_chunks;
     for (uint32_t c = threadIdx.x; c < next - b.chunk0; c += 64) chunk_frame[b.chunk0 + c] = c < b.nchunks ? f : 0xFFFFFFFFu;
     for (uint32_t t = threadIdx.x; t < b.ntiles; t += 64) tile_frame[b.tile0 + t] = f;
@@ -1482,15 +1512,12 @@
         if (grid == 0) grid = L.total_chunks;
     }
     hb_prof_begin(fused ? "k_match_fused" : "k_match", s);
-    if (fused) launch_match_fused(a, grid, desc, records, 0u, s, d_bf, chunk_frame, L.total_chunks);
-    else launch_match(a, grid, desc, records, L.total_chunks, s, d_bf, chunk_frame);
+    if (fused) launch_match_fused(a, grid, desc, records, 0u, s, nullptr, d_bf, chunk_frame, L.total_chunks);
+    else launch_match(a, grid, desc, records, L.total_chunks, s, nullptr, d_bf, chunk_frame);
     hb_prof_end(s);
     hb_prof_begin("k_tiles", s);
-    hipLaunchKernelGGL(k_tiles, dim3(L.total_tiles), dim3(256), 0, s, desc, 0u, tile_agg, tile_nf, (const BatchFrame *)d_bf, (const uint32_t *)tile_frame);
-    hb_prof_end(s);
-    hb_prof_begin("k_scan", s);
-    hipLaunchKernelGGL(k_scan, dim3((unsigned)nframes), dim3(256), 0, s, tile_agg, tile_nf, tile_pre, tile_suf, 0u, 0u, (uint64_t)0, (EncPlan *)nullptr,
-                       (uint8_t *)nullptr, fi, (hb_result *)nullptr, has_index, (const BatchFrame *)d_bf);
+    hipLaunchKernelGGL(k_tiles, dim3(L.total_tiles), dim3(256), 0, s, desc, 0u, tile_agg, tile_nf, tile_pre, tile_suf, 0u, (uint64_t)0, (EncPlan *)nullptr,
+                       (uint8_t *)nullptr, fi, (hb_result *)nullptr, has_index, (const BatchFrame *)d_bf, (const uint32_t *)tile_frame);
     hb_prof_end(s);
     if (fused || fused_bits) {
         const int rc = hb_launch_filter_batch(fused_bits ? HB_OP_BITSHUFFLE : HB_OP_SHUFFLE, d_jobs + nframes, nframes, max_n, typesize, s, 1);
```

After: 400.7 GB/s (median of 6 runs). About the same (+0.6%).
